# OER-9000/MB-iSTFT-VITS

Hardware: AMD Instinct MI355X
Metric: audio samples/sec (22.05 kHz), MB-iSTFT-VITS infer, batch 64 per GPU (higher is better)
Workload: dtype f32; 1 GPU; configs[1]: ljs_mb_istft_vits, batch 64 per GPU, infer(noise_scale=0, length_scale=1), all 8 outputs; global_batch=64, t_text=200, t_frames_max=566, parallelism=utterance-sharded dp1

## Files before the change

### include/mbistft_vits.h

```cpp
#ifndef MBISTFT_VITS_H
#define MBISTFT_VITS_H

#include <stddef.h>
#include <stdint.h>

#ifdef __cplusplus
extern "C" {
#endif

#define MBV_ABI_VERSION 3

#define MBV_DEC_MULTIBAND   0
#define MBV_DEC_MULTISTREAM 1
#define MBV_DEC_SINGLEBAND  2

typedef struct mbv_model mbv_model;

typedef struct mbv_config {
  int32_t struct_bytes;
  int32_t n_vocab;
  int32_t inter_channels;
  int32_t hidden_channels;
  int32_t filter_channels;
  int32_t n_heads;
  int32_t n_layers;
  int32_t kernel_size;
  int32_t upsample_initial_channel;
  int32_t spec_channels;
  int32_t resblock_kernel_sizes[3];
  int32_t resblock_dilations[3][3];
  int32_t resblock_type;
  int32_t n_speakers;
  int32_t gin_channels;
  int32_t decoder;
  int32_t device;
  int32_t use_sdp;
} mbv_config;

typedef struct mbv_outputs {
  float *o;
  float *o_mb;
  float *spec;
  float *phase;
  float *attn;
  float *y_mask;
  float *z;
  float *z_p;
  float *m_p;
  float *logs_p;
} mbv_outputs;

int  mbv_abi_version(void);
int  mbv_create(const mbv_config *cfg, mbv_model **out);
void mbv_destroy(mbv_model *m);
const char *mbv_last_error(const mbv_model *m);

int mbv_load_weight(mbv_model *m, const char *name, const float *data,
                    const int64_t *shape, int ndim);
int mbv_finalize_weights(mbv_model *m, void *stream);

int64_t mbv_arena_floats(mbv_model *m);
int mbv_export_arena(mbv_model *m, float *dst, int64_t capacity, void *stream);
int mbv_import_arena(mbv_model *m, const float *src, int64_t n_floats, void *stream);
int mbv_missing_weights(mbv_model *m, char *buf, size_t cap);

int mbv_encode(mbv_model *m, const int64_t *ids, const int64_t *lengths, const int64_t *sid,
               int B, int T, float length_scale, const float *noise_w, float noise_scale_w,
               int64_t *y_lengths_out, void *stream);

int mbv_synthesize(mbv_model *m, int t_frames, const float *noise, float noise_scale,
                   int max_len, const mbv_outputs *outs, void *stream);

int mbv_decode(mbv_model *m, const float *z, const float *g, int B, int t_frames,
               const mbv_outputs *outs, void *stream);

int mbv_decoder_context(const mbv_config *cfg, int32_t out[2]);
int mbv_decode_range(mbv_model *m, const float *z, const float *g, int B, int t_frames, int first, int count,
                     float *o, int64_t o_row_stride, void *stream);

int mbv_ragged_classes(const mbv_config *cfg, int splitk, int t_max, int32_t *first, int capacity);
int mbv_ragged_plan(const mbv_config *cfg, int splitk, int B, int t_frames, const int64_t *lengths, int32_t *run_of_row);
int mbv_decode_ragged(mbv_model *m, const float *z, const float *g, int B, int t_frames, const int64_t *lengths_host,
                      float *o, void *stream);
int mbv_synthesize_ragged(mbv_model *m, int t_frames, const float *noise, float noise_scale, int max_len,
                          const mbv_outputs *outs, const int64_t *y_lengths_host, void *stream);

typedef struct mbv_chunk {
  const float *z;
  int64_t z_stride;
  const float *g;
  int32_t t_frames;
  int32_t first, count;
  float *o;
} mbv_chunk;
int mbv_chunks_plan(const mbv_config *cfg, int splitk, int n, const int32_t *t_frames, int32_t *run_of_chunk);
int mbv_decode_chunks(mbv_model *m, const mbv_chunk *chunks_host, int n, void *stream);
int mbv_decode_chunks_routed(mbv_model *m, const mbv_chunk *chunks_host, const int32_t *route_frames, int n,
                             void *stream);
int64_t mbv_decoder_runs(mbv_model *m);

int mbv_tail_plan(const mbv_config *cfg, int32_t *out, int capacity);
int mbv_decode_masked(mbv_model *m, const float *z, const float *g, const int32_t *lengths, int B, int t_frames,
                      const mbv_outputs *outs, void *stream);
int64_t mbv_tail_dropped(mbv_model *m);

typedef struct mbv_enc_row {
  float length_scale, noise_scale_w;
  const float *noise_w;
  const void *durations;
  int32_t durations_dtype;
  int32_t t_text;
} mbv_enc_row;
typedef struct mbv_row {
  const float *noise;
  int64_t noise_stride;
  float noise_scale;
  int32_t keep;
  float *z;
} mbv_row;
int mbv_admit_plan(const mbv_config *cfg, int splitk, int n, const int32_t *t_text, int32_t *run_of_request);
int mbv_encode_rows(mbv_model *m, int slot, const int64_t *ids, const int64_t *lengths, const int64_t *sid, int B, int T,
                    const mbv_enc_row *rows_host, int64_t *y_lengths_out, void *stream);
int mbv_synthesize_rows(mbv_model *m, int slot, int t_frames, const mbv_row *rows_host, int n, void *stream);
int64_t mbv_encoder_runs(mbv_model *m);

int mbv_speaker_embedding(mbv_model *m, const int64_t *sid, int B, float *out, void *stream);

#define MBV_SPEAKER_SLOTS 256
#define MBV_BLEND_MAX 16
typedef struct mbv_speaker_def {
  int32_t slot;
  int32_t count;
  int32_t ids[MBV_BLEND_MAX];
  float weights[MBV_BLEND_MAX];
  const float *vector;
} mbv_speaker_def;
int mbv_speakers_define(mbv_model *m, const mbv_speaker_def *defs, int n, void *stream);
int mbv_speaker_release(mbv_model *m, int slot, void *stream);
int mbv_speaker_slots(void);
int mbv_speaker_defined(mbv_model *m, int64_t sid);
int64_t mbv_speaker_runs(mbv_model *m);

int mbv_set_option(mbv_model *m, const char *name, int value);
int mbv_get_option(mbv_model *m, const char *name);

int mbv_stage_times_ms(mbv_model *m, float out[5]);
int64_t mbv_ticket(mbv_model *m);
int mbv_stage_times_ms_at(mbv_model *m, int64_t ticket, float out[5]);

int mbv_kernel_times_ms(mbv_model *m, float out[2]);

int mbv_istft_pqmf(mbv_model *m, const float *x_post, int B, int t_frames, const float *filter,
                   int multistream, float *o, float *o_mb, float *spec, float *phase,
                   void *stream);

int mbv_voice_conversion(mbv_model *m, const float *y, const int64_t *y_lengths,
                         const int64_t *sid_src, const int64_t *sid_tgt, int B, int T,
                         const float *noise, const mbv_outputs *outs, int32_t *status, void *stream);

typedef struct mbv_align_outputs {
  int32_t *w;
  float *attn;
  float *x_mask;
  float *y_mask;
  float *z;
  float *z_p;
  float *m_p;
  float *logs_p;
  float *neg_cent;
} mbv_align_outputs;
int mbv_align(mbv_model *m, const int64_t *ids, const int64_t *lengths, const float *y, const int64_t *y_lengths,
              const int64_t *sid, int B, int T_text, int T_spec, const float *noise, float noise_scale,
              const mbv_align_outputs *outs, int32_t *status, void *stream);

int mbv_set_durations(mbv_model *m, const void *w, int dtype, int B, int T, int64_t *y_lengths_out, void *stream);

int mbv_istft_finalize(mbv_model *m, const float *spec, const float *phase, int B, int frames,
                       float *o, float *o_mb, void *stream);

int mbv_pcm16(mbv_model *m, const float *wave, const int64_t *y_lengths, int B, int64_t stride,
              int auto_normalize, int16_t *pcm, void *stream);

int mbv_pcm16_samples(mbv_model *m, const float *wave, const int64_t *valid_samples, int B, int64_t stride,
                      int auto_normalize, int16_t *pcm, void *stream);

#define MBV_RESAMPLE_KAISER_BEST 0
#define MBV_RESAMPLE_KAISER_FAST 1
// ... 210 lines not shown
  const void *wave;
  int64_t samples;
  int32_t wave_dtype;
  int32_t sid_src, sid_tgt;
  const float *noise;
  float noise_scale;
  float *z;
} mbv_convert_row;
int mbv_convert_plan(const mbv_config *cfg, int splitk, int n, const int32_t *t_frames, int32_t *run_of_request);
int mbv_convert_rows(mbv_model *m, const mbv_convert_row *rows_host, int n, int t_frames, int hop, int win,
                     float *g_out, void *stream);
int64_t mbv_converter_runs(mbv_model *m);

typedef struct mbv_convert_range {
  const void *wave;
  int64_t arrived;
  int32_t closed;
  int32_t wave_dtype;
  int32_t sid_src, sid_tgt;
  int32_t first, count;
  const float *noise;
  int64_t noise_stride;
  float noise_scale;
  float *z;
  int64_t z_stride;
} mbv_convert_range;
int mbv_converter_context(const mbv_config *cfg, int32_t out[2]);
int64_t mbv_spectrogram_ready(int64_t arrived, int closed, int n_fft, int hop);
int mbv_convert_window(const mbv_config *cfg, int first, int count, int64_t final_frames, int32_t out[2]);
int mbv_convert_ranges_plan(const mbv_config *cfg, int n, const int32_t *window_frames, int32_t *run_of_range);
int mbv_convert_ranges(mbv_model *m, const mbv_convert_range *rows_host, int n, int hop, int win, void *stream);

int64_t mbv_read_stage(mbv_model *m, const char *name, float *dst, int64_t capacity,
                       void *stream);

int mbv_op_rel_attention(mbv_model *m, const float *qkv, const float *emb_k, const float *emb_v,
                         const int64_t *lengths, float *o, int B, int H, int n_heads, int T, void *stream);

int mbv_op_conv1d(mbv_model *m, const float *x, const float *w_host, const float *bias_host,
                  float *y, int B, int Cin, int Cout, int T, int K, int dilation,
                  float in_slope, void *stream);

#define MBV_CONV_KIND_CONV 0
#define MBV_CONV_KIND_CONVT4 4
#define MBV_CONV_KIND_CONVT8 8
#define MBV_CONV_EPI_STORE 0
#define MBV_CONV_EPI_RESID 1
#define MBV_CONV_EPI_RESID_ACC 2
#define MBV_CONV_EPI_LN 7
typedef struct mbv_conv_desc {
  int32_t B, Cin, Cout, Tin, T, K, dil;
  int32_t x_rstride;
  int32_t kind;
  int32_t epi;
  float in_slope;
  int32_t relu, reflect1;
  const int32_t *in_lens;
  const int32_t *out_lens;
  const float *chan_add;
  const float *res;
  const float *res_chan_add;
  const float *accum_in;
  float out_scale;
  const int64_t *trim_lens;
  int32_t trim_num, trim_add;
  int32_t splitk;
  int32_t prec;
  int32_t legacy_convt;
  int64_t ws_floats;
  int32_t n_counters;
  const float *ln_gamma;
  const float *ln_beta;
  const int32_t *ln_out_lens;
  int32_t tail_once;
} mbv_conv_desc;
#define MBV_ROUTE_NARROW_M 1
#define MBV_ROUTE_NARROW_LAUNCH 2
#define MBV_ROUTE_M64 3
#define MBV_ROUTE_HALF 4
#define MBV_ROUTE_SMALL 5
#define MBV_ROUTE_BIG 6
#define MBV_ROUTE_SPLIT_BATCH 7
#define MBV_ROUTE_VS 8
int mbv_op_conv(mbv_model *m, const mbv_conv_desc *d, const float *x, const float *w_host, const float *bias_host,
                float *y, int32_t *plan_out, void *stream);
int mbv_conv_plan(const mbv_conv_desc *d, int32_t out[8]);

int mbv_op_embed(mbv_model *m, const int64_t *ids, const int64_t *lengths, const float *emb, float *x, int32_t *lens32,
                 int32_t *bad, int B, int T, int H, int n_vocab, void *stream);
int mbv_op_layernorm(mbv_model *m, const float *a, const float *r, const float *gamma, const float *beta, float *y,
                     int B, int C, int T, int pre_relu, const int32_t *out_lens, void *stream);
int mbv_op_durations(mbv_model *m, const float *h, const float *w, const float *bias, const int32_t *lens,
                     float length_scale, float *logw, float *w_ceil, int32_t *cum, int32_t *ylen32, int64_t *ylen64,
                     const int32_t *bad, int B, int C, int T, void *stream);
int mbv_op_expand(mbv_model *m, const float *stats, const int32_t *cum, const int32_t *ylen32, const float *noise,
                  float noise_scale, float *m_p, float *logs_p, float *z_p, float *z, float *attn, float *y_mask,
                  int B, int I, int T, int Tp, void *stream);
int mbv_op_cond_gemv(mbv_model *m, const float *g, const float *W, const float *bias, float *out, int B, int Cin,
                     int Cout, void *stream);
int mbv_op_gather_rows(mbv_model *m, const float *table, const int64_t *sid, float *out, int B, int C, int n_rows,
                       int32_t *bad, void *stream);
int mbv_op_posterior_sample(mbv_model *m, const float *stats, const float *noise, const int32_t *lens, float *z,
                            int B, int I, int T, void *stream);
int mbv_op_lens(mbv_model *m, const int64_t *lengths, int32_t *lens32, int32_t *bad, float *mask, int B, int T,
                void *stream);
int mbv_op_dds_sep(mbv_model *m, const float *x, const int32_t *lens, const float *w, const float *bias,
                   const float *gamma, const float *beta, float *y, int B, int C, int T, int K, int dil, void *stream);
int mbv_op_dds_res(mbv_model *m, const float *a, const float *xres, const float *gamma, const float *beta, float *y,
                   int B, int C, int T, const int32_t *out_lens, void *stream);
int mbv_op_sdp_pre(mbv_model *m, const float *z, int zc, const float *pre_w, const float *pre_b, const float *cond,
                   float *h, int B, int C, int T, void *stream);
int mbv_op_sdp_spline(mbv_model *m, const float *h, float *z, const int32_t *lens, int B, int C, int T,
                      float edge_const, void *stream);
int mbv_op_sdp_logw(mbv_model *m, const float *z, const float *mean, const float *logs, const int32_t *lens,
                    float *logw, int B, int T, void *stream);
int mbv_op_sdp_noise(mbv_model *m, const float *noise, float scale, float *z, int64_t n, void *stream);
int mbv_op_chan_add(mbv_model *m, float *x, const float *v, int B, int C, int T, void *stream);
int mbv_op_istft_single(mbv_model *m, const float *x_post, int B, int frames, int prescaled, float *o, float *spec,
                        float *phase, void *stream);
int mbv_op_neg_cent(mbv_model *m, const float *z_p, const float *m_p, const float *logs_p, const int32_t *t_y32,
                    const int32_t *t_x32, float *value, int B, int I, int T_t, int T_s, void *stream);
int mbv_op_max_path(mbv_model *m, const float *value, const int32_t *t_y32, const int32_t *t_x32, int32_t *w_out,
                    int32_t *path_out, int32_t *status, int B, int T_t, int T_s, void *stream);

#ifdef __cplusplus
}
#endif
#endif
```

### mb-istft-vits_amd/_capi.py

```python
import ctypes as C
import os
import subprocess

_HERE = os.path.dirname(os.path.abspath(__file__))
CSRC = os.path.join(_HERE, "csrc")
LIB_PATH = os.environ.get("MBV_LIB") or os.path.join(CSRC, "libmbistft_vits.so")

SYMBOLS = [
    "mbv_abi_version", "mbv_create", "mbv_destroy", "mbv_last_error", "mbv_load_weight",
    "mbv_finalize_weights", "mbv_missing_weights", "mbv_encode", "mbv_synthesize", "mbv_decode",
    "mbv_speaker_embedding", "mbv_stage_times_ms", "mbv_istft_pqmf", "mbv_read_stage",
    "mbv_op_conv1d", "mbv_kernel_times_ms", "mbv_istft_finalize", "mbv_pcm16", "mbv_voice_conversion",
    "mbv_set_option", "mbv_arena_floats", "mbv_export_arena", "mbv_import_arena", "mbv_ticket", "mbv_stage_times_ms_at", "mbv_op_rel_attention",
    "mbv_pcm16_samples", "mbv_resample", "mbv_resample_bank", "mbv_op_conv", "mbv_conv_plan",
    "mbv_spectrogram", "mbv_spectrogram_frames", "mbv_decoder_context", "mbv_decode_range",
    "mbv_resample_ready", "mbv_resample_pcm16_range",
    "mbv_ragged_classes", "mbv_decode_ragged", "mbv_synthesize_ragged", "mbv_ragged_plan",
    "mbv_chunks_plan", "mbv_decode_chunks", "mbv_decoder_runs",
    "mbv_pcm_chunks_plan", "mbv_resample_pcm16_chunks", "mbv_wire_runs",
    "mbv_op_embed", "mbv_op_layernorm", "mbv_op_durations", "mbv_op_expand", "mbv_op_cond_gemv", "mbv_op_gather_rows",
    "mbv_op_posterior_sample", "mbv_op_lens", "mbv_op_dds_sep", "mbv_op_dds_res", "mbv_op_sdp_pre", "mbv_op_sdp_spline",
    "mbv_op_sdp_logw", "mbv_op_sdp_noise", "mbv_op_chan_add", "mbv_op_istft_single",
    "mbv_align", "mbv_set_durations", "mbv_op_neg_cent", "mbv_op_max_path",
    "mbv_admit_plan", "mbv_encode_rows", "mbv_synthesize_rows", "mbv_encoder_runs", "mbv_get_option",
    "mbv_tail_plan", "mbv_tail_dropped", "mbv_decode_masked",
    "mbv_convert_plan", "mbv_convert_rows", "mbv_converter_runs",
    "mbv_decode_chunks_routed", "mbv_converter_context", "mbv_spectrogram_ready", "mbv_convert_window",
    "mbv_convert_ranges_plan", "mbv_convert_ranges",
    "mbv_resample_ready_open", "mbv_resample_ranges", "mbv_input_runs",
    "mbv_randn_blocks", "mbv_randn_host", "mbv_noise_runs",
    "mbv_limiter_ready", "mbv_resample_pcm16_range_limited", "mbv_resample_pcm16_chunks_limited",
    "mbv_g711_encode", "mbv_g711_decode", "mbv_resample_g711_range", "mbv_resample_g711_chunks",
    "mbv_pcm_fade_make", "mbv_resample_pcm16_range_faded", "mbv_resample_pcm16_chunks_faded",
    "mbv_resample_g711_range_faded", "mbv_resample_g711_chunks_faded",
    "mbv_token_marks", "mbv_token_marks_rows",
    "mbv_kweighting", "mbv_loudness_segments", "mbv_loudness", "mbv_loudness_range", "mbv_loudness_chunks",
    "mbv_loudness_runs",
    "mbv_turn_plan", "mbv_resample_turns",
    "mbv_shape_durations", "mbv_shape_durations_rows", "mbv_op_shape_durations", "mbv_shape_runs",
    "mbv_frame_gain", "mbv_frame_gain_rows", "mbv_op_frame_gain", "mbv_gain_runs",
    "mbv_resample_pcm16_range_shaped", "mbv_resample_pcm16_chunks_shaped", "mbv_resample_turns_shaped",
    "mbv_warp_plan", "mbv_warp_ready", "mbv_warp_ranges", "mbv_warp_runs",
    "mbv_speakers_define", "mbv_speaker_release", "mbv_speaker_slots", "mbv_speaker_defined", "mbv_speaker_runs",
]


ABI_VERSION = 3


class MbvConfig(C.Structure):
    _fields_ = [
        ("struct_bytes", C.c_int32), ("n_vocab", C.c_int32), ("inter_channels", C.c_int32),
        ("hidden_channels", C.c_int32), ("filter_channels", C.c_int32), ("n_heads", C.c_int32),
        ("n_layers", C.c_int32), ("kernel_size", C.c_int32),
        ("upsample_initial_channel", C.c_int32), ("spec_channels", C.c_int32),
        ("resblock_kernel_sizes", C.c_int32 * 3), ("resblock_dilations", (C.c_int32 * 3) * 3),
        ("resblock_type", C.c_int32),
        ("n_speakers", C.c_int32), ("gin_channels", C.c_int32), ("decoder", C.c_int32),
        ("device", C.c_int32), ("use_sdp", C.c_int32),
    ]


class MbvOutputs(C.Structure):
    _fields_ = [(n, C.c_void_p) for n in
                ("o", "o_mb", "spec", "phase", "attn", "y_mask", "z", "z_p", "m_p", "logs_p")]


class MbvChunk(C.Structure):
    _fields_ = [("z", C.c_void_p), ("z_stride", C.c_int64), ("g", C.c_void_p), ("t_frames", C.c_int32),
                ("first", C.c_int32), ("count", C.c_int32), ("o", C.c_void_p)]


class MbvPcmChunk(C.Structure):
    _fields_ = [("wave", C.c_void_p), ("in_total", C.c_int64), ("valid_samples", C.c_void_p),
                ("in_avail", C.c_int64), ("out_first", C.c_int64), ("out_count", C.c_int64), ("peak", C.c_void_p),
                ("pcm", C.c_void_p), ("pcm_capacity", C.c_int64), ("running_peak", C.c_void_p),
                ("out_samples", C.c_void_p)]


class MbvPcmLimit(C.Structure):
    _fields_ = [("ceiling", C.c_float), ("lookahead", C.c_int32), ("hold", C.c_int32)]


class MbvPcmFade(C.Structure):
    _fields_ = [("first", C.c_int64), ("count", C.c_int64), ("inv", C.c_float)]


def pcm_fade(first, count):
    f = MbvPcmFade()
    if lib().mbv_pcm_fade_make(int(first), int(count), C.byref(f)):
        raise ValueError("a fade is (first, count) with first >= 0 and count >= 0, got (%r, %r)" % (first, count))
    return f


NO_FADE = (0, -1, 0.0)


class MbvTurnSeg(C.Structure):
    _fields_ = [("wave", C.c_void_p), ("start", C.c_int64), ("length", C.c_int64), ("ramp", C.c_int32)]


class MbvTurnChunk(C.Structure):
    _fields_ = [("chunk", MbvPcmChunk), ("segs", C.POINTER(MbvTurnSeg)), ("n_segs", C.c_int32)]


TURN_MAX_SEGS = 4096


# ... 41 lines not shown


class MbvLoudnessChunk(C.Structure):
    _fields_ = [("wave", C.c_void_p), ("in_total", C.c_int64), ("valid_samples", C.c_void_p), ("in_avail", C.c_int64),
                ("seg_first", C.c_int64), ("seg_count", C.c_int64), ("state", C.c_void_p), ("energies", C.c_void_p),
                ("energy_capacity", C.c_int64), ("loudness", C.c_void_p)]


def kweighting(rate):
    c, m = (C.c_double * 10)(), (C.c_double * 16)()
    if lib().mbv_kweighting(int(rate), c, m):
        raise ValueError((lib().mbv_last_error(None) or b"mbv_kweighting failed").decode())
    return list(c), list(m)


def loudness_segments(rate, samples):
    hop = C.c_int32()
    n = lib().mbv_loudness_segments(int(rate), int(samples), C.byref(hop))
    if n < 0:
        raise ValueError((lib().mbv_last_error(None) or b"mbv_loudness_segments failed").decode())
    return int(hop.value), int(n)


class MbvEncRow(C.Structure):
    _fields_ = [("length_scale", C.c_float), ("noise_scale_w", C.c_float), ("noise_w", C.c_void_p),
                ("durations", C.c_void_p), ("durations_dtype", C.c_int32), ("t_text", C.c_int32)]


class MbvRow(C.Structure):
    _fields_ = [("noise", C.c_void_p), ("noise_stride", C.c_int64), ("noise_scale", C.c_float), ("keep", C.c_int32),
                ("z", C.c_void_p)]


class MbvConvertRow(C.Structure):
    _fields_ = [("wave", C.c_void_p), ("samples", C.c_int64), ("wave_dtype", C.c_int32), ("sid_src", C.c_int32),
                ("sid_tgt", C.c_int32), ("noise", C.c_void_p), ("noise_scale", C.c_float), ("z", C.c_void_p)]


class MbvConvertRange(C.Structure):
    _fields_ = [("wave", C.c_void_p), ("arrived", C.c_int64), ("closed", C.c_int32), ("wave_dtype", C.c_int32),
                ("sid_src", C.c_int32), ("sid_tgt", C.c_int32), ("first", C.c_int32), ("count", C.c_int32),
                ("noise", C.c_void_p), ("noise_stride", C.c_int64), ("noise_scale", C.c_float), ("z", C.c_void_p),
                ("z_stride", C.c_int64)]


class MbvResampleRange(C.Structure):
    _fields_ = [("wave", C.c_void_p), ("wave_dtype", C.c_int32), ("in_avail", C.c_int64), ("in_total", C.c_int64),
                ("out_first", C.c_int64), ("out_count", C.c_int64), ("out", C.c_void_p), ("out_capacity", C.c_int64)]


class MbvRandnBlock(C.Structure):
    _fields_ = [("dst", C.c_void_p), ("stride", C.c_int64), ("channels", C.c_int32), ("reserved", C.c_int32),
                ("first", C.c_int64), ("count", C.c_int64), ("seed", C.c_uint64), ("purpose", C.c_uint32),
                ("row", C.c_uint32)]


G711_LAWS = {"ulaw": 1, "alaw": 2}
WAVE_F32, WAVE_PCM16, WAVE_ULAW, WAVE_ALAW = 0, 1, 8, 9


NOISE_PRIOR, NOISE_SDP, NOISE_POSTERIOR = 0, 1, 2


class MbvAlignOutputs(C.Structure):
    _fields_ = [(n, C.c_void_p) for n in
                ("w", "attn", "x_mask", "y_mask", "z", "z_p", "m_p", "logs_p", "neg_cent")]


class MbvConvDesc(C.Structure):
    _fields_ = [(n, C.c_int32) for n in ("B", "Cin", "Cout", "Tin", "T", "K", "dil", "x_rstride", "kind", "epi")] + [
        ("in_slope", C.c_float), ("relu", C.c_int32), ("reflect1", C.c_int32),
        ("in_lens", C.c_void_p), ("out_lens", C.c_void_p), ("chan_add", C.c_void_p), ("res", C.c_void_p),
        ("res_chan_add", C.c_void_p), ("accum_in", C.c_void_p), ("out_scale", C.c_float),
        ("trim_lens", C.c_void_p), ("trim_num", C.c_int32), ("trim_add", C.c_int32),
        ("splitk", C.c_int32), ("prec", C.c_int32), ("legacy_convt", C.c_int32),
        ("ws_floats", C.c_int64), ("n_counters", C.c_int32),
        ("ln_gamma", C.c_void_p), ("ln_beta", C.c_void_p), ("ln_out_lens", C.c_void_p),
        ("tail_once", C.c_int32),
    ]


CONV_KIND_CONV, CONV_KIND_CONVT4, CONV_KIND_CONVT8 = 0, 4, 8
CONV_EPI_STORE, CONV_EPI_RESID, CONV_EPI_RESID_ACC, CONV_EPI_LN = 0, 1, 2, 7
ROUTES = {1: "NARROW_M", 2: "NARROW_LAUNCH", 3: "M64", 4: "HALF", 5: "SMALL", 6: "BIG", 7: "SPLIT_BATCH", 8: "VS"}
PLAN_FIELDS = ("route", "bm", "bn", "threads", "ck", "nb_big", "vs_tv", "S")


def build(force=False, verbose=False):
    if force:
        for f in os.listdir(CSRC):
            if f.endswith(".o") or f.endswith(".so"):
                os.remove(os.path.join(CSRC, f))
    r = subprocess.run(["bash", os.path.join(CSRC, "build.sh")], capture_output=True, text=True)
    if verbose or r.returncode:
        print(r.stdout, r.stderr)
    if r.returncode:
        raise RuntimeError("building libmbistft_vits.so failed:\n" + r.stderr[-4000:])
    return LIB_PATH


_lib = None


def lib():
    global _lib
    if _lib is not None:
        return _lib
    if not os.path.isfile(LIB_PATH):
        raise RuntimeError("%s not found: build it with `python -c 'import __graft_entry__ as g; "
                           "g.build()'` (hipcc, gfx950). There is no CPU fallback." % LIB_PATH)
    import torch
    L = C.CDLL(LIB_PATH)
    vp, i32, i64p, fp = C.c_void_p, C.c_int, C.POINTER(C.c_int64), C.c_void_p
    L.mbv_abi_version.restype = i32
    L.mbv_create.argtypes = [C.POINTER(MbvConfig), C.POINTER(vp)]
    L.mbv_destroy.argtypes = [vp]
    L.mbv_destroy.restype = None
    L.mbv_last_error.argtypes = [vp]
    L.mbv_last_error.restype = C.c_char_p
    L.mbv_load_weight.argtypes = [vp, C.c_char_p, vp, i64p, i32]
    L.mbv_finalize_weights.argtypes = [vp, vp]
    L.mbv_missing_weights.argtypes = [vp, C.c_char_p, C.c_size_t]
    L.mbv_encode.argtypes = [vp, vp, vp, vp, i32, i32, C.c_float, vp, C.c_float, vp, vp]
    L.mbv_synthesize.argtypes = [vp, i32, vp, C.c_float, i32, C.POINTER(MbvOutputs), vp]
    L.mbv_decode.argtypes = [vp, vp, vp, i32, i32, C.POINTER(MbvOutputs), vp]
    L.mbv_decoder_context.argtypes = [C.POINTER(MbvConfig), C.POINTER(C.c_int32 * 2)]
    L.mbv_decode_range.argtypes = [vp, vp, vp, i32, i32, i32, i32, vp, C.c_int64, vp]
    L.mbv_speaker_embedding.argtypes = [vp, vp, i32, vp, vp]
    L.mbv_stage_times_ms.argtypes = [vp, C.POINTER(C.c_float * 5)]
    L.mbv_kernel_times_ms.argtypes = [vp, C.POINTER(C.c_float * 2)]
    L.mbv_istft_pqmf.argtypes = [vp, vp, i32, i32, vp, i32, vp, vp, vp, vp, vp]
    L.mbv_istft_finalize.argtypes = [vp, vp, vp, i32, i32, vp, vp, vp]
    L.mbv_voice_conversion.argtypes = [vp, vp, vp, vp, vp, i32, i32, vp, C.POINTER(MbvOutputs), vp, vp]
    L.mbv_pcm16.argtypes = [vp, vp, vp, i32, C.c_int64, i32, vp, vp]
    L.mbv_pcm16_samples.argtypes = [vp, vp, vp, i32, C.c_int64, i32, vp, vp]
    L.mbv_resample.argtypes = [vp, vp, vp, i32, C.c_int64, i32, i32, i32, vp, C.c_int64, vp, vp]
    L.mbv_resample_bank.argtypes = [i32, i32, i32, vp, C.c_int64, C.POINTER(C.c_int32), C.POINTER(C.c_int32),
                                    C.POINTER(C.c_int32)]
    L.mbv_resample_ready.argtypes = [i32, i32, i32, C.c_int64, C.c_int64]
    L.mbv_resample_ready.restype = C.c_int64
    L.mbv_resample_pcm16_range.argtypes = [vp, vp, vp, i32, C.c_int64, i32, i32, i32, C.c_int64, C.c_int64, C.c_int64,
                                           vp, vp, C.c_int64, vp, vp, vp]
    L.mbv_spectrogram.argtypes = [vp, vp, i32, vp, i32, C.c_int64, i32, i32, i32, vp, C.c_int64, vp, vp]
    L.mbv_spectrogram_frames.argtypes = [C.c_int64, i32, i32]
    L.mbv_spectrogram_frames.restype = C.c_int64
    L.mbv_set_option.argtypes = [vp, C.c_char_p, i32]
    L.mbv_ticket.argtypes = [vp]
    L.mbv_ticket.restype = C.c_int64
    L.mbv_stage_times_ms_at.argtypes = [vp, C.c_int64, C.POINTER(C.c_float * 5)]
    L.mbv_arena_floats.argtypes = [vp]
    L.mbv_arena_floats.restype = C.c_int64
    L.mbv_export_arena.argtypes = [vp, vp, C.c_int64, vp]
    L.mbv_import_arena.argtypes = [vp, vp, C.c_int64, vp]
    L.mbv_read_stage.argtypes = [vp, C.c_char_p, vp, C.c_int64, vp]
    L.mbv_read_stage.restype = C.c_int64
    L.mbv_op_rel_attention.argtypes = [vp, vp, vp, vp, vp, vp, i32, i32, i32, i32, vp]
    L.mbv_op_conv1d.argtypes = [vp, vp, vp, vp, vp, i32, i32, i32, i32, i32, i32, C.c_float, vp]
    L.mbv_op_conv.argtypes = [vp, C.POINTER(MbvConvDesc), vp, vp, vp, vp, C.POINTER(C.c_int32 * 8), vp]
    L.mbv_conv_plan.argtypes = [C.POINTER(MbvConvDesc), C.POINTER(C.c_int32 * 8)]
    f32 = C.c_float
    L.mbv_op_embed.argtypes = [vp, vp, vp, vp, vp, vp, vp, i32, i32, i32, i32, vp]
    L.mbv_op_layernorm.argtypes = [vp, vp, vp, vp, vp, vp, i32, i32, i32, i32, vp, vp]
    L.mbv_op_durations.argtypes = [vp, vp, vp, vp, vp, f32, vp, vp, vp, vp, vp, vp, i32, i32, i32, vp]
    L.mbv_op_expand.argtypes = [vp, vp, vp, vp, vp, f32, vp, vp, vp, vp, vp, vp, i32, i32, i32, i32, vp]
    L.mbv_op_cond_gemv.argtypes = [vp, vp, vp, vp, vp, i32, i32, i32, vp]
    L.mbv_op_gather_rows.argtypes = [vp, vp, vp, vp, i32, i32, i32, vp, vp]
    L.mbv_op_posterior_sample.argtypes = [vp, vp, vp, vp, vp, i32, i32, i32, vp]
    L.mbv_op_lens.argtypes = [vp, vp, vp, vp, vp, i32, i32, vp]
    L.mbv_op_dds_sep.argtypes = [vp, vp, vp, vp, vp, vp, vp, vp, i32, i32, i32, i32, i32, vp]
    L.mbv_op_dds_res.argtypes = [vp, vp, vp, vp, vp, vp, i32, i32, i32, vp, vp]
    L.mbv_op_sdp_pre.argtypes = [vp, vp, i32, vp, vp, vp, vp, i32, i32, i32, vp]
    L.mbv_op_sdp_spline.argtypes = [vp, vp, vp, vp, i32, i32, i32, f32, vp]
    L.mbv_op_sdp_logw.argtypes = [vp, vp, vp, vp, vp, vp, i32, i32, vp]
    L.mbv_op_sdp_noise.argtypes = [vp, vp, f32, vp, C.c_int64, vp]
    L.mbv_op_chan_add.argtypes = [vp, vp, vp, i32, i32, i32, vp]
    L.mbv_op_istft_single.argtypes = [vp, vp, i32, i32, i32, vp, vp, vp, vp]
    L.mbv_align.argtypes = [vp, vp, vp, vp, vp, vp, i32, i32, i32, vp, f32, C.POINTER(MbvAlignOutputs), vp, vp]
    L.mbv_set_durations.argtypes = [vp, vp, i32, i32, i32, vp, vp]
    L.mbv_op_neg_cent.argtypes = [vp, vp, vp, vp, vp, vp, vp, i32, i32, i32, i32, vp]
    L.mbv_op_max_path.argtypes = [vp, vp, vp, vp, vp, vp, vp, i32, i32, i32, vp]
    optional = ("mbv_ragged_classes", "mbv_ragged_plan", "mbv_decode_ragged", "mbv_synthesize_ragged",
                "mbv_chunks_plan", "mbv_decode_chunks", "mbv_decoder_runs",
                "mbv_pcm_chunks_plan", "mbv_resample_pcm16_chunks", "mbv_wire_runs",
                "mbv_admit_plan", "mbv_encode_rows", "mbv_synthesize_rows", "mbv_encoder_runs",
                "mbv_get_option", "mbv_tail_plan", "mbv_tail_dropped", "mbv_decode_masked",
                "mbv_convert_plan", "mbv_convert_rows", "mbv_converter_runs",
                "mbv_decode_chunks_routed", "mbv_converter_context", "mbv_spectrogram_ready", "mbv_convert_window",
                "mbv_convert_ranges_plan", "mbv_convert_ranges",
                "mbv_resample_ready_open", "mbv_resample_ranges", "mbv_input_runs",
                "mbv_randn_blocks", "mbv_randn_host", "mbv_noise_runs",
                "mbv_limiter_ready", "mbv_resample_pcm16_range_limited", "mbv_resample_pcm16_chunks_limited",
                "mbv_g711_encode", "mbv_g711_decode", "mbv_resample_g711_range",
                "mbv_resample_g711_chunks",
                "mbv_pcm_fade_make", "mbv_resample_pcm16_range_faded", "mbv_resample_pcm16_chunks_faded",
                "mbv_resample_g711_range_faded", "mbv_resample_g711_chunks_faded",
                "mbv_token_marks", "mbv_token_marks_rows",
                "mbv_kweighting", "mbv_loudness_segments", "mbv_loudness", "mbv_loudness_range", "mbv_loudness_chunks",
                "mbv_loudness_runs", "mbv_turn_plan", "mbv_resample_turns",
                "mbv_shape_durations", "mbv_shape_durations_rows", "mbv_op_shape_durations", "mbv_shape_runs",
                "mbv_frame_gain", "mbv_frame_gain_rows", "mbv_op_frame_gain", "mbv_gain_runs",
                "mbv_resample_pcm16_range_shaped", "mbv_resample_pcm16_chunks_shaped",
                "mbv_resample_turns_shaped",
                "mbv_warp_plan", "mbv_warp_ready", "mbv_warp_ranges", "mbv_warp_runs",
                "mbv_speakers_define", "mbv_speaker_release", "mbv_speaker_slots", "mbv_speaker_defined",
                "mbv_speaker_runs") if os.environ.get("MBV_LIB") else ()
    if hasattr(L, "mbv_ragged_classes") or not optional:
        L.mbv_ragged_classes.argtypes = [C.POINTER(MbvConfig), i32, i32, C.POINTER(C.c_int32), i32]
        L.mbv_ragged_plan.argtypes = [C.POINTER(MbvConfig), i32, i32, i32, i64p, C.POINTER(C.c_int32)]
        L.mbv_decode_ragged.argtypes = [vp, vp, vp, i32, i32, i64p, vp, vp]
        L.mbv_synthesize_ragged.argtypes = [vp, i32, vp, C.c_float, i32, C.POINTER(MbvOutputs), i64p, vp]
    if hasattr(L, "mbv_decode_chunks") or not optional:
        L.mbv_chunks_plan.argtypes = [C.POINTER(MbvConfig), i32, i32, C.POINTER(C.c_int32), C.POINTER(C.c_int32)]
        L.mbv_decode_chunks.argtypes = [vp, C.POINTER(MbvChunk), i32, vp]
        L.mbv_decoder_runs.argtypes = [vp]
        L.mbv_decoder_runs.restype = C.c_int64
    if hasattr(L, "mbv_resample_pcm16_chunks") or not optional:
        L.mbv_pcm_chunks_plan.argtypes = [i32, i32, i32, C.POINTER(MbvPcmChunk), i32, i64p]
        L.mbv_pcm_chunks_plan.restype = C.c_int64
        L.mbv_resample_pcm16_chunks.argtypes = [vp, C.POINTER(MbvPcmChunk), i32, i32, i32, i32, vp, C.c_int64, vp]
        L.mbv_wire_runs.argtypes = [vp]
        L.mbv_wire_runs.restype = C.c_int64
    if hasattr(L, "mbv_encode_rows") or not optional:
        L.mbv_admit_plan.argtypes = [C.POINTER(MbvConfig), i32, i32, C.POINTER(C.c_int32), C.POINTER(C.c_int32)]
        L.mbv_encode_rows.argtypes = [vp, i32, vp, vp, vp, i32, i32, C.POINTER(MbvEncRow), vp, vp]
        L.mbv_synthesize_rows.argtypes = [vp, i32, i32, C.POINTER(MbvRow), i32, vp]
        L.mbv_encoder_runs.argtypes = [vp]
        L.mbv_encoder_runs.restype = C.c_int64
        L.mbv_get_option.argtypes = [vp, C.c_char_p]
    if hasattr(L, "mbv_tail_plan") or not optional:
        L.mbv_tail_plan.argtypes = [C.POINTER(MbvConfig), C.POINTER(C.c_int32), i32]
        L.mbv_tail_dropped.argtypes = [vp]
        L.mbv_tail_dropped.restype = C.c_int64
        L.mbv_decode_masked.argtypes = [vp, vp, vp, vp, i32, i32, C.POINTER(MbvOutputs), vp]
    if hasattr(L, "mbv_convert_rows") or not optional:
        L.mbv_convert_plan.argtypes = [C.POINTER(MbvConfig), i32, i32, C.POINTER(C.c_int32), C.POINTER(C.c_int32)]
        L.mbv_convert_rows.argtypes = [vp, C.POINTER(MbvConvertRow), i32, i32, i32, i32, vp, vp]
        L.mbv_converter_runs.argtypes = [vp]
        L.mbv_converter_runs.restype = C.c_int64
    if hasattr(L, "mbv_convert_ranges") or not optional:
        L.mbv_decode_chunks_routed.argtypes = [vp, C.POINTER(MbvChunk), C.POINTER(C.c_int32), i32, vp]
        L.mbv_converter_context.argtypes = [C.POINTER(MbvConfig), C.POINTER(C.c_int32 * 2)]
        L.mbv_spectrogram_ready.argtypes = [C.c_int64, i32, i32, i32]
        L.mbv_spectrogram_ready.restype = C.c_int64
        L.mbv_convert_window.argtypes = [C.POINTER(MbvConfig), i32, i32, C.c_int64, C.POINTER(C.c_int32 * 2)]
        L.mbv_convert_ranges_plan.argtypes = [C.POINTER(MbvConfig), i32, C.POINTER(C.c_int32), C.POINTER(C.c_int32)]
        L.mbv_convert_ranges.argtypes = [vp, C.POINTER(MbvConvertRange), i32, i32, i32, vp]
    if hasattr(L, "mbv_resample_ranges") or not optional:
        L.mbv_resample_ready_open.argtypes = [i32, i32, i32, C.c_int64]
        L.mbv_resample_ready_open.restype = C.c_int64
        L.mbv_resample_ranges.argtypes = [vp, C.POINTER(MbvResampleRange), i32, i32, i32, i32, vp]
        L.mbv_input_runs.argtypes = [vp]
        L.mbv_input_runs.restype = C.c_int64
    if hasattr(L, "mbv_randn_blocks") or not optional:
        L.mbv_randn_blocks.argtypes = [vp, C.POINTER(MbvRandnBlock), i32, vp]
        L.mbv_randn_host.argtypes = [C.c_uint64, C.c_uint32, C.c_uint32, C.c_uint32, C.c_int64, C.c_int64, vp]
        L.mbv_noise_runs.argtypes = [vp]
        L.mbv_noise_runs.restype = C.c_int64
    if hasattr(L, "mbv_limiter_ready") or not optional:
        L.mbv_limiter_ready.argtypes = [i32, i32, i32, C.c_int64, C.c_int64, i32]
        L.mbv_limiter_ready.restype = C.c_int64
        L.mbv_resample_pcm16_range_limited.argtypes = [vp, vp, vp, i32, C.c_int64, i32, i32, i32, C.c_int64, C.c_int64,
                                                       C.c_int64, vp, vp, C.c_int64, vp, vp, C.POINTER(MbvPcmLimit), vp]
        L.mbv_resample_pcm16_chunks_limited.argtypes = [vp, C.POINTER(MbvPcmChunk), C.POINTER(MbvPcmLimit), i32, i32,
                                                        i32, i32, vp, C.c_int64, vp]
    if hasattr(L, "mbv_resample_g711_range") or not optional:
        L.mbv_g711_encode.argtypes = [vp, vp, C.c_int64, i32, vp, vp]
        L.mbv_g711_decode.argtypes = [vp, vp, C.c_int64, i32, vp, vp]
        L.mbv_resample_g711_range.argtypes = [vp, vp, vp, i32, C.c_int64, i32, i32, i32, C.c_int64, C.c_int64, C.c_int64,
                                              vp, vp, C.c_int64, vp, vp, C.POINTER(MbvPcmLimit), i32, vp]
        L.mbv_resample_g711_chunks.argtypes = [vp, C.POINTER(MbvPcmChunk), C.POINTER(MbvPcmLimit), i32, i32, i32, i32,
                                               i32, vp, C.c_int64, vp]
    if hasattr(L, "mbv_pcm_fade_make") or not optional:
        fadep = C.POINTER(MbvPcmFade)
        L.mbv_pcm_fade_make.argtypes = [C.c_int64, C.c_int64, fadep]
        L.mbv_resample_pcm16_range_faded.argtypes = [vp, vp, vp, i32, C.c_int64, i32, i32, i32, C.c_int64, C.c_int64,
                                                     C.c_int64, vp, vp, C.c_int64, vp, vp, C.POINTER(MbvPcmLimit),
                                                     fadep, vp]
        L.mbv_resample_pcm16_chunks_faded.argtypes = [vp, C.POINTER(MbvPcmChunk), C.POINTER(MbvPcmLimit), fadep, i32,
                                                      i32, i32, i32, vp, C.c_int64, vp]
        L.mbv_resample_g711_range_faded.argtypes = [vp, vp, vp, i32, C.c_int64, i32, i32, i32, C.c_int64, C.c_int64,
                                                    C.c_int64, vp, vp, C.c_int64, vp, vp, C.POINTER(MbvPcmLimit), i32,
                                                    fadep, vp]
        L.mbv_resample_g711_chunks_faded.argtypes = [vp, C.POINTER(MbvPcmChunk), C.POINTER(MbvPcmLimit), fadep, i32,
                                                     i32, i32, i32, i32, vp, C.c_int64, vp]
    if hasattr(L, "mbv_token_marks") or not optional:
        L.mbv_token_marks.argtypes = [vp, vp, C.c_int64, vp]
        L.mbv_token_marks_rows.argtypes = [vp, i32, C.POINTER(MbvMarkRow), i32, vp]
    if hasattr(L, "mbv_loudness") or not optional:
        dp = C.POINTER(C.c_double)
        L.mbv_kweighting.argtypes = [i32, dp, dp]
        L.mbv_loudness_segments.argtypes = [i32, C.c_int64, C.POINTER(C.c_int32)]
        L.mbv_loudness_segments.restype = C.c_int64
        L.mbv_loudness.argtypes = [vp, vp, vp, i32, C.c_int64, i32, vp, vp, vp]
        L.mbv_loudness_range.argtypes = [vp, vp, vp, i32, C.c_int64, i32, C.c_int64, C.c_int64, C.c_int64, vp, vp,
                                         C.c_int64, vp, vp]
        L.mbv_loudness_chunks.argtypes = [vp, C.POINTER(MbvLoudnessChunk), i32, i32, vp]
        L.mbv_loudness_runs.argtypes = [vp]
        L.mbv_loudness_runs.restype = C.c_int64
    if hasattr(L, "mbv_resample_turns") or not optional:
        L.mbv_turn_plan.argtypes = [i32, i32, i32, C.POINTER(MbvTurnChunk), C.POINTER(MbvPcmLimit), i32, i64p]
        L.mbv_turn_plan.restype = C.c_int64
        L.mbv_resample_turns.argtypes = [vp, C.POINTER(MbvTurnChunk), C.POINTER(MbvPcmLimit), C.POINTER(MbvPcmFade), i32,
                                         i32, i32, i32, i32, vp, C.c_int64, vp]
    if hasattr(L, "mbv_shape_durations") or not optional:
        L.mbv_shape_durations.argtypes = [vp, vp, vp, C.POINTER(MbvFit), i32, i32, vp, vp, vp]
        L.mbv_shape_durations_rows.argtypes = [vp, i32, C.POINTER(MbvShapeRow), i32, vp, vp]
        L.mbv_op_shape_durations.argtypes = [vp, vp, vp, vp, vp, f32, C.POINTER(MbvFit), vp, vp, vp, vp, vp, vp, i32, i32,
                                             vp]
        L.mbv_shape_runs.argtypes = [vp]
        L.mbv_shape_runs.restype = C.c_int64
    if hasattr(L, "mbv_frame_gain") or not optional:
        envp = C.POINTER(MbvPcmEnvelope)
        L.mbv_frame_gain.argtypes = [vp, vp, vp, C.c_int64, i32, vp]
        L.mbv_frame_gain_rows.argtypes = [vp, i32, C.POINTER(MbvGainRow), i32, vp]
        L.mbv_op_frame_gain.argtypes = [vp, vp, vp, vp, vp, C.c_int64, i32, i32, i32, vp]
        L.mbv_gain_runs.argtypes = [vp]
# ... 41 lines not shown
```

### mb-istft-vits_amd/csrc/capi.hip

```cpp
#include "../../include/mbistft_vits.h"
#include "kernels.h"
#include "g711.h"

#include <algorithm>
#include <array>
#include <cmath>
#include <cstdarg>
#include <cstdio>
#include <cstdlib>
#include <cstring>
#include <map>
#include <set>
#include <string>
#include <vector>

using namespace mbv;

namespace {

constexpr int kWindow = 4;
constexpr int kDpFilter = 256;
constexpr int kFlowLayers = 4;
constexpr int kFlowK = 5;
constexpr int kNFlows = 4;
// ... 886 lines not shown
    HIPCHK(m, hipMalloc((void**)&m->darena, arena.size() * sizeof(float)));
    m->darena_floats = arena.size();
  }
  if (m->import_src) {
    if ((int64_t)arena.size() != m->import_n)
      return m->fail("mbv_import_arena: %lld floats offered, this configuration's arena has %zu (exported by another configuration or library build?)",
                     (long long)m->import_n, arena.size());
    HIPCHK(m, hipMemcpyAsync(m->darena, m->import_src, arena.size() * sizeof(float), hipMemcpyDeviceToDevice, stream));
    m->raw.clear();
  } else {
    HIPCHK(m, hipMemcpyAsync(m->darena, arena.data(), arena.size() * sizeof(float),
                             hipMemcpyHostToDevice, stream));
  }
  HIPCHK(m, hipStreamSynchronize(stream));
  m->arena_used = arena.size();
  m->harena.swap(arena);
  m->finalized = true;
  m->split_valid = false;
  if (m->conv_bf16 == 3 && ensure_split_arena(m, stream)) return 1;
  return reblend_voices(m, stream);
}

struct Bump {
  char* base; size_t cap, off = 0;
  template <typename Tp> Tp* take(size_t n) {
    off = align_up(off, 256);
    Tp* p = base ? reinterpret_cast<Tp*>(base + off) : nullptr;
    off += n * sizeof(Tp);
    return p;
  }
  bool fits() const { return off <= cap; }
};

int ensure(mbv_model* m, char** buf, size_t* cap, size_t need) {
  if (*cap >= need) return 0;
  if (*buf) { HIPCHK(m, hipDeviceSynchronize()); HIPCHK(m, hipFree(*buf)); *buf = nullptr; *cap = 0; }
  need = align_up(need + (need >> 3), 1 << 20);
  HIPCHK(m, hipMalloc((void**)buf, need));
  *cap = need;
  return 0;
}

template <typename Carve>
int lay_out(mbv_model* m, const char* who, char** buf, size_t* cap, Carve&& carve) {
  Bump sc{*buf, *cap};
  if (*buf) carve(sc);
  if (*buf && sc.fits()) return 0;
  Bump measure{nullptr, 0};
  carve(measure);
  if (ensure(m, buf, cap, measure.off)) return 1;
  sc = Bump{*buf, *cap};
  carve(sc);
  return sc.fits() ? 0 : m->fail("%s: scratch layout exceeds its buffer", who);
}

ConvArgs conv_shape(int Cin, int M, int K, int dil, int Tin, int T, int B, int splitk) {
  ConvArgs a{};
  a.Cin = Cin; a.M = M; a.Mpad = (int)align_up(M, 128); a.K = K; a.dil = dil; a.pad_left = (K - 1) * dil / 2;
  a.Tin = Tin; a.x_rstride = Tin; a.x_bstride = (int64_t)Cin * Tin;
  a.T = T; a.y_bstride = (int64_t)M * T; a.epi = EPI_STORE; a.in_slope = 1.f; a.out_scale = 1.f; a.B = B;
  a.splitk = splitk;
  return a;
}

ConvArgs conv_bind(const mbv_model* m, const PConv& p, ConvArgs a, const float* x, float* y) {
  a.x = x; a.y = y;
  a.w = m->W(p.w); a.bias = p.has_bias ? m->W(p.bias) : nullptr;
  a.w_split = m->Wsplit(p.w);
  a.ws = m->conv_ws; a.ws_floats = m->conv_ws_floats; a.counters = m->conv_cnt; a.n_counters = m->conv_ncnt;
  a.prec = a.w_split ? 3 : 0;
  return a;
}

ConvArgs conv_args(const mbv_model* m, const PConv& p, const float* x, int64_t x_bstride, int Tin,
                   float* y, int64_t y_bstride, int T, int B, int dil = 1) {
  ConvArgs a = conv_shape(p.Cin, p.M, p.K, dil, Tin, T, B, m->splitk);
  a.x_bstride = x_bstride; a.y_bstride = y_bstride;
  return conv_bind(m, p, a, x, y);
}


int tail_mode(const mbv_model* m) { return (!m->trim && !m->splitk && m->conv_bf16 != 3) ? m->tail_once : 0; }
bool tail_stage(int mode, int B, long conv_tiles) { return B > 1 && (mode == 2 || (mode == 1 && conv_tiles > 256)); }

bool decoder_stage_concurrent(const mbv_model* m, int B, int ch, int Lo, bool tail = false) {
  const long conv_tiles = (long)B * ((Lo + 383) / 384) * ((ch + 127) / 128);
  return m->dec_streams && m->aux_ok && m->cfg.resblock_type != 2 && (conv_tiles <= 192 || tail) && !m->trim;
}

struct DecodeRange {
  int t_full;
  int keep_first, keep_count;
  float* o;
  int64_t o_row_stride;
  const PoolRow* rows = nullptr;
  int max_keep = 0;
};

std::vector<DecLaunch> decoder_table(const mbv_config& c) {
  const bool sb = c.decoder == MBV_DEC_SINGLEBAND;
  const int us = dec_us(c), C0 = c.upsample_initial_channel;
  const int kPre = 7, kPost = 7;
  const int n_fft = 16, hop = 4;
  const int bands = sb ? 1 : 4, taps = 63;
  const int nq = c.resblock_type == 2 ? 2 : 3;
  std::vector<DecLaunch> t;
  auto conv = [&](int kind, int stage, int j, int q, int Cin, int M, int K, int dil, int num, int epi) -> DecLaunch& {
    DecLaunch e{};
    e.kind = kind; e.stage = stage; e.j = j; e.q = q;
    e.Cin = Cin; e.M = M; e.K = K; e.dil = dil; e.pad_left = (K - 1) * dil / 2;
    e.num = e.rate = num; e.lens = stage + 1; e.epi = epi; e.res = epi == EPI_RESID || epi == EPI_RESID_ACC;
    t.push_back(e);
    return t.back();
  };
  conv(DL_PRE, -1, 0, 0, c.inter_channels, C0, kPre, 1, 1, EPI_STORE);
  int num = 1;
  for (int i = 0; i < 2; ++i) {
    const int ch = C0 >> (i + 1);
    DecLaunch& u = conv(DL_UP, i, 0, 0, C0 >> i, us * ch, convt_taps(us), 1, num, EPI_CONVT);
    u.pad_left = convt_pad_left(us); u.convt_u = us; u.rate = us * num; u.lens = i;
    u.tk = kConvtK; u.tp = (kConvtK - us) / 2;
    num *= us;
    for (int j = 0; j < 3; ++j) {
      const int k = c.resblock_kernel_sizes[j];
      for (int q = 0; q < nq; ++q) {
        const int d = c.resblock_dilations[j][q];
        const int last = q == nq - 1 ? EPI_RESID_ACC : EPI_RESID;
        if (c.resblock_type == 2) {
          DecLaunch& e = conv(DL_C2, i, j, q, ch, ch, k, d, num, last);
          e.chan_add = e.res_chan_add = q == 0;
        } else {
          conv(DL_C1, i, j, q, ch, ch, k, d, num, EPI_STORE).chan_add = q == 0;
          conv(DL_C2, i, j, q, ch, ch, k, 1, num, last).res_chan_add = q == 0;
        }
      }
    }
  }
  DecLaunch& p = conv(DL_POST, 2, 0, 0, C0 >> 2, 2 * (n_fft / 2 + 1) * bands, kPost, 1, num, EPI_STORE);
  p.add = 1; p.reflect1 = 1; p.lens = 2;
  DecLaunch w{};
  w.kind = DL_TAIL; w.stage = 2; w.num = num; w.add = 1; w.rate = num * hop * bands;
  w.n_fft = n_fft; w.hop = hop; w.bands = bands; w.taps = taps;
  t.push_back(w);
  return t;
}

ConvArgs dec_shape(const DecLaunch& e, int len, int B, int splitk) {
  ConvArgs a = conv_shape(e.Cin, e.M, e.K, e.dil, e.num * len, e.num * len + e.add, B, splitk);
  a.pad_left = e.pad_left; a.epi = e.epi; a.convt_u = e.convt_u; a.reflect1 = e.reflect1;
  if (e.res) a.res_bstride = a.y_bstride;
  return a;
}
ConvArgs dec_planner_args(const DecLaunch& e, int len, int B, int splitk, int prec = 0, bool cond = false) {
  static const float kSome = 0.f;
  ConvArgs a = dec_shape(e, len, B, splitk);
  if (e.res) a.res = &kSome;
  if (cond && e.chan_add) a.chan_add = &kSome;
  if (cond && e.res_chan_add) a.res_chan_add = &kSome;
  a.prec = prec;
  return a;
}

struct Span { int64_t lo, hi; };
static Span span_conv(Span y, int K, int dil, int pad_left) { return {y.lo - pad_left, y.hi + (int64_t)(K - 1) * dil - pad_left}; }
static int64_t floor_div(int64_t a, int64_t b) { return a >= 0 ? a / b : -((-a + b - 1) / b); }
static int64_t ceil_div(int64_t a, int64_t b) { return -floor_div(-a, b); }
// ... 3 lines not shown
void decoder_context(const std::vector<DecLaunch>& table, int* Lc, int* Rc) {
  const int64_t t = 1 << 20;
  Span x{}, need{}, r{};
  for (size_t n = table.size(); n-- > 0;) {
    const DecLaunch& e = table[n];
    switch (e.kind) {
      case DL_TAIL:
        x = {e.rate * t, e.rate * t + e.rate - 1};
        if (e.bands > 1) x = {ceil_div(x.lo - e.taps / 2, e.bands), floor_div(x.hi + e.taps / 2, e.bands)};
        x = {ceil_div(x.lo + e.n_fft / 2 - (e.n_fft - 1), e.hop), floor_div(x.hi + e.n_fft / 2, e.hop)};
        break;
      case DL_POST:
        need = r = x = span_conv(x, e.K, e.dil, e.pad_left + e.reflect1);
        break;
      case DL_C1: case DL_C2:
        if (e.epi == EPI_RESID_ACC) { need = span_union(need, r); r = x; }
        r = span_conv(r, e.K, e.dil, e.pad_left);
        break;
      case DL_UP:
        need = r = x = span_convt(span_union(need, r), e.tk, e.convt_u, e.tp);
        break;
      case DL_PRE:
        x = span_conv(x, e.K, e.dil, e.pad_left);
        break;
    }
  }
  *Lc = (int)(t - x.lo);
  *Rc = (int)(x.hi - t);
}

static int64_t reach_conv(int64_t hi, int pad_left) { return hi + pad_left; }
static int64_t reach_convt(int64_t hi, int k, int u, int p) { return (int64_t)u * hi - p + k - 1; }
struct TailLaunch { int kind, stage, j, q, rate, reach; };
void decoder_tail_plan(const std::vector<DecLaunch>& table, std::vector<TailLaunch>* out) {
  out->clear();
  const int64_t len = 1 << 20;
  int64_t sum_hi = len - 1;
  int64_t hi = sum_hi, r = sum_hi;
  for (const DecLaunch& e : table) {
    int64_t h = 0;
    switch (e.kind) {
      case DL_PRE:
        h = sum_hi = reach_conv(sum_hi, e.pad_left);
        break;
      case DL_UP:
        h = hi = r = sum_hi = reach_convt(sum_hi, e.tk, e.convt_u, e.tp);
        break;
      case DL_C1: case DL_C2:
        h = r = reach_conv(r, e.pad_left);
        if (e.epi == EPI_RESID_ACC) { h = sum_hi = sum_hi > r ? sum_hi : r; r = hi; }
        break;
      case DL_POST:
        h = sum_hi = reach_conv(sum_hi, e.pad_left + e.reflect1);
        break;
      case DL_TAIL:
        h = e.hop * sum_hi + e.n_fft / 2 - 1;
        if (e.bands > 1) h = e.bands * h + e.taps / 2;
        break;
    }
    out->push_back({e.kind, e.stage, e.j, e.q, e.rate, (int)(h - ((int64_t)e.rate * len - 1))});
  }
}

struct RaggedRows {
  const int* len;
  const int* len_u;
  const int* len_uu;
  const int* row_map;
  float* o;
  int64_t o_row_stride;
  int t_min;
};

struct DecCall { int B, Td, zstride; bool lens, cond, own_o, ranged, ragged; };

constexpr int kTrimMargin = 32;
struct DecBufs {
  DecCall call;
  bool trim, tail;
  float* x0;
  struct TrimMap { int num, add, T, bn; int* map; bool built; };
  TrimMap trim_maps[12]; int n_trim;
  int trim_of[48];
  struct TailMap { int kind, j, q, bn; const int* map; };
  struct Stage { float *u, *t1s[3], *rs[3], *xs, *cb[3]; bool conc; int n_tail; TailMap tail_maps[kTailMapJobs]; TailMapJobs jobs; } st[2];
  int Bc;
  float *xpost, *otmp;
};

void carve_decoder(const mbv_model* m, const DecCall& k, Bump& sc, DecBufs* out) {
  const mbv_config& c = m->cfg;
  const std::vector<DecLaunch>& table = m->dec_table;
  const int B = k.B, Td = k.Td;
  DecBufs& d = *out;
  std::memset(&d, 0, sizeof d); d.call = k;
  d.trim = k.ragged ? !m->splitk : (m->trim && k.lens && !m->splitk && c.decoder != MBV_DEC_SINGLEBAND);
  d.tail = tail_mode(m) && !d.trim && !k.ragged && !k.ranged && k.lens && B > 1 && B <= 65535 && !k.cond;
  auto planned = [&](const DecLaunch& e) {
    ConvArgs a = dec_planner_args(e, Td, B, m->splitk, m->Wsplit(0) ? 3 : 0,
                                  k.cond && e.stage >= 0 && e.stage < 2 && m->rb[e.stage * 3 + e.j].cw.present);
    if (e.kind == DL_PRE) { a.x_rstride = k.zstride; a.x_bstride = (int64_t)e.Cin * k.zstride; }
    return a;
  };
  std::vector<TailLaunch> tail_plan;
  if (d.tail) decoder_tail_plan(table, &tail_plan);
  d.x0 = sc.take<float>((size_t)B * table[0].M * Td);
  for (const DecLaunch& up : table) {
    if (up.kind != DL_UP) continue;
    DecBufs::Stage& st = d.st[up.stage];
    const int ch = up.M / up.convt_u, Lo = up.rate * Td;
    const size_t n = (size_t)B * ch * Lo;
    const long stage_tiles = (long)B * ((Lo + 383) / 384) * ((ch + 127) / 128);
    if (d.tail && tail_stage(tail_mode(m), B, stage_tiles))
      for (size_t n_e = 0; n_e < table.size() && st.n_tail < kTailMapJobs; ++n_e) {
        const DecLaunch& e = table[n_e];
        if (e.stage != up.stage || (e.kind != DL_C1 && e.kind != DL_C2)) continue;
        const ConvArgs a = planned(e);
        const int bn = conv1d_trim_bn(a);
        if (!bn || conv1d_plan(a, false).route != conv1d_plan(a, true).route) continue;
        st.jobs.job[st.n_tail] = {e.rate, tail_plan[n_e].reach, Lo, bn, nullptr};
        st.tail_maps[st.n_tail++] = {e.kind, e.j, e.q, bn, nullptr};
      }
    st.conc = decoder_stage_concurrent(m, B, ch, Lo, st.n_tail > 0) && !d.trim;
    st.u = sc.take<float>(n);
    for (int j = 0; j < 3; ++j) {
      st.t1s[j] = j == 0 || st.conc ? sc.take<float>(n) : st.t1s[0];
      st.rs[j] = j == 0 || st.conc ? sc.take<float>(n) : st.rs[0];
    }
    st.xs = sc.take<float>(n);
  }
  for (const DecLaunch& up : table)
    for (int j = 0; j < 3 && up.kind == DL_UP; ++j)
      if (k.cond && m->rb[up.stage * 3 + j].cw.present) d.st[up.stage].cb[j] = sc.take<float>((size_t)B * (up.M / up.convt_u));
  const DecLaunch& post = table[table.size() - 2];
  const int64_t utt_bytes = (int64_t)post.M * (post.num * (int64_t)Td + post.add) * 4;
  int64_t cap_bytes = (1LL << 31) - 1;
  if (m->xpost_chunk_bytes > 0 && m->xpost_chunk_bytes < cap_bytes) cap_bytes = m->xpost_chunk_bytes;
  d.Bc = utt_bytes > (1LL << 31) - 1 ? 0 : (int)std::min<int64_t>(B, std::max<int64_t>(1, cap_bytes / utt_bytes));
  for (size_t n_e = 0; n_e < table.size(); ++n_e) {
    const DecLaunch& e = table[n_e];
    d.trim_of[n_e] = -1;
    if (!d.trim || e.kind == DL_TAIL || (e.kind == DL_POST && d.Bc != B)) continue;
    const ConvArgs a = planned(e);
    const int bn = conv1d_trim_bn(a);
    for (int t = 0; bn && t < d.n_trim && d.trim_of[n_e] < 0; ++t)
      if (d.trim_maps[t].num == e.num && d.trim_maps[t].add == e.add && d.trim_maps[t].T == a.T && d.trim_maps[t].bn == bn) d.trim_of[n_e] = t;
    if (bn && d.trim_of[n_e] < 0 && d.n_trim < 12) {
      d.trim_of[n_e] = d.n_trim;
      d.trim_maps[d.n_trim++] = {e.num, e.add, a.T, bn, sc.take<int>(launch_trim_map_ints(B, a.T, bn)), false};
    }
  }
  for (auto& st : d.st)
    for (int i = 0; i < st.n_tail; ++i)
      st.tail_maps[i].map = st.jobs.job[i].out = sc.take<int>(launch_tail_map_ints(B, st.jobs.job[i].T, st.jobs.job[i].BN));
  d.xpost = sc.take<float>((size_t)d.Bc * (utt_bytes / 4));
  if (k.own_o) d.otmp = sc.take<float>((size_t)B * table.back().rate * Td);
}

int run_decoder(mbv_model* m, const float* z, const int* zlens, const float* gvec, const mbv_outputs* outs,
                hipStream_t s, DecBufs& d, const DecodeRange* rg = nullptr, const RaggedRows* rr = nullptr) {
  const mbv_config& c = m->cfg;
  const std::vector<DecLaunch>& table = m->dec_table;
  const int B = d.call.B, Td = d.call.Td, zstride = d.call.zstride, gin = c.gin_channels;
  ++m->decoder_runs;
  if (rr) zlens = rr->len;
  float* o = rg ? rg->o : rr ? rr->o : outs ? outs->o : nullptr;
  const bool pooled = rg && rg->rows;
  if (d.call.lens != (zlens != nullptr) || d.call.cond != (gvec && gin) || d.call.ranged != (rg != nullptr) ||
      d.call.ragged != (rr != nullptr) || d.call.own_o != (!o && !pooled))
    return m->fail("internal error: the decoder's scratch was laid out for another call");
  if (!d.Bc)
    return m->fail("utterance too long for one launch: %d frames (x_post of ONE utterance must stay below 2 GiB)", Td);
  if (!o) o = d.otmp;
  const int rt_num = rg && !m->splitk ? rg->t_full : 0;
  hipStream_t const s_main = s;
  const int* const rr_lens[3] = {rr ? rr->len : nullptr, rr ? rr->len_u : nullptr, rr ? rr->len_uu : nullptr};
  auto conv = [&](const DecLaunch& e, const PConv& p, const float* x, float* y, float in_slope, int nb) {
    ConvArgs a = conv_bind(m, p, dec_shape(e, Td, nb, m->splitk), x, y);
    a.in_slope = in_slope;
    if (rr) a.in_lens = rr_lens[e.lens];
    return a;
  };
  HIPCHK(m, hipEventRecord(m->evk[0], s));
  bool route_drift = false, tail_drift = false;
  auto narrow_alone = [&](const ConvArgs& a, int num, int add, int len) {
    ConvArgs s1 = a;
    s1.B = 1; s1.trim_map = nullptr;
    s1.T = num * len + add;
    s1.Tin = a.Tin - a.T + s1.T;
    s1.x_rstride = s1.Tin; s1.x_bstride = (int64_t)a.Cin * s1.Tin;
    s1.y_bstride = a.y_bstride / a.T * s1.T;
    s1.res_bstride = a.res ? (int64_t)a.M * s1.T : 0;
    const int r = conv1d_plan(s1, false).route;
    return r == CONV_NARROW_M || r == CONV_NARROW_LAUNCH;
  };
  auto with_trim = [&](ConvArgs& a, const DecLaunch& e) {
    if (rr && !m->splitk) {
      const bool narrow_long = narrow_alone(a, e.num, e.add, rg ? rg->t_full : Td);
      if (narrow_alone(a, e.num, e.add, rr->t_min) != narrow_long) route_drift = true;
      if (rg) {
        const int r = conv1d_plan(a, false, rt_num * e.num + e.add).route;
        if ((r == CONV_NARROW_M || r == CONV_NARROW_LAUNCH) != narrow_long) route_drift = true;
      }
    }
    if (!d.trim) return;
    const int at = d.trim_of[&e - table.data()], bn = conv1d_trim_bn(a);
    if (bn != (at < 0 ? 0 : d.trim_maps[at].bn)) { tail_drift = true; return; }
    if (at < 0) return;
    DecBufs::TrimMap& k = d.trim_maps[at];
    if (!k.built) launch_trim_map(zlens, B, e.num, e.num * (rr ? 0 : kTrimMargin) + e.add, a.T, bn, k.map, s_main);
    k.built = true;
    a.trim_map = k.map; a.trim_bn = bn;
  };
  const DecBufs::Stage* tail_stage_bufs = nullptr;
  auto with_tail = [&](ConvArgs& a, const DecLaunch& e) -> const DecBufs::TailMap* {
    for (int n_t = 0; n_t < tail_stage_bufs->n_tail; ++n_t) {
      const DecBufs::TailMap& t = tail_stage_bufs->tail_maps[n_t];
      if (t.kind != e.kind || t.j != e.j || t.q != e.q) continue;
      if (conv1d_trim_bn(a) != t.bn) { tail_drift = true; return nullptr; }
      a.trim_map = t.map; a.trim_bn = t.bn;
      return &t;
    }
    return nullptr;
  };
  {
    const DecLaunch& e = table[0];
    ConvArgs a = conv(e, m->conv_pre, z, d.x0, 1.f, B);
    a.x_bstride = (int64_t)e.Cin * zstride;
    a.x_rstride = zstride;
    a.in_lens = zlens;
    with_trim(a, e);
    launch_conv1d(a, s, rt_num);
  }
  m->stages["dec_conv_pre"] = {d.x0, (int64_t)B * table[0].M * Td};
  const float* cur = d.x0;
  size_t next = 1;
  for (int i = 0; i < 2; ++i) {
    DecBufs::Stage& bufs = d.st[i];
    const DecLaunch& up = table[next++];
    const int ch = up.M / up.convt_u;
    const size_t n = (size_t)B * ch * up.rate * Td;
    float *const u = bufs.u, *const xs = bufs.xs;
    const bool conc = bufs.conc;
    tail_stage_bufs = &bufs;
    launch_tail_maps(zlens, B, bufs.jobs, bufs.n_tail, m->tail_cnt, s_main);
    {
      ConvArgs a = conv(up, m->upc[i], cur, u, kLrelu, B);
      with_trim(a, up);
      launch_conv1d(a, s);
    }
    m->stages[i == 0 ? "dec_up_0" : "dec_up_1"] = {u, (int64_t)n};
    if (conc) {
      HIPCHK(m, hipEventRecord(m->ev_fork, s_main));
      for (auto& st : m->aux) HIPCHK(m, hipStreamWaitEvent(st, m->ev_fork, 0));
    }
    auto resblocks = [&]() -> int {
    for (int j = 0; j < 3; ++j) {
      const auto& R = m->rb[i * 3 + j];
      hipStream_t s = (conc && j > 0) ? m->aux[j - 1] : s_main;
      float* const t1 = bufs.t1s[j];
      float* const r = bufs.rs[j];
      auto own_ws = [&](ConvArgs& a) {
        if (!conc) return;
        const size_t third = a.ws_floats / 3;
        const int cthird = a.n_counters / 3;
        a.ws += (size_t)j * third; a.ws_floats = third;
        a.counters += (size_t)j * cthird; a.n_counters = cthird;
      };
      const float* cadd = nullptr;
      if (gvec && gin && R.cw.present) {
        launch_cond_gemv(gvec, nullptr, nullptr, m->W(R.cw.off), m->W(R.cb.off), bufs.cb[j], B, gin, ch, s);
        cadd = bufs.cb[j];
      }
      const float* state = u;
      for (; table[next].stage == i && table[next].j == j; ++next) {
        const DecLaunch& e = table[next];
        const bool first = e.kind == DL_C1, second = !first && c.resblock_type != 2;
        ConvArgs a = conv(e, second ? R.c2[e.q] : R.c1[e.q], second ? t1 : state, first ? t1 : r, kLrelu, B);
        if (e.res) a.res = state;
        if (e.chan_add) a.chan_add = cadd;
        if (e.res_chan_add) a.res_chan_add = cadd;
        if (e.epi == EPI_RESID_ACC) {
          a.y = xs;
          a.accum_in = j == 0 ? nullptr : xs;
          a.out_scale = j == 2 ? (1.f / 3.f) : 1.f;
          if (conc && j > 0) HIPCHK(m, hipStreamWaitEvent(s, m->ev_rb[j - 1], 0));
        }
        own_ws(a);
        with_trim(a, e);
        const DecBufs::TailMap* tm = with_tail(a, e);
        launch_conv1d(a, s, rt_num * e.num);
        if (tm) launch_tail_fill(a.y, a.y_bstride, B, a.M, a.T, tm->bn, tm->map, s);
        if (conc && e.epi == EPI_RESID_ACC) HIPCHK(m, hipEventRecord(m->ev_rb[j], s));
        if (!first) state = r;
      }
    }
    return 0;
    };
    if (resblocks()) {
      if (conc) for (auto& st : m->aux) (void)hipStreamSynchronize(st);
      return 1;
    }
    if (conc) HIPCHK(m, hipStreamWaitEvent(s_main, m->ev_rb[2], 0));
    m->stages[i == 0 ? "dec_res_0" : "dec_res_1"] = {xs, (int64_t)n};
    cur = xs;
  }
  const DecLaunch &post = table[next], &wave = table[next + 1];
  const bool sb = wave.bands == 1;
  const int L = post.num * Td, Fr = L + post.add, prow = post.M, Bc = d.Bc;
  const int bins = wave.n_fft / 2 + 1;
  float* const xpost = d.xpost;
  const int upf = wave.rate / 4;
  IstftRange keep{rg ? upf * rg->keep_first : 0, rg ? upf * (rg->keep_first + rg->keep_count) : 0,
                  rg ? rg->o_row_stride : 0, nullptr, nullptr};
  if (rr) keep = IstftRange{0, upf * Td, rr->o_row_stride, rr->len, rr->row_map};
  const int64_t M4 = (int64_t)wave.rate * Td;
  for (int b0 = 0; b0 < B; b0 += Bc) {
    const int nb = B - b0 < Bc ? B - b0 : Bc;
    {
      ConvArgs a = conv(post, m->conv_post, cur + (size_t)b0 * post.Cin * L, xpost, 0.01f, nb);
      if (rr) a.in_lens += b0;
      if (nb == B) with_trim(a, post);
      launch_conv1d(a, s);
    }
    if (b0 == 0) HIPCHK(m, hipEventRecord(m->evk[1], s));
    const bool plain = !rg && !rr;
    float* const ob = pooled ? nullptr : rr ? o : o + (size_t)b0 * (rg ? rg->o_row_stride : M4);
    auto extra = [&](float* p, int64_t per_row) { return plain && p ? p + (size_t)b0 * per_row : nullptr; };
    IstftRange kb = keep;
    if (rr) { kb.row_lens += b0; kb.row_map += b0; }
    if (sb) {
      IstftSbArgs ia{};
      ia.x_post = xpost; ia.o = ob;
      ia.spec = extra(outs ? outs->spec : nullptr, bins * Fr);
      ia.phase = extra(outs ? outs->phase : nullptr, bins * Fr);
      ia.B = nb; ia.F = Fr; ia.exact_math = m->exact_math; ia.prescaled = 1;
      if (pooled) launch_istft_single_pool(ia, rg->rows + b0, rg->max_keep, s);
      else if (!plain) launch_istft_single_range(ia, kb, s);
      else launch_istft_single(ia, s);
    } else {
      IstftArgs ia{};
      const bool ms = c.decoder == MBV_DEC_MULTISTREAM;
      ia.x_post = xpost; ia.filt = m->W(m->filt.off); ia.o = ob;
      ia.o_mb = extra(outs ? outs->o_mb : nullptr, (ms ? wave.bands : 1) * M4);
      ia.spec = extra(outs ? outs->spec : nullptr, wave.bands * bins * Fr);
      ia.phase = extra(outs ? outs->phase : nullptr, wave.bands * bins * Fr);
      ia.B = nb; ia.Tp = Td; ia.multistream = ms;
      ia.fixed_bank = !ia.multistream; ia.exact_math = m->exact_math; ia.prescaled = 1;
      if (plain && d.trim && nb == B && !ia.o_mb && !ia.spec && !ia.phase) ia.trim_lens = zlens;
      if (pooled) launch_istft_pqmf_pool(ia, rg->rows + b0, rg->max_keep, s);
      else if (!plain) launch_istft_pqmf_range(ia, kb, s);
      else launch_istft_pqmf(ia, s);
    }
  }
  if (Bc == B) m->stages["x_post"] = {xpost, (int64_t)B * prow * Fr};
  m->xpost_F = Fr;
  m->xpost_rows = prow;
  HIPCHK(m, hipEventRecord(m->evk[2], s));
  m->evk_set = true;
  m->evk_split = Bc < B;
  if (tail_drift) return m->fail("internal error: a tile map was planned for another tile width than its launch uses");
  if (route_drift) return m->fail("internal error: a %s run holds rows whose convs plan differently (ragged_classes out of step with run_decoder)", pooled ? "pooled" : "ragged");
  return 0;
}

void ragged_classes(const mbv_config& c, int splitk, int t_max, std::vector<int>* first) {
  first->assign(1, 1);
  if (splitk) return;
  const std::vector<DecLaunch> table = decoder_table(c);
  std::vector<char> prev, cur;
  for (int len = 1; len <= t_max; ++len) {
    cur.clear();
    for (const DecLaunch& e : table) {
      if (e.kind == DL_TAIL) continue;
      const int r = conv1d_plan(dec_planner_args(e, len, 1, 0), false).route;
// ... 3402 lines not shown
  OP_REFUSE((int64_t)B * 18 * frames * 4 >= (1LL << 31), "x_post must stay below 2 GiB");
  OP_BEGIN();
  IstftSbArgs a{};
  a.x_post = x_post; a.o = o; a.spec = spec; a.phase = phase;
  a.B = B; a.F = frames; a.exact_math = m->exact_math; a.prescaled = prescaled != 0;
  launch_istft_single(a, s);
  OP_END();
}

int mbv_op_neg_cent(mbv_model* m, const float* z_p, const float* m_p, const float* logs_p, const int32_t* t_y32,
                    const int32_t* t_x32, float* value, int B, int I, int T_t, int T_s, void* stream) {
  if (!m) return 1;
  OP_REFUSE(!z_p || !m_p || !logs_p || !t_y32 || !t_x32 || !value, "NULL argument");
  OP_REFUSE(B <= 0 || I <= 0 || T_t <= 0 || T_s <= 0, "B, I, T_t and T_s must be > 0");
  OP_REFUSE(B > kGridYZ || (T_t + 63) / 64 > kGridYZ, "B <= 65535 and T_t <= 64 * 65535 required");
  OP_BEGIN();
  launch_neg_cent(z_p, m_p, logs_p, (int64_t)I * T_s, t_y32, t_x32, value, B, I, T_t, T_s, s);
  OP_END();
}

int mbv_op_max_path(mbv_model* m, const float* value, const int32_t* t_y32, const int32_t* t_x32, int32_t* w_out,
                    int32_t* path_out, int32_t* status, int B, int T_t, int T_s, void* stream) {
  if (!m) return 1;
  OP_REFUSE(!value || !t_y32 || !t_x32 || !w_out, "NULL argument");
  OP_REFUSE(B <= 0 || T_t <= 0 || T_s <= 0, "B, T_t and T_s must be > 0");
  OP_REFUSE(!max_path_supported(T_s), "T_s must be <= 1024");
  OP_BEGIN();
  const size_t bits_bytes = max_path_scratch_bytes(B, T_t, T_s);
  if (bits_bytes && ensure(m, &m->scrB, &m->scrB_bytes, bits_bytes)) return 1;
  launch_max_path(value, t_y32, t_x32, w_out, path_out, status, bits_bytes ? m->scrB : nullptr, B, T_t, T_s, s);
  OP_END();
}
#undef OP_REFUSE
#undef OP_BEGIN
#undef OP_END

int mbv_op_conv1d(mbv_model* m, const float* x, const float* w_host, const float* bias_host, float* y,
                  int B, int Cin, int Cout, int T, int K, int dilation, float in_slope, void* stream) {
  if (!m) return 1;
  if (Cin % 32) return m->fail("mbv_op_conv1d: Cin must be a multiple of 32");
  if (!conv1d_supported(K, dilation)) return m->fail("mbv_op_conv1d: K <= 11 and (K-1)*dilation <= 72 required");
  DEVICE_GUARD(m);
  hipStream_t s = (hipStream_t)stream;
  const int Mpad = (int)align_up(Cout, 128);
  std::vector<float> packed((size_t)K * Cin * Mpad, 0.f);
  for (int k = 0; k < K; ++k)
    for (int ci = 0; ci < Cin; ++ci)
      for (int co = 0; co < Cout; ++co)
        packed[conv_pack_index(k, ci, co, Cin, Mpad)] = w_host[((size_t)co * Cin + ci) * K + k];
  float *dw = nullptr, *db = nullptr;
  HIPCHK(m, hipMalloc((void**)&dw, packed.size() * 4));
  HIPCHK(m, hipMemcpy(dw, packed.data(), packed.size() * 4, hipMemcpyHostToDevice));
  if (bias_host) {
    HIPCHK(m, hipMalloc((void**)&db, (size_t)Cout * 4));
    HIPCHK(m, hipMemcpy(db, bias_host, (size_t)Cout * 4, hipMemcpyHostToDevice));
  }
  ConvArgs a{};
  a.x = x; a.x_bstride = (int64_t)Cin * T; a.Tin = T; a.x_rstride = T; a.Cin = Cin;
  a.w = dw; a.bias = db; a.M = Cout; a.Mpad = Mpad; a.K = K; a.dil = dilation;
  a.pad_left = (K - 1) * dilation / 2; a.in_slope = in_slope;
  a.y = y; a.y_bstride = (int64_t)Cout * T; a.T = T; a.epi = EPI_STORE; a.out_scale = 1.f; a.B = B;
  a.ws = m->conv_ws; a.ws_floats = m->conv_ws_floats; a.counters = m->conv_cnt; a.n_counters = m->conv_ncnt;
  a.splitk = m->splitk;
  float* dws = nullptr;
  if (m->conv_bf16 == 3) {
    HIPCHK(m, hipMalloc((void**)&dws, packed.size() * 4));
    launch_split_planes(dw, dws, packed.size(), s);
    a.w_split = dws;
  }
  a.prec = a.w_split ? 3 : 0;
  launch_conv1d(a, s);
  HIPCHK(m, hipStreamSynchronize(s));
  HIPCHK(m, hipFree(dw));
  if (dws) HIPCHK(m, hipFree(dws));
  if (db) HIPCHK(m, hipFree(db));
  return 0;
}

}

namespace {
static_assert(MBV_ROUTE_NARROW_M == CONV_NARROW_M && MBV_ROUTE_NARROW_LAUNCH == CONV_NARROW_LAUNCH &&
              MBV_ROUTE_M64 == CONV_M64 && MBV_ROUTE_HALF == CONV_HALF && MBV_ROUTE_SMALL == CONV_SMALL &&
              MBV_ROUTE_BIG == CONV_BIG && MBV_ROUTE_SPLIT_BATCH == CONV_SPLIT_BATCH && MBV_ROUTE_VS == CONV_VS,
              "route numbers of the C-ABI and the launcher");
static_assert(MBV_CONV_EPI_LN == EPI_LN, "epilogue numbers of the C-ABI and the launcher");

const char* conv_desc_args(const mbv_conv_desc& d, ConvArgs* out) {
  const bool convt = d.kind == MBV_CONV_KIND_CONVT4 || d.kind == MBV_CONV_KIND_CONVT8;
  if (d.kind != MBV_CONV_KIND_CONV && !convt) return "kind must be MBV_CONV_KIND_CONV, _CONVT4 or _CONVT8";
  if (d.B <= 0 || d.Cin <= 0 || d.Cout <= 0 || d.Tin <= 0 || d.T <= 0) return "B, Cin, Cout, Tin and T must be > 0";
  if (d.x_rstride != 0 && d.x_rstride < d.Tin) return "x_rstride must be 0 or >= Tin";
  const bool ln = d.epi == MBV_CONV_EPI_LN;
  if ((d.epi < MBV_CONV_EPI_STORE || d.epi > MBV_CONV_EPI_RESID_ACC) && !ln) return "epi must be STORE, RESID, RESID_ACC or LN";
  if (d.prec != 0 && d.prec != 3) return "prec must be 0 or 3";
  if (d.epi == MBV_CONV_EPI_STORE && (d.res || d.res_chan_add)) return "res / res_chan_add need a RESID epilogue";
  if (d.epi != MBV_CONV_EPI_STORE && !ln && !d.res) return "RESID and RESID_ACC need res";
  if (d.epi != MBV_CONV_EPI_STORE && !ln && (d.out_lens || d.relu)) return "out_lens / relu belong to STORE and LN";
  if (!ln && (d.ln_gamma || d.ln_beta || d.ln_out_lens)) return "ln_gamma / ln_beta / ln_out_lens belong to LN";
  if (ln) {
    if (convt) return "LN: a conv only";
    if (!d.ln_gamma || !d.ln_beta) return "LN needs ln_gamma and ln_beta";
    if (d.res_chan_add || d.trim_lens || d.prec) return "LN takes no res_chan_add, no trimmed launch and no prec 3";
    if (d.T > 256) return "LN: T <= 256 (the narrow kernel's rule in mbv_encode)";
  }
  if (d.epi != MBV_CONV_EPI_RESID_ACC && d.accum_in) return "accum_in belongs to RESID_ACC";
  if (d.legacy_convt) return "legacy_convt must be 0 (the stand-alone ConvTranspose kernel was removed)";
  if (d.trim_lens && d.splitk) return "a trimmed launch takes no split-K";
  if (d.tail_once && (!d.trim_lens || convt || ln)) return "tail_once needs trim_lens and a conv with a STORE / RESID / RESID_ACC epilogue";
  const int U = d.kind;
  if (convt) {
    if (d.T != d.Tin) return "ConvTranspose: T must equal Tin (input frames)";
    if (d.epi != MBV_CONV_EPI_STORE || d.out_lens || d.relu || d.reflect1) return "ConvTranspose: plain STORE only";
    if (d.Cin % 16 || d.Cout % 32) return "ConvTranspose: Cin % 16 == 0 and Cout % 32 == 0";
  } else {
    if (d.Cin % 32) return "conv: Cin must be a multiple of 32";
    if (!conv1d_supported(d.K, d.dil)) return "conv: K <= 11 and (K - 1) * dil <= 72 required";
  }
  ConvArgs a{};
  a.Tin = d.Tin; a.x_rstride = d.x_rstride ? d.x_rstride : d.Tin; a.Cin = d.Cin;
  a.x_bstride = (int64_t)d.Cin * a.x_rstride;
  a.M = convt ? U * d.Cout : d.Cout;
  a.Mpad = (int)align_up(a.M, 128);
  a.K = convt ? convt_taps(U) : d.K;
  a.dil = convt ? 1 : d.dil;
  a.pad_left = convt ? convt_pad_left(U) : (a.K - 1) * a.dil / 2;
  a.in_slope = d.in_slope;
  a.in_lens = d.in_lens; a.chan_add = d.chan_add; a.reflect1 = d.reflect1;
  a.T = d.T;
  a.y_bstride = (int64_t)d.Cout * d.T * (convt ? U : 1);
  a.epi = convt ? EPI_CONVT : d.epi;
  a.convt_u = convt ? U : 0;
  a.relu = d.relu; a.out_lens = d.out_lens;
  a.res = d.res; a.res_bstride = (int64_t)d.Cout * d.T; a.res_chan_add = d.res_chan_add;
  a.accum_in = d.accum_in; a.out_scale = d.epi == MBV_CONV_EPI_RESID_ACC ? d.out_scale : 1.f;
  a.B = d.B;
  a.splitk = d.splitk != 0;
  a.prec = d.prec;
  if ((a.epi == EPI_RESID || a.epi == EPI_RESID_ACC) && (unsigned long long)a.M * a.T * 4ull >= (1ull << 32))
    return "one utterance's output exceeds 4 GiB";
  if (ln) {
    a.ln_gamma = d.ln_gamma; a.ln_beta = d.ln_beta; a.ln_out_lens = d.ln_out_lens;
    if (!conv1d_narrow_supported(a)) return "LN outside the narrow kernel's range (conv1d_narrow_supported)";
  }
  *out = a;
  return nullptr;
}

void plan_ints(const ConvPlan& p, int32_t* out) {
  const int32_t v[8] = {p.route, p.bm, p.bn, p.threads, p.ck, p.nb_big, p.vs_tv, p.S};
  std::memcpy(out, v, sizeof v);
}

const char* conv_desc_plan(const mbv_conv_desc& d, const ConvArgs& a, ConvPlan* p) {
  if (d.trim_lens) {
    const int bn = conv1d_trim_bn(a);
    if (!bn) return "this conv runs on a kernel without trimmed launches (conv1d_trim_bn 0)";
    *p = conv1d_plan(a, true);
    if (p->bn != bn) return "internal error: conv1d_trim_bn and the trimmed plan disagree";
    return nullptr;
  }
  *p = conv1d_plan(a, false);
  return nullptr;
}

struct DevAllocs {
  std::vector<void*> p;
  ~DevAllocs() { for (void* q : p) (void)hipFree(q); }
};
}

extern "C" {

int mbv_conv_plan(const mbv_conv_desc* d, int32_t out[8]) {
  if (!d || !out) { g_create_error = "mbv_conv_plan: NULL argument"; return 1; }
  ConvArgs a{};
  const char* why = conv_desc_args(*d, &a);
  ConvPlan p{};
  if (!why) {
    a.ws_floats = d->ws_floats > 0 ? (size_t)d->ws_floats : 0;
    a.n_counters = d->n_counters > 0 ? d->n_counters : 0;
    why = conv_desc_plan(*d, a, &p);
  }
  if (why) { g_create_error = std::string("mbv_conv_plan: ") + why; return 1; }
  plan_ints(p, out);
  return 0;
}

int mbv_op_conv(mbv_model* m, const mbv_conv_desc* d, const float* x, const float* w_host, const float* bias_host,
                float* y, int32_t* plan_out, void* stream) {
  if (!m) return 1;
  if (!d || !x || !w_host || !y) return m->fail("mbv_op_conv: NULL argument");
  ConvArgs a{};
  const char* why = conv_desc_args(*d, &a);
  if (why) return m->fail("mbv_op_conv: %s", why);
  a.ws = m->conv_ws; a.ws_floats = m->conv_ws_floats; a.counters = m->conv_cnt; a.n_counters = m->conv_ncnt;
  if (m->splitk && !d->trim_lens) a.splitk = 1;
  ConvPlan p{};
  if ((why = conv_desc_plan(*d, a, &p))) return m->fail("mbv_op_conv: %s", why);
  DEVICE_GUARD(m);
  hipStream_t s = (hipStream_t)stream;
  DevAllocs mem;
  auto upload = [&](const void* src, size_t bytes, void** dst) -> int {
    HIPCHK(m, hipMalloc(dst, bytes));
    mem.p.push_back(*dst);
    HIPCHK(m, hipMemcpy(*dst, src, bytes, hipMemcpyHostToDevice));
    return 0;
  };
  const bool convt = a.epi == EPI_CONVT;
  const int U = a.convt_u;
  std::vector<float> zero_bias;
  if (!bias_host) { zero_bias.assign(d->Cout, 0.f); bias_host = zero_bias.data(); }
  std::vector<float> wp((size_t)a.K * a.Cin * a.Mpad, 0.f), bp(a.M);
  if (convt) {
    pack_convt_rows(w_host, bias_host, a.Cin, d->Cout, U, a.Mpad, wp.data(), bp.data());
  } else {
    std::vector<int> rows(a.M);
    for (int i = 0; i < a.M; ++i) rows[i] = i;
    pack_conv_rows(w_host, a.Cin, a.K, rows.data(), a.M, nullptr, a.Mpad, wp.data());
    std::memcpy(bp.data(), bias_host, (size_t)a.M * 4);
  }
  void *dw = nullptr, *db = nullptr;
  if (upload(wp.data(), wp.size() * 4, &dw) || upload(bp.data(), bp.size() * 4, &db)) return 1;
  a.w = (const float*)dw; a.bias = (const float*)db;
  if (a.prec == 3) {
    void* dws = nullptr;
    HIPCHK(m, hipMalloc(&dws, wp.size() * 4));
    mem.p.push_back(dws);
    launch_split_planes(a.w, (float*)dws, wp.size(), s);
    a.w_split = (const float*)dws;
  }
  a.x = x; a.y = y;
  if (d->trim_lens) {
    std::vector<int> l32(d->B);
    for (int b = 0; b < d->B; ++b) {
      const int64_t v = d->trim_lens[b];
      l32[b] = v < 0 ? 0 : (v > a.T ? a.T : (int)v);
    }
    void* dl = nullptr;
    if (upload(l32.data(), l32.size() * 4, &dl)) return 1;
    void* map = nullptr;
    HIPCHK(m, hipMalloc(&map, launch_trim_map_ints(d->B, a.T, p.bn) * sizeof(int)));
    mem.p.push_back(map);
    if (d->tail_once) {
      if (d->B > 65535) return m->fail("mbv_op_conv: tail_once takes at most 65535 rows");
      void* tmap = nullptr;
      HIPCHK(m, hipMalloc(&tmap, launch_tail_map_ints(d->B, a.T, p.bn) * sizeof(int)));
      mem.p.push_back(tmap);
      TailMapJobs jobs{};
      jobs.job[0] = {d->trim_num, d->trim_add, a.T, p.bn, (int*)tmap};
      launch_tail_maps((const int*)dl, d->B, jobs, 1, m->tail_cnt, s);
      map = tmap;
    } else {
      launch_trim_map((const int*)dl, d->B, d->trim_num, d->trim_add, a.T, p.bn, (int*)map, s);
    }
    a.trim_map = (const int*)map; a.trim_bn = p.bn;
  }
  launch_conv1d(a, s);
  if (d->tail_once) launch_tail_fill(a.y, a.y_bstride, a.B, a.M, a.T, a.trim_bn, a.trim_map, s);
  HIPCHK(m, hipGetLastError());
  HIPCHK(m, hipStreamSynchronize(s));
  if (plan_out) plan_ints(p, plan_out);
  return 0;
}

}
```

### mb-istft-vits_amd/csrc/conv1d.hip

```cpp
#include "kernels.h"
#include <cstdio>
#include <cstdlib>

#ifndef MBV_CONV_GLDS
#define MBV_CONV_GLDS 8
#endif
namespace mbv {

typedef float f32x16 __attribute__((ext_vector_type(16)));
typedef float f32x4 __attribute__((ext_vector_type(4)));

__device__ __forceinline__ float lrelu(float v, float slope) { return v > 0.f ? v : v * slope; }
__device__ __forceinline__ float sigmoidf_(float v) { return 1.f / (1.f + expf(-v)); }

#ifdef MBV_CONV_STAMPS
#define MBV_CSTAMP(ID)                                                                        \
  if ((tid & 255) == 0 && stamp_n < 511) stamp_lds[tid >> 8][++stamp_n] = (__builtin_amdgcn_s_memrealtime() << 4) | (unsigned)(ID);
#define MBV_CSTAMP_FLUSH()                                                                    \
  {                                                                                           \
    if ((tid & 255) == 0) stamp_lds[tid >> 8][0] = stamp_n;                                   \
    __syncthreads();                                                                          \
    unsigned long long* sb_ = reinterpret_cast<unsigned long long*>(a.ws) + (size_t)blockIdx.x * 1024; \
    for (int e = tid; e < 1024; e += NT) sb_[e] = stamp_lds[e >> 9][e & 511];                 \
  }
// ... 49 lines not shown
        }
      if (EPI == EPI_RESID_ACC && a.accum_in) {
        const __amdgpu_buffer_rsrc_t ra =
            __builtin_amdgcn_make_buffer_rsrc(const_cast<float*>(a.accum_in + (int64_t)b * a.y_bstride), 0, nrec, 0x00020000);
#pragma unroll
        for (int i = 0; i < WM; ++i) {
          float tmp[16][WN];
#pragma unroll
          for (int r = 0; r < 16; ++r) {
            const unsigned so = (unsigned)(i * 32 + (r & 3) + 8 * (r >> 2)) * rowT;
#pragma unroll
            for (int j = 0; j < WN; ++j)
              tmp[r][j] = __builtin_bit_cast(float, __builtin_amdgcn_raw_buffer_load_b32(ra, (int)vo[j], (int)so, 0));
          }
#pragma unroll
          for (int r = 0; r < 16; ++r)
#pragma unroll
            for (int j = 0; j < WN; ++j) acc[i][j][r] += tmp[r][j];
        }
      }
    } else if (EPI == EPI_RES_SKIP && full && a.split % 32 == 0) {
      const int64_t col_off = (int64_t)(4 * hl) * a.T + t0 + wn * 32 * WN + l31;
#pragma unroll
      for (int i = 0; i < WM; ++i) {
        const int trow = wrow0 + i * 32;
        const bool is_x = trow < a.split;
        const float* base = is_x ? a.y + (int64_t)b * a.y_bstride + (int64_t)trow * a.T
                                 : a.skip + ((int64_t)b * (a.M - a.split) + (trow - a.split)) * a.T;
        if (is_x || a.skip_accum) {
#pragma unroll
          for (int r = 0; r < 16; ++r) {
            const float* q = base + col_off + (int64_t)((r & 3) + 8 * (r >> 2)) * a.T;
#pragma unroll
            for (int j = 0; j < WN; ++j) acc[i][j][r] = q[j * 32];
          }
        } else {
#pragma unroll
          for (int r = 0; r < 16; ++r)
#pragma unroll
            for (int j = 0; j < WN; ++j) acc[i][j][r] = 0.f;
        }
      }
    } else if (EPI == EPI_COUPLE && full) {
      const float* py = a.y + (int64_t)b * a.y_bstride + lane_off;
#pragma unroll
      for (int i = 0; i < WM; ++i)
#pragma unroll
        for (int r = 0; r < 16; ++r) {
          const float* q = py + (int64_t)(i * 32 + (r & 3) + 8 * (r >> 2)) * a.T;
#pragma unroll
          for (int j = 0; j < WN; ++j) acc[i][j][r] = a.couple_sign * q[j * 32];
        }
    } else {
#pragma unroll
    for (int i = 0; i < WM; ++i)
#pragma unroll
      for (int r = 0; r < 16; ++r) {
        const int row = wrow0 + i * 32 + (r & 3) + 8 * (r >> 2) + 4 * hl;
#pragma unroll
        for (int j = 0; j < WN; ++j) {
          float v0 = 0.f;
          if constexpr (kInit) {
            const int t = t0 + wn * 32 * WN + j * 32 + l31;
            if (row < a.M && t < a.T) {
              if constexpr (EPI == EPI_RESID) {
                v0 = a.res[(int64_t)b * a.res_bstride + (int64_t)row * a.T + t];
              } else if constexpr (EPI == EPI_RESID_ACC) {
                v0 = a.res[(int64_t)b * a.res_bstride + (int64_t)row * a.T + t];
                if (a.accum_in) v0 += a.accum_in[(int64_t)b * a.y_bstride + (int64_t)row * a.T + t];
              } else if constexpr (EPI == EPI_RES_SKIP) {
                if (row < a.split) v0 = a.y[(int64_t)b * a.y_bstride + (int64_t)row * a.T + t];
                else if (a.skip_accum) v0 = a.skip[((int64_t)b * (a.M - a.split) + (row - a.split)) * a.T + t];
              } else {
                v0 = a.couple_sign * a.y[(int64_t)b * a.y_bstride + (int64_t)row * a.T + t];
              }
            }
          }
          acc[i][j][r] = v0;
        }
      }
    }
}

template <int WM, int WN, int CK, int NWN, int EPI, int PREC = 0, int NWM = 2, int VS = 0>
__global__ __launch_bounds__(64 * NWM * NWN, 2) void conv1d_mfma_kernel(const ConvArgs a, int tiles_x,
                                                                        int tiles_y, int total_tiles,
                                                                        int ksplit) {
  constexpr int NT = 64 * NWM * NWN;
  constexpr bool DB = NWN == 4;
  constexpr int BM = 32 * WM * NWM;
  constexpr int BN = 32 * WN * NWN;
  constexpr int G = CK / 8;
  extern __shared__ __attribute__((aligned(16))) float lds[];

  const int tid = threadIdx.x;
  const int lane = tid & 63;
#ifdef MBV_CONV_STAMPS
  int stamp_n = 0;
  __shared__ unsigned long long stamp_lds[2][512];
#endif
  const int wave = NWN == 2 ? __builtin_amdgcn_readfirstlane(tid >> 6) : tid >> 6;
  const int wm = wave / NWN, wn = wave % NWN;
  const int hl = lane >> 5, l31 = lane & 31;

  const int halo = (a.K - 1) * a.dil;
  const int XL = BN + halo;
  const int buf_f4 = G * 2 * XL + a.K * G * 2 * BM + 2 * BM;
  f32x4* const lds4 = reinterpret_cast<f32x4*>(lds);
  const int tin_eff = a.reflect1 ? a.Tin + 1 : a.Tin;

  constexpr int HALO_MAX = CK == 8 ? 72 : (CK == 16 ? 24 : 0);
  constexpr int KMAX = CK == 8 ? 11 : (CK == 16 ? 5 : 1);
  constexpr int NXP = (G * 2 * (BN + HALO_MAX) + NT - 1) / NT;
  constexpr int NW = (KMAX * G * 2 * BM + NT - 1) / NT;
  constexpr int RPI = NT / BM;
  constexpr int ROWS_PER_TAP = 2 * G;
  static_assert(RPI % ROWS_PER_TAP == 0 || ROWS_PER_TAP % RPI == 0, "weight-row decomposition");
  constexpr bool GLDS = DB && (CK <= MBV_CONV_GLDS || NWM == 1);
  f32x4 wreg[GLDS ? 1 : NW];
  f32x4 xreg[NXP];
  int xoff[NXP];
  const int totalW = a.K * ROWS_PER_TAP * BM;
  const int wq = tid % BM, wR0 = tid / BM;
  const int wtap0 = RPI >= ROWS_PER_TAP ? wR0 / ROWS_PER_TAP : 0;
  const int wrem0 = RPI >= ROWS_PER_TAP ? wR0 % ROWS_PER_TAP : wR0;
  const int64_t tap_stride = (int64_t)(a.Cin / 8) * 2 * a.Mpad * 4;

  int lb = 0, lm0 = 0, lt0 = 0;
  const float* wlane = nullptr;
  const float* xb = nullptr;

#define MBV_SETUP_TILE(TILE)                                                                 \
  {                                                                                          \
    const int tile_ = (TILE);                                                                \
    if (a.trim_map) {                     \
      const int ux_ = tile_ / tiles_y;                                                       \
      lb = a.trim_map[a.B + 1 + ux_]; lm0 = (tile_ % tiles_y) * BM; lt0 = (ux_ - a.trim_map[lb]) * BN; \
    } else {                                                                                 \
      const int tx_ = tile_ % tiles_x, rest_ = tile_ / tiles_x;                              \
      lb = rest_ / tiles_y; lm0 = (rest_ % tiles_y) * BM; lt0 = tx_ * BN;                    \
    }                                                                                        \
    wlane = (PREC == 3 ? a.w_split : a.w) + (int64_t)wtap0 * tap_stride + ((int64_t)wrem0 * a.Mpad + lm0 + wq) * 4; \
    xb = a.x + (int64_t)lb * a.x_bstride;                                                    \
    const int len_in_ = a.in_lens ? a.in_lens[lb] : 0x7fffffff;                              \
    int P = tid / XL, col = tid - P * XL;                                                    \
    _Pragma("unroll") for (int u = 0; u < NXP; ++u) {                                        \
      int off = -1;                                                                          \
      if (P < 2 * G) {                                                                       \
        int gi = lt0 - a.pad_left + col;                                                     \
        if constexpr (VS) {      \
          if (gi >= 0) {                                                                     \
            const int bq_ = gi / a.vs_tv, tq_ = gi - bq_ * a.vs_tv;                          \
            if (bq_ < a.B && tq_ < a.Tin && (!a.in_lens || tq_ < a.in_lens[bq_]))            \
              off = bq_ * (int)a.x_bstride + ((P >> 1) * 8 + (P & 1)) * a.x_rstride + tq_;   \
          }                                                                                  \
        } else                                                                               \
        if (gi >= 0 && gi < tin_eff) {                                                       \
          if (a.reflect1) gi = gi == 0 ? 1 : gi - 1;                                         \
          if (gi < len_in_) off = ((P >> 1) * 8 + (P & 1)) * a.x_rstride + gi;               \
        }                                                                                    \
      }                                                                                      \
      xoff[u] = off;                                                                         \
      col += NT;                                                                             \
      _Pragma("unroll") for (int w = 0; w < NT / 128; ++w)                                   \
        if (col >= XL) { col -= XL; ++P; }                                                   \
    }                                                                                        \
  }
#define MBV_ISSUE(CN)                                                                        \
  {                                                                                          \
    const int cn_ = (CN);                                                                    \
    const float* wchunk = wlane + (int64_t)(cn_ / 8) * 2 * a.Mpad * 4;                       \
    if constexpr (!GLDS) {                                                                   \
    _Pragma("unroll") for (int u = 0; u < NW; ++u) {                                         \
      int64_t off;                                                                           \
      if constexpr (RPI >= ROWS_PER_TAP) {                                                   \
        int tap = wtap0 + u * (RPI / ROWS_PER_TAP);     \
        tap = tap < a.K ? tap : a.K - 1;                                                     \
        off = (int64_t)(tap - wtap0) * tap_stride;                                           \
      } else {                                                                               \
        constexpr int PPT = ROWS_PER_TAP / RPI;                          \
        int tap = u / PPT;                                                 \
        tap = tap < a.K ? tap : a.K - 1;                                                     \
        off = tap * tap_stride + (int64_t)((u % PPT) * RPI) * a.Mpad * 4;                    \
      }                                                                                      \
      wreg[u] = *reinterpret_cast<const f32x4*>(wchunk + off);                               \
    }                                                                                        \
    }                                                                                        \
    const float* xchunk = xb + (int64_t)cn_ * a.x_rstride;                                   \
    const unsigned rs2 = 2u * (unsigned)a.x_rstride;                                         \
    _Pragma("unroll") for (int u = 0; u < NXP; ++u) {                                        \
      f32x4 v = {0.f, 0.f, 0.f, 0.f};                                                        \
      if (xoff[u] >= 0) {                                                                    \
        const unsigned o = (unsigned)xoff[u];                                                \
        v[0] = xchunk[o]; v[1] = xchunk[o + rs2]; v[2] = xchunk[o + 2 * rs2]; v[3] = xchunk[o + 3 * rs2]; \
      }                                                                                      \
      xreg[u] = v;                                                                           \
    }                                                                                        \
  }
#define MBV_COMMIT(CN, XS, WS)                                                               \
  {                                                                                          \
    const int cn_ = (CN);                                                                    \
    if constexpr (!GLDS) {                                                                   \
    _Pragma("unroll") for (int u = 0; u < NW; ++u) {                                         \
      const int e = tid + NT * u;                                                            \
      if (e < totalW) (WS)[e] = wreg[u];                        \
    }                                                                                        \
    }                                                                                        \
    int P = tid / XL, col = tid - P * XL;                                                    \
    _Pragma("unroll") for (int u = 0; u < NXP; ++u) {                                        \
      if (P < 2 * G) {                                                                       \
        f32x4 v = {0.f, 0.f, 0.f, 0.f};                                                      \
        if (xoff[u] >= 0) {                                                                  \
          v = xreg[u];                                                                       \
          if (a.chan_add) {                                                                  \
            const float* ca = a.chan_add + lb * a.Cin + cn_ + (P >> 1) * 8 + (P & 1);        \
            v[0] += ca[0]; v[1] += ca[2]; v[2] += ca[4]; v[3] += ca[6];                      \
          }                                                                                  \
          _Pragma("unroll") for (int s4 = 0; s4 < 4; ++s4) v[s4] = lrelu(v[s4], a.in_slope); \
        }                                                                                    \
        (XS)[P * XL + col] = PREC == 3 ? split_slot(v) : v;                                  \
      }                                                                                      \
      col += NT;                                                                             \
      _Pragma("unroll") for (int w = 0; w < NT / 128; ++w)                                   \
        if (col >= XL) { col -= XL; ++P; }                                                   \
    }                                                                                        \
  }

#define MBV_GLDS_W(CN, WS)                                                                   \
  {                                                                                          \
    const float* wchunk = wlane + (int64_t)((CN) / 8) * 2 * a.Mpad * 4;                      \
    const int wave_e0 = __builtin_amdgcn_readfirstlane(tid & ~63);                           \
    const unsigned lds0 = __builtin_amdgcn_readfirstlane(                                    \
        (unsigned)(size_t)(__attribute__((address_space(3))) void*)((WS) + wave_e0));        \
    _Pragma("unroll") for (int u = 0; u < NW; ++u) {                                         \
      int64_t off;                                                                           \
      if constexpr (RPI >= ROWS_PER_TAP) {                                                   \
        off = (int64_t)(u * (RPI / ROWS_PER_TAP)) * tap_stride;                              \
      } else {                                                                               \
        constexpr int PPT = ROWS_PER_TAP / RPI;                                              \
        off = (u / PPT) * tap_stride + (int64_t)((u % PPT) * RPI) * a.Mpad * 4;              \
      }                                                                                      \
      if (wave_e0 + NT * u < totalW) {                 \
        unsigned keep_m0;                                                                    \
        asm volatile("s_mov_b32 %0, m0\n\ts_mov_b32 m0, %2\n\ts_nop 0\n\t"                  \
                     "global_load_lds_dwordx4 %1, off\n\ts_mov_b32 m0, %0"                   \
                     : "=&s"(keep_m0) : "v"(wchunk + off), "s"(lds0 + (unsigned)(NT * u * 16)) : "memory"); \
      }                                                                                      \
    }                                                                                        \
  }
#define MBV_GLDS_DRAIN() asm volatile("s_waitcnt vmcnt(0)" ::: "memory")

  const int nck = a.Cin / CK;
  const int S = NWN == 2 ? ksplit : 1;
  if (a.trim_map) total_tiles = a.trim_map[a.B] * tiles_y;
  const int total_units = total_tiles * S;
  __shared__ int s_ticket;
  int s_unit = blockIdx.x;
  int s_c = (s_unit % S) * nck / S, s_end = (s_unit % S + 1) * nck / S;
  int pend_cn = -1;
#define MBV_ISSUE_NEXT()                                                                     \
  if (s_unit < total_units) {                                                                \
    const bool first_ = s_c == (s_unit % S) * nck / S;                                       \
    if (first_) MBV_SETUP_TILE(s_unit / S);                                                  \
    MBV_ISSUE(s_c * CK);                                                                     \
    pend_cn = s_c * CK;                                                                      \
    if (++s_c == s_end) {                                                                    \
      s_unit += gridDim.x;                                                                   \
      s_c = (s_unit % S) * nck / S;                                                          \
      s_end = (s_unit % S + 1) * nck / S;                                                    \
    }                                                                                        \
  }

  MBV_ISSUE_NEXT();
  {
    f32x4* const X0 = lds4;
    f32x4* const W0 = X0 + G * 2 * XL;
    if (pend_cn >= 0) {
      if constexpr (GLDS) { MBV_GLDS_W(pend_cn, W0); }
      MBV_COMMIT(pend_cn, X0, W0);
    }
    pend_cn = -1;
  }
  if constexpr (GLDS) { MBV_GLDS_DRAIN(); }
  __syncthreads();

  int q = 0;
  for (int unit = blockIdx.x; unit < total_units; unit += gridDim.x) {
    const int tile = unit / S, sp = unit % S;
    const int c_lo = sp * nck / S, c_hi = (sp + 1) * nck / S;
    int b, m0, t0;
    if (a.trim_map) {
      const int ux = tile / tiles_y;
      b = a.trim_map[a.B + 1 + ux]; m0 = (tile % tiles_y) * BM; t0 = (ux - a.trim_map[b]) * BN;
    } else {
      const int tx = tile % tiles_x, rest = tile / tiles_x;
      b = rest / tiles_y; m0 = (rest % tiles_y) * BM; t0 = tx * BN;
    }
    const int wrow0 = m0 + wm * 32 * WM;
    int nact = (a.M - wrow0 + 31) / 32;
    nact = nact < 0 ? 0 : (nact > WM ? WM : nact);
    int nj = ((VS ? a.B * a.vs_tv : a.T) - (t0 + wn * 32 * WN) + 31) / 32;
    nj = nj < 0 ? 0 : (nj > WN ? WN : nj);

    f32x16 acc[WM][WN];
    MBV_CSTAMP(1)
    float rowc = 0.f;
    {
      const int row = wrow0 + lane;
      if constexpr (EPI == EPI_GATE) {
        const int ch = (wrow0 >> 6) * 32 + l31;
        if (lane < 32 * WM && ch < a.gate_half) {
          const int idx = hl ? a.gate_half + ch : ch;
          rowc = a.bias ? a.bias[idx] : 0.f;
          if (a.gate_cond) rowc += a.gate_cond[(int64_t)b * a.gate_cond_bstride + idx];
        }
      } else if (lane < 32 * WM && row < a.M) {
        rowc = a.bias ? a.bias[row] : 0.f;
        if constexpr (EPI == EPI_RESID || EPI == EPI_RESID_ACC)
          if (a.res_chan_add) rowc += a.res_chan_add[b * a.M + row];
      }
    }
    const bool full = !VS && wrow0 + 32 * WM <= a.M && t0 + wn * 32 * WN + 32 * WN <= a.T;
    const int64_t lane_off = (int64_t)(wrow0 + 4 * hl) * a.T + t0 + wn * 32 * WN + l31;
    if (S == 1) {
      conv_acc_init<WM, WN, EPI>(acc, a, b, wrow0, t0, wn, hl, l31, full, lane_off);
    } else {
#pragma unroll
      for (int i = 0; i < WM; ++i)
#pragma unroll
        for (int j = 0; j < WN; ++j)
#pragma unroll
          for (int r = 0; r < 16; ++r) acc[i][j][r] = 0.f;
    }
    if constexpr (DB) { MBV_ISSUE_NEXT(); }
    if constexpr (EPI == EPI_RESID || EPI == EPI_RESID_ACC || EPI == EPI_RES_SKIP || EPI == EPI_COUPLE) {
#ifndef MBV_CONV_NO_ACC_PIN
#pragma unroll
      for (int i = 0; i < WM; ++i)
#pragma unroll
        for (int j = 0; j < WN; ++j) asm volatile("" : "+v"(acc[i][j]));
#endif
    }
    MBV_CSTAMP(2)

    for (int c = c_lo; c < c_hi; ++c, ++q) {
      f32x4* const Xs = lds4 + (DB ? ((q & 1) ? buf_f4 : 0) : 0);
      f32x4* const Ws = Xs + G * 2 * XL;
      f32x4* const Xn = lds4 + (DB ? ((q & 1) ? 0 : buf_f4) : 0);
      f32x4* const Wn = Xn + G * 2 * XL;
      if constexpr (!DB) { MBV_ISSUE_NEXT(); }
      if constexpr (GLDS) {
        if (pend_cn >= 0) { MBV_GLDS_W(pend_cn, Wn); }
      }

      MBV_CSTAMP(3)
      const int nsteps = a.K * G;
      const f32x4* wbase = Ws + hl * BM + wm * 32 * WM + l31;
      const f32x4* xbase = Xs + hl * XL + wn * 32 * WN + l31;
      if (nact == WM || (PREC == 3 && nact > 0)) {
        f32x4 a0[WM], b0[WN], a1[WM], b1[WN];
#define MBV_LOAD_AB(ST, AV, BV)                                                   \
        {                                                                          \
          const int st_ = (ST);                                                    \
          const int tap_ = st_ / G, g_ = st_ % G;                                  \
          const f32x4* wp_ = wbase + st_ * (2 * BM);                               \
          const f32x4* xp_ = xbase + g_ * (2 * XL) + tap_ * a.dil;                 \
          _Pragma("unroll") for (int i = 0; i < WM; ++i) AV[i] = wp_[i * 32];      \
          _Pragma("unroll") for (int j = 0; j < WN; ++j) BV[j] = xp_[j * 32];      \
        }
           \
#define MBV_SKIP(ST) (EPI == EPI_CONVT ? ((ST) / G == 0 ? 1 : ((ST) / G == a.K - 1 ? 0 : -1)) : -1)
#define MBV_MMA(AV, BV, SK, ALLJ)                                                  \
        {                                                                          \
          const int sk_ = (SK);                                                    \
          _Pragma("unroll") for (int s4 = 0; s4 < 4; ++s4)                         \
            _Pragma("unroll") for (int i = 0; i < WM; ++i)                         \
              _Pragma("unroll") for (int j = 0; j < WN; ++j)                       \
                if (((ALLJ) || j < nj) && (EPI != EPI_CONVT || i != sk_))          \
                  acc[i][j] = __builtin_amdgcn_mfma_f32_32x32x2f32(AV[i][s4], BV[j][s4], acc[i][j], 0, 0, 0);   \
        }
#define MBV_STEP_LOOP(ALLJ)                                                        \
        {                                                                          \
          MBV_LOAD_AB(0, a0, b0);                                                  \
          int st = 0;                                                              \
          for (; st + 1 < nsteps; st += 2) {                                       \
            MBV_LOAD_AB(st + 1, a1, b1);                                           \
            __builtin_amdgcn_sched_barrier(0);                                     \
            MBV_MMA(a0, b0, MBV_SKIP(st), ALLJ);                                   \
            __builtin_amdgcn_sched_barrier(0);                                     \
            MBV_LOAD_AB(st + 2, a0, b0);    \
            __builtin_amdgcn_sched_barrier(0);                                     \
            MBV_MMA(a1, b1, MBV_SKIP(st + 1), ALLJ);                               \
            __builtin_amdgcn_sched_barrier(0);                                     \
          }                                                                        \
          if (st < nsteps) { MBV_MMA(a0, b0, MBV_SKIP(st), ALLJ); }    \
        }
#define MBV_BF16_LOOP()                                                                                   \
        for (int st = 0; st < nsteps; st += 2) {                                                           \
          f32x4 ra0[WM], rb0[WN], ra1[WM], rb1[WN];                                                        \
          MBV_LOAD_AB(st, ra0, rb0);                                                                       \
          if (st + 1 < nsteps) {                                                                           \
            MBV_LOAD_AB(st + 1, ra1, rb1);                                                                 \
          } else {                                      \
            _Pragma("unroll") for (int i = 0; i < WM; ++i) ra1[i] = f32x4{0.f, 0.f, 0.f, 0.f};             \
            _Pragma("unroll") for (int j = 0; j < WN; ++j) rb1[j] = f32x4{0.f, 0.f, 0.f, 0.f};             \
          }                                                                                                \
// ... 131 lines not shown
      if constexpr (WM == 2) {
        if (nact == 2) {
          const int cbase = (wrow0 >> 6) * 32;
          float* yb = a.y + (int64_t)b * a.y_bstride;
#pragma unroll
          for (int r = 0; r < 16; ++r) {
            const int k = (r & 3) + 8 * (r >> 2) + 4 * hl;
            const float bt = __shfl(rowc, k), bs = __shfl(rowc, 32 + k);
            const int c = cbase + k;
            if (c >= a.gate_half) continue;
#pragma unroll
            for (int j = 0; j < WN; ++j) {
              const int t = t0 + wn * 32 * WN + j * 32 + l31;
              if (t < T) {
                const float vt = tanhf(acc[0][j][r] + bt);
                const float vs = sigmoidf_(acc[1][j][r] + bs);
                yb[(int64_t)c * T + t] = vt * vs;
              }
            }
          }
        }
      }
    } else if constexpr (EPI == EPI_CONVT) {
      if constexpr (WM == 2) {
        float* yb = a.y + (int64_t)b * a.y_bstride;
        if (a.convt_u == 4) {
          const int Tout = 4 * T;
          int64_t vs_o[VS ? WN : 1];
          bool vs_ok[VS ? WN : 1];
          if constexpr (VS) {
#pragma unroll
            for (int j = 0; j < WN; ++j) {
              const int tv = t0 + wn * 32 * WN + j * 32 + l31;
              const int bq = tv / a.vs_tv, tq = tv - bq * a.vs_tv;
              vs_ok[j] = bq < a.B && tq < T;
              vs_o[j] = (int64_t)bq * a.y_bstride + 4 * (int64_t)tq;
            }
          }
#pragma unroll
          for (int r = 0; r < 16; r += 2) {
            const int k = (r & 3) + 8 * (r >> 2) + 4 * hl;
            const float bias = __shfl(rowc, k);
            const int co = (wrow0 >> 6) * 16 + (k >> 1);
#pragma unroll
            for (int j = 0; j < WN; ++j) {
              const int t = t0 + wn * 32 * WN + j * 32 + l31;
              if constexpr (VS) {
                if (vs_ok[j]) {
                  f32x4 o = {acc[0][j][r] + bias, acc[0][j][r + 1] + bias, acc[1][j][r] + bias,
                             acc[1][j][r + 1] + bias};
                  *reinterpret_cast<f32x4*>(a.y + vs_o[j] + (int64_t)co * Tout) = o;
                }
              } else
              if (t < T) {
                f32x4 o = {acc[0][j][r] + bias, acc[0][j][r + 1] + bias, acc[1][j][r] + bias,
                           acc[1][j][r + 1] + bias};
                *reinterpret_cast<f32x4*>(yb + (int64_t)co * Tout + 4 * (int64_t)t) = o;
              }
            }
          }
        } else {
          const int Tout = 8 * T;
#pragma unroll
          for (int rg = 0; rg < 4; ++rg) {
            const int k = 8 * rg + 4 * hl;
            const float bias = __shfl(rowc, k);
            const int co = (wrow0 >> 6) * 8 + (k >> 2);
#pragma unroll
            for (int j = 0; j < WN; ++j) {
              const int t = t0 + wn * 32 * WN + j * 32 + l31;
              if (t < T) {
                float* dst = yb + (int64_t)co * Tout + 8 * (int64_t)t;
#pragma unroll
                for (int i = 0; i < 2; ++i) {
                  f32x4 o = {acc[i][j][4 * rg] + bias, acc[i][j][4 * rg + 1] + bias,
                             acc[i][j][4 * rg + 2] + bias, acc[i][j][4 * rg + 3] + bias};
                  *reinterpret_cast<f32x4*>(dst + 4 * i) = o;
                }
              }
            }
          }
        }
      }
    } else if ((EPI == EPI_STORE || EPI == EPI_RESID || EPI == EPI_RESID_ACC) && full && !a.out_lens) {
      float* py = a.y + (int64_t)b * a.y_bstride + lane_off;
#pragma unroll
      for (int i = 0; i < WM; ++i)
#pragma unroll
        for (int r = 0; r < 16; ++r) {
          const int k0 = i * 32 + (r & 3) + 8 * (r >> 2);
          const float bias = __shfl(rowc, k0 + 4 * hl);
          float* q = py + (int64_t)k0 * T;
#pragma unroll
          for (int j = 0; j < WN; ++j) {
            float v = acc[i][j][r] + bias;
            if constexpr (EPI == EPI_STORE) { if (a.relu) v = fmaxf(v, 0.f); }
            if constexpr (EPI == EPI_RESID_ACC) v *= a.out_scale;
            q[j * 32] = v;
          }
        }
    } else if (EPI == EPI_RES_SKIP && full && a.split % 32 == 0) {
      const int64_t col_off = (int64_t)(4 * hl) * T + t0 + wn * 32 * WN + l31;
#pragma unroll
      for (int i = 0; i < WM; ++i) {
        const int trow = wrow0 + i * 32;
        const bool is_x = trow < a.split;
        float* base = is_x ? a.y + (int64_t)b * a.y_bstride + (int64_t)trow * T
                           : a.skip + ((int64_t)b * (a.M - a.split) + (trow - a.split)) * T;
#pragma unroll
        for (int r = 0; r < 16; ++r) {
          const int k0 = (r & 3) + 8 * (r >> 2);
          const float bias = __shfl(rowc, i * 32 + k0 + 4 * hl);
          float* q = base + col_off + (int64_t)k0 * T;
#pragma unroll
          for (int j = 0; j < WN; ++j) {
            const int t = t0 + wn * 32 * WN + j * 32 + l31;
            float v = acc[i][j][r] + bias;
            if (is_x) v = t < len_out ? v : 0.f;
            q[j * 32] = v;
          }
        }
      }
    } else if (EPI == EPI_COUPLE && full) {
      float* py = a.y + (int64_t)b * a.y_bstride + lane_off;
#pragma unroll
      for (int i = 0; i < WM; ++i)
#pragma unroll
        for (int r = 0; r < 16; ++r) {
          const int k0 = i * 32 + (r & 3) + 8 * (r >> 2);
          const float bias = __shfl(rowc, k0 + 4 * hl);
          float* q = py + (int64_t)k0 * T;
#pragma unroll
          for (int j = 0; j < WN; ++j) {
            const int t = t0 + wn * 32 * WN + j * 32 + l31;
            const float v = a.couple_sign * (acc[i][j][r] + bias);
            q[j * 32] = t < len_out ? v : 0.f;
          }
        }
    } else {
#pragma unroll
      for (int i = 0; i < WM; ++i) {
#pragma unroll
        for (int r = 0; r < 16; ++r) {
          const int k = i * 32 + (r & 3) + 8 * (r >> 2) + 4 * hl;
          const float bias = __shfl(rowc, k);
          const int row = wrow0 + k;
          if (i >= nact || row >= a.M) continue;
#pragma unroll
          for (int j = 0; j < WN; ++j) {
            const int t = t0 + wn * 32 * WN + j * 32 + l31;
            if (t >= T) continue;
            float v = acc[i][j][r] + bias;
            const float mask = t < len_out ? 1.f : 0.f;
            const int64_t o = (int64_t)b * a.y_bstride + (int64_t)row * T + t;
            if constexpr (EPI == EPI_STORE) {
              if (a.relu) v = fmaxf(v, 0.f);
              if (a.out_lens) v *= mask;
              a.y[o] = v;
            } else if constexpr (EPI == EPI_RESID) {
              a.y[o] = v;
            } else if constexpr (EPI == EPI_RESID_ACC) {
              a.y[o] = v * a.out_scale;
            } else if constexpr (EPI == EPI_RES_SKIP) {
              if (row < a.split) a.y[o] = v * mask;
              else a.skip[((int64_t)b * (a.M - a.split) + (row - a.split)) * T + t] = v;
            } else if constexpr (EPI == EPI_COUPLE) {
              a.y[o] = a.couple_sign * v * mask;
            }
          }
        }
      }
    }
    MBV_CSTAMP(8)
  }
  MBV_CSTAMP_FLUSH()
#undef MBV_ISSUE_NEXT
#undef MBV_SETUP_TILE
#undef MBV_ISSUE
#undef MBV_COMMIT
#undef MBV_GLDS_W
#undef MBV_GLDS_DRAIN
}

constexpr int kSplitkTinyDiv = 16;
static int conv_splitk_factor(const ConvArgs& a, int BM, int BN, int CK, int NWN, int NT, long total, bool trimmed) {
  const long slots = 256L * (NT == 512 ? 1 : 2);
  int S = 1;
  const int nck = a.Cin / CK;
  const bool tiny = total * (long)kSplitkTinyDiv <= slots;
  const int min_chunks = tiny ? 2 : 4;
  if (NWN == 2 && a.splitk && a.ws_floats && a.n_counters && total * 4 <= slots && nck >= (tiny ? 4 : 16) &&
      total <= a.n_counters && !trimmed) {
    S = (int)(slots / total);
    if (S > nck / min_chunks) S = nck / min_chunks;
    if (S > 16) S = 16;
    while (S > 1 && (size_t)total * S * BM * BN > a.ws_floats) --S;
    if (S < 1) S = 1;
  }
  return S;
}

template <int WM, int WN, int CK, int NWN, int EPI, int PREC = 0, int NWM = 2, int VS = 0>
static void launch_epi(const ConvArgs& a, hipStream_t s) {
  constexpr int BM = 32 * WM * NWM, BN = 32 * WN * NWN, G = CK / 8, NT = 64 * NWM * NWN;
  const int XL = BN + (a.K - 1) * a.dil;
  const size_t buf_f4 = (size_t)G * 2 * XL + (size_t)a.K * G * 2 * BM + 2 * BM;
  const size_t lds_bytes = buf_f4 * 16 * (NWN == 4 ? 2 : 1);
  const int tiles_x = VS ? (int)(((long)a.B * a.vs_tv + BN - 1) / BN) : (a.T + BN - 1) / BN, tiles_y = (a.M + BM - 1) / BM;
  const long total = VS ? (long)tiles_x * tiles_y : (long)tiles_x * tiles_y * a.B;
  const long slots = 256L * (NT == 512 ? 1 : 2);
  const int S = conv_splitk_factor(a, BM, BN, CK, NWN, NT, total, a.trim_map != nullptr);
  if (a.trim_map && a.trim_bn != BN) {
    fprintf(stderr, "mbv: trimmed decode: tile map built for %d-column tiles, the launch uses %d\n", a.trim_bn, BN);
    abort();
  }
  const long units = total * S;
  const int grid = (int)(units > slots ? slots : units);
  static bool attr = false;
  if (!attr) {
    (void)hipFuncSetAttribute(reinterpret_cast<const void*>(&conv1d_mfma_kernel<WM, WN, CK, NWN, EPI, PREC, NWM, VS>),
                              hipFuncAttributeMaxDynamicSharedMemorySize,
#ifdef MBV_CONV_STAMPS
                              150 * 1024);
#else
                              160 * 1024 - 256);
#endif
    attr = true;
  }
  hipLaunchKernelGGL((conv1d_mfma_kernel<WM, WN, CK, NWN, EPI, PREC, NWM, VS>), dim3(grid), dim3(NT), lds_bytes, s, a,
                     tiles_x, tiles_y, (int)total, S);
}

template <int WM, int WN, int CK, int NWN>
static void launch_one(const ConvArgs& a, hipStream_t s) {
  if constexpr (WM == 2) {
    if (a.prec == 3) {
      if constexpr (CK <= 16) {
        switch (a.epi) {
          case EPI_STORE: launch_epi<WM, WN, CK, NWN, EPI_STORE, 3>(a, s); return;
          case EPI_RESID: launch_epi<WM, WN, CK, NWN, EPI_RESID, 3>(a, s); return;
          case EPI_RESID_ACC: launch_epi<WM, WN, CK, NWN, EPI_RESID_ACC, 3>(a, s); return;
          case EPI_CONVT:
            if constexpr (CK == 16) { launch_epi<WM, WN, CK, NWN, EPI_CONVT, 3>(a, s); return; }
            break;
          case EPI_GATE:
            if constexpr (CK == 16) { launch_epi<WM, WN, CK, NWN, EPI_GATE, 3>(a, s); return; }
            break;
          default: break;
        }
      } else {
        if (a.epi == EPI_RES_SKIP) { launch_epi<WM, WN, CK, NWN, EPI_RES_SKIP, 3>(a, s); return; }
      }
    }
  }
  switch (a.epi) {
    case EPI_STORE: launch_epi<WM, WN, CK, NWN, EPI_STORE>(a, s); break;
    case EPI_RESID: launch_epi<WM, WN, CK, NWN, EPI_RESID>(a, s); break;
    case EPI_RESID_ACC: launch_epi<WM, WN, CK, NWN, EPI_RESID_ACC>(a, s); break;
    case EPI_RES_SKIP: launch_epi<WM, WN, CK, NWN, EPI_RES_SKIP>(a, s); break;
    case EPI_COUPLE: launch_epi<WM, WN, CK, NWN, EPI_COUPLE>(a, s); break;
    case EPI_GATE:
      if constexpr (WM == 2) { launch_epi<WM, WN, CK, NWN, EPI_GATE>(a, s); break; }
    case EPI_CONVT:
      if constexpr (WM == 2 && CK == 16) {
        if (a.epi == EPI_CONVT) { launch_epi<WM, WN, CK, NWN, EPI_CONVT>(a, s); break; }
      }
    default:
      fprintf(stderr, "mbv: conv1d epilogue %d not built for this tile shape\n", a.epi);
      abort();
  }
}

bool conv1d_supported(int K, int dil) {
  return K >= 1 && K <= 11 && (K - 1) * dil <= 72;
}

template <int WM, int WN, int NWN>
static void launch_ck(const ConvArgs& a, hipStream_t s) {
  const int halo = (a.K - 1) * a.dil;
  if (!conv1d_supported(a.K, a.dil)) {
    fprintf(stderr, "mbv: conv1d kernel size %d / dilation %d outside the built range\n", a.K, a.dil);
    abort();
  }
  if (a.K == 1) launch_one<WM, WN, 32, NWN>(a, s);
  else if (a.K <= 5 && halo <= 24) launch_one<WM, WN, 16, NWN>(a, s);
  else launch_one<WM, WN, 8, NWN>(a, s);
}

constexpr int kNarrowMinUnits = 16;

ConvPlan conv1d_plan(const ConvArgs& a, bool trimmed, int route_T) {
  ConvPlan p{};
  p.S = 1;
  if (a.epi == EPI_LN) { p.route = CONV_NARROW_M; return p; }
  if (!trimmed && conv1d_narrow_supported(a)) {
    const long tiles128 = (long)((a.T + 127) / 128) * ((a.M + 127) / 128) * a.B;
    const long units32 = (((long)a.B * ((a.T + 15) / 16) + 1) / 2) * ((a.M + 127) / 128);
    if (a.splitk && tiles128 <= 128) {
      if (units32 >= kNarrowMinUnits) { p.route = CONV_NARROW_LAUNCH; return p; }
    } else if ((route_T > 0 ? route_T : a.T) <= 256) {
      p.route = CONV_NARROW_M;
      return p;
    }
  }
  const int halo = (a.K - 1) * a.dil;
  const int ck = a.K == 1 ? 32 : (a.K <= 5 && halo <= 24) ? 16 : 8;
  const bool wide_m = a.M > 64 || a.epi == EPI_GATE || a.epi == EPI_CONVT;
  bool big = false;
  int nb_big = 0;
  if (wide_m && a.T >= 384) {
    const double eff2 = 0.90 * a.T / (double)(((a.T + 127) / 128) * 128);
    const double eff3 = a.T / (double)(((a.T + 383) / 384) * 384);
    const long tpb3 = (long)((a.T + 383) / 384) * ((a.M + 127) / 128);
    const long tpb2 = (long)((a.T + 127) / 128) * ((a.M + 127) / 128);
    const long blocks3 = tpb3 * a.B;
    big = eff3 >= eff2 && blocks3 >= 512;
    if (!a.splitk && !trimmed && eff3 >= eff2 && blocks3 > 256 && a.B > 1) {
      const double c2 = 0.65;
      auto rounds = [](long n, long slots) { return (double)((n + slots - 1) / slots); };
      double best = big ? rounds(blocks3, 256) : rounds(tpb2 * a.B, 512) * c2;
      for (long k = blocks3 / 256; k >= 1; --k) {
        const long nb = 256 * k / tpb3;
        if (nb < 1 || nb >= a.B) continue;
        const double cost = rounds(nb * tpb3, 256) + rounds((a.B - nb) * tpb2, 512) * c2;
        if (cost < 0.9 * best) { best = cost / 0.9; nb_big = (int)nb; }
      }
    }
  }
  auto shape = [&](int route, int bm, int bn, int threads, int ck_) {
    p.route = route; p.bm = bm; p.bn = bn; p.threads = threads; p.ck = ck_;
  };
  if (a.epi == EPI_CONVT && a.convt_u == 4 && a.prec != 3 && !a.splitk && !trimmed && !a.chan_add &&
      !a.reflect1 && a.B > 1 && a.K > 1 && a.K <= 5 && halo <= 24 && a.T >= 128 &&
      (int64_t)a.B * a.x_bstride < (1ll << 31)) {
    auto rounds = [](long n, long slots) { return (double)((n + slots - 1) / slots); };
    const long tiles_y = (a.M + 127) / 128;
    const long tv = a.T + halo;
    const double cost_vs = rounds(((long)a.B * tv + 383) / 384 * tiles_y, 256);
    double cur;
    if (nb_big > 0) {
      const long tpb3 = (long)((a.T + 383) / 384) * tiles_y, tpb2 = (long)((a.T + 127) / 128) * tiles_y;
      cur = rounds(nb_big * tpb3, 256) + rounds((a.B - nb_big) * tpb2, 512) * 0.65;
    } else if (big) {
      cur = rounds((long)((a.T + 383) / 384) * tiles_y * a.B, 256);
    } else {
      cur = rounds((long)((a.T + 127) / 128) * tiles_y * a.B, 512) * 0.65;
    }
    if (cost_vs >= 2.0 && cost_vs < 0.95 * cur) {
      shape(CONV_VS, 128, 384, 512, 16);
      p.vs_tv = (int)tv;
      return p;
    }
  }
  if (nb_big > 0) {
    shape(CONV_SPLIT_BATCH, 128, 384, 512, ck);
    p.nb_big = nb_big;
    return p;
  }
  if (wide_m) {
    if (big) shape(CONV_BIG, 128, 384, 512, ck);
    else shape(CONV_SMALL, 128, 128, 256, ck);
  } else {
    if (a.T >= 384 && a.K > 1 && a.prec != 3 && !a.splitk && !trimmed &&
        (a.epi == EPI_STORE || a.epi == EPI_RESID || a.epi == EPI_RESID_ACC) &&
        (long)((a.T + 383) / 384) * a.B >= 512 && a.T / (double)(((a.T + 383) / 384) * 384) >= 0.90 * a.T / (double)(((a.T + 127) / 128) * 128)) {
      shape(CONV_HALF, 64, 384, 256, a.K <= 5 && halo <= 24 ? 16 : 8);
      return p;
    }
    shape(CONV_M64, 64, 128, 256, ck);
  }
  const long total = (long)((a.T + p.bn - 1) / p.bn) * ((a.M + p.bm - 1) / p.bm) * a.B;
  p.S = conv_splitk_factor(a, p.bm, p.bn, p.ck, p.bn == 384 ? 4 : 2, p.threads, total, trimmed);
  return p;
}

int conv1d_trim_bn(const ConvArgs& a) {
  if (a.epi == EPI_LN || a.splitk) return 0;
  const int r = conv1d_plan(a, false).route;
  if (r == CONV_NARROW_M || r == CONV_NARROW_LAUNCH) return 0;
  return conv1d_plan(a, true).bn;
}

void launch_conv1d(const ConvArgs& a, hipStream_t s, int route_T) {
  if ((a.epi == EPI_RESID || a.epi == EPI_RESID_ACC) && (unsigned long long)a.M * a.T * 4ull >= (1ull << 32)) {
    fprintf(stderr, "mbv: conv1d: one utterance's [%d x %d] output exceeds 4 GiB\n", a.M, a.T);
    abort();
  }
  if (a.epi == EPI_LN && !conv1d_narrow_supported(a)) { fprintf(stderr, "mbv: EPI_LN outside the narrow kernel's range\n"); abort(); }
  const ConvPlan p = conv1d_plan(a, a.trim_map != nullptr, route_T);
  switch (p.route) {
    case CONV_NARROW_M: launch_conv1d_narrow(a, false, s); return;
    case CONV_NARROW_LAUNCH: launch_conv1d_narrow(a, true, s); return;
    case CONV_VS: {
      ConvArgs av = a;
      av.vs_tv = p.vs_tv;
      launch_epi<2, 3, 16, 4, EPI_CONVT, 0, 2, 1>(av, s);
      return;
    }
    case CONV_SPLIT_BATCH: {
      ConvArgs a1 = a, a2 = a;
      const int nb = p.nb_big;
      a1.B = nb;
      a2.B = a.B - nb;
      a2.x += (int64_t)nb * a.x_bstride;
      a2.y += (int64_t)nb * a.y_bstride;
      if (a.in_lens) a2.in_lens += nb;
      if (a.out_lens) a2.out_lens += nb;
      if (a.chan_add) a2.chan_add += (int64_t)nb * a.Cin;
      if (a.res) a2.res += (int64_t)nb * a.res_bstride;
      if (a.res_chan_add) a2.res_chan_add += (int64_t)nb * a.M;
      if (a.accum_in) a2.accum_in += (int64_t)nb * a.y_bstride;
      if (a.gate_cond) a2.gate_cond += (int64_t)nb * a.gate_cond_bstride;
      if (a.skip) a2.skip += (int64_t)nb * (a.M - a.split) * a.T;
      launch_ck<2, 3, 4>(a1, s);
      launch_ck<2, 2, 2>(a2, s);
      return;
    }
    case CONV_BIG: launch_ck<2, 3, 4>(a, s); return;
    case CONV_SMALL: launch_ck<2, 2, 2>(a, s); return;
    case CONV_HALF:
      if (p.ck == 16) {
        switch (a.epi) {
          case EPI_STORE: launch_epi<2, 3, 16, 4, EPI_STORE, 0, 1>(a, s); return;
          case EPI_RESID: launch_epi<2, 3, 16, 4, EPI_RESID, 0, 1>(a, s); return;
          default: launch_epi<2, 3, 16, 4, EPI_RESID_ACC, 0, 1>(a, s); return;
        }
      }
      switch (a.epi) {
        case EPI_STORE: launch_epi<2, 3, 8, 4, EPI_STORE, 0, 1>(a, s); return;
        case EPI_RESID: launch_epi<2, 3, 8, 4, EPI_RESID, 0, 1>(a, s); return;
        default: launch_epi<2, 3, 8, 4, EPI_RESID_ACC, 0, 1>(a, s); return;
      }
    default: launch_ck<1, 2, 2>(a, s); return;
  }
}

}
```

### mb-istft-vits_amd/csrc/kernels.h

```cpp
#pragma once
#include <hip/hip_runtime.h>
#include <stdint.h>

#include <vector>

namespace mbv {

template <typename Row, int N>
struct RowsArg { Row row[N]; };
struct NoExtra {
  template <typename Row>
  __device__ void operator()(int, const Row&) const {}
};
template <typename Row, int N, typename Extra>
__global__ void rows_kernel(const RowsArg<Row, N> r, int n, int first, Row* __restrict__ dst, const Extra extra) {
  const int i = threadIdx.x;
  if (i >= n) return;
  dst[first + i] = r.row[i];
  extra(first + i, r.row[i]);
}
template <int N, typename Row, typename Fill, typename Extra = NoExtra>
void upload_rows(size_t n, Row* dst, hipStream_t s, Fill fill, Extra extra = Extra{}) {
  static_assert(sizeof(RowsArg<Row, N>) + 64 <= 4096, "kernel arguments stay under 4 KiB per launch");
  for (size_t f = 0; f < n; f += N) {
    RowsArg<Row, N> r{};
    const int nn = (int)(n - f < (size_t)N ? n - f : (size_t)N);
    for (int i = 0; i < nn; ++i) r.row[i] = fill(f + i);
    hipLaunchKernelGGL((rows_kernel<Row, N, Extra>), dim3(1), dim3(N), 0, s, r, nn, (int)f, dst, extra);
  }
}

enum ConvEpilogue : int {
  EPI_STORE = 0,
  EPI_RESID = 1,
  EPI_RESID_ACC = 2,
  EPI_GATE = 3,
  EPI_RES_SKIP = 4,
  EPI_COUPLE = 5,
  EPI_CONVT = 6,
  EPI_LN = 7,
};

struct ConvArgs {
  const float* x;
  int64_t x_bstride;
  int Tin;
  int x_rstride;
  int Cin;
  const float* w;
  const float* bias;
  int M;
  int Mpad;
  int K;
  int dil;
  int pad_left;
  float in_slope;
  const int* in_lens;
  const float* chan_add;
  int reflect1;
  float* y;
  int64_t y_bstride;
  int T;
  int epi;
  int relu;
  const int* out_lens;
  const float* res;
  int64_t res_bstride;
  const float* res_chan_add;
  const float* accum_in;
  float out_scale;
  const float* gate_cond;
  int gate_cond_bstride;
  int gate_half;
  float* skip;
  int split;
  int skip_accum;
  float couple_sign;
  int B;
  const int* trim_map;
  int trim_bn;
  int vs_tv;
  float* ws;
  size_t ws_floats;
  unsigned* counters;
  int n_counters;
  int convt_u;
  int splitk;
  int prec;
  const float* w_split;
  const float* ln_gamma;
  const float* ln_beta;
  const int* ln_out_lens;
};
enum ConvRoute : int {
  CONV_NARROW_M = 1,
  CONV_NARROW_LAUNCH = 2,
  CONV_M64 = 3,
  CONV_HALF = 4,
  CONV_SMALL = 5,
  CONV_BIG = 6,
  CONV_SPLIT_BATCH = 7,
  CONV_VS = 8,
};
struct ConvPlan {
  int route;
  int bm, bn, threads, ck;
  int nb_big;
  int vs_tv;
  int S;
};
ConvPlan conv1d_plan(const ConvArgs& a, bool trimmed, int route_T = 0);
inline ConvPlan conv1d_plan(const ConvArgs& a) { return conv1d_plan(a, a.trim_map != nullptr); }
void launch_conv1d(const ConvArgs& a, hipStream_t s, int route_T = 0);
bool conv1d_supported(int K, int dil);
bool conv1d_narrow_supported(const ConvArgs& a);
void launch_conv1d_narrow(const ConvArgs& a, bool by_launch_size, hipStream_t s);

struct WnLayerArgs {
  const float* h_in;
  float* h_out;
  float* skip;
  const int* lens;
  const int* ustart;
  const int* hmap;
  const float* wg; const float* bg;
  const float* gcond;
  int gcond_bstride;
  const float* wr; const float* br;
  int B, H, T;
  int Mg_pad;
  int Mr, Mr_pad;
  int last;
  int skip_accum;
  int Gi;
  int in_cb;
  const float* wpre;
  int wpre_Mpad;
  int Cs;
  float* x1;
  int64_t x1_bstride;
  float couple_sign;
};
bool wn_fused_supported(int H, int K);
bool wn_fused_fits(int B, int H, int T);
bool wn_prefold_fits(int H, int I);
bool wn_postfold_fits(int H, int I);
size_t wn_units_ints(int B, int T);
void launch_wn_units(const int* lens, int B, int T, int* ustart, int* hmap, hipStream_t s);
void launch_wn_layer(const WnLayerArgs& a, hipStream_t s);

void launch_embed(const int64_t* ids, const int64_t* lens, const float* emb, float* x, int* lens32,
                  int* bad, int B, int T, int H, int n_vocab, hipStream_t s);
void launch_split_planes(const float* src, float* dst, size_t n_floats, hipStream_t s);
void launch_layernorm(const float* a, const float* r, const float* gamma, const float* beta,
                      float* y, int B, int C, int T, int pre_relu, const int* out_lens,
                      hipStream_t s);
void launch_rel_attention(const float* qkv, const float* emb_k, const float* emb_v,
                          const int* lens, float* o, int B, int H, int n_heads, int T,
                          hipStream_t s);

void launch_durations(const float* h, const float* w, const float* b, const int* lens,
                      float length_scale, float* logw, float* w_ceil, int* cum, int* ylen32,
                      int64_t* ylen64, const int* bad, int B, int C, int T, hipStream_t s);
struct FitOut { float scale; int32_t status; };
struct ShapeRow {
  const float* scale;
  const int* extra;
  FitOut* fit_out;
  int64_t frames;
  float lo, hi, scalar;
  int32_t row, t_text, pad_;
};
constexpr int kShapeChunk = 64;
void launch_shape_durations(const float* logw, const int* lens, const float* scale, const int* extra, float scalar,
                            const ShapeRow* fit, float* w_ceil, int* cum, int* ylen32, int64_t* ylen64, const int* bad,
                            float* fit_stage, FitOut* fit_out, int B, int T, hipStream_t s);
void launch_shape_durations_rows(const float* logw, const int* lens, const ShapeRow* rows, int n, float* w_ceil,
                                 int* cum, int* ylen32, int64_t* ylen64, const int* bad, int T, hipStream_t s);
struct MarkRow {
  int64_t* dst;
  int32_t count, pad_;
};
void launch_token_marks(const int* cum, int B, int T, int64_t* dst, int64_t stride, int count, const MarkRow* rows,
                        hipStream_t s);
struct GainRow {
// ... 219 lines not shown
constexpr int kWaveAlaw = 9;
struct ResampleRangeRow {
  const void* x;
  int32_t dtype;
  int32_t closed;
  int64_t n;
  int64_t out_first, out_end;
  float* out;
};
int64_t resample_ready_open(const ResampleGeom& g, int64_t in_avail);
void launch_resample_ranges(const ResampleRangeRow* rows, int n, int64_t max_count, const float* bank,
                            const ResampleGeom& g, hipStream_t s);

void resample_window(int filter, std::vector<double>* win, int* num_zeros, int* nb);

constexpr float kPitchMin = 0.5f, kPitchMax = 2.0f;
constexpr int kWarpTile = 256;
constexpr int kWarpWindow = 776;
int64_t warp_plan(int hop, int64_t F, const float* R, double* U, int64_t* n_out);
int warp_half_width(int num_zeros, int64_t F, const float* R);
int64_t warp_ready(int hop, int64_t F, const float* R, const double* U, int num_zeros, int64_t in_avail);
struct WarpRow {
  const float* x;
  int64_t n, in_avail;
  const double* U;
  const float* R;
  int32_t F, hop;
  PcmEnv env;
  int64_t out_first, out_end;
  float* out;
  const float* win;
  int32_t num_zeros, hw;
};
void launch_warp_ranges(const WarpRow* rows, int n, int64_t max_count, hipStream_t s);

constexpr size_t kSpectrogramMaxLds = 80 * 1024;
int64_t spectrogram_frames(int64_t n, int n_fft, int hop);
size_t spectrogram_lds_bytes(int n_fft, int hop, int FB);
int spectrogram_block_frames(int n_fft, int hop);
void spectrogram_tables(int n_fft, int win, std::vector<float>* tw, std::vector<float>* window);
void launch_spectrogram(const void* x, int dtype, const int64_t* valid, int B, int64_t in_stride, int n_fft, int hop,
                        const float* tw, const float* win, float* spec, int64_t F, int64_t* spec_lengths,
                        hipStream_t s);

void launch_neg_cent(const float* z_p, const float* m_p, const float* logs_p, int64_t p_bstride, const int* t_ys,
                     const int* t_xs, float* value, int B, int I, int Tt, int Ts, hipStream_t s);
constexpr int kMaxPathMaxTs = 1024;
constexpr size_t kMaxPathLdsBytes = 64 * 1024;
bool max_path_supported(int Ts);
size_t max_path_lds_bytes(int Tt, int Ts);
size_t max_path_scratch_bytes(int B, int Tt, int Ts);
void launch_max_path(const float* value, const int* t_ys, const int* t_xs, int* w, int* path, int* status,
                     void* bits_scratch, int B, int Tt, int Ts, hipStream_t s);
void launch_set_durations(const void* w, int dtype, const int* lens, float* w_ceil, int* cum, int* ylen32,
                          int64_t* ylen64, const int* bad, int B, int T, hipStream_t s);
void launch_align_status(const int* bad_x, const int* bad_y, const int* mas, int* status, float* w_f, const int* w_i,
                         int B, int T, hipStream_t s);

void launch_posterior_sample(const float* stats, const float* noise, const int* lens, float* z, int B,
                             int I, int T, hipStream_t s, float noise_scale = 1.f);

struct ConvertRow {
  const void* wave;
  int64_t samples;
  int dtype, frames;
  int sid_src, sid_tgt;
  int first, reserved;
};
struct ConvertRowCols {
  int* lens; int64_t* sid_src; int64_t* sid_tgt;
  __device__ void operator()(int i, const ConvertRow& k) const { lens[i] = k.frames; sid_src[i] = k.sid_src; sid_tgt[i] = k.sid_tgt; }
};
void launch_spectrogram_rows(const ConvertRow* rows, int B, int n_fft, int hop, const float* tw, const float* win,
                             float* dst, int cpad, int64_t F, hipStream_t s);
void launch_posterior_sample_rows(const float* stats, const AdmitSynRow* rows, const int* lens, float* z, int B,
                                  int I, int T, hipStream_t s);
void launch_sequence_mask(const int* lens, float* mask, int B, int T, hipStream_t s);
void launch_lens_to_i32(const int64_t* lens, int* out, int B, int T, int* bad, hipStream_t s);

void launch_fill(float* p, float v, int64_t n, hipStream_t s);
size_t launch_trim_map_ints(int B, int T, int BN);
void launch_trim_map(const int* lens, int B, int num, int add, int T, int BN, int* out, hipStream_t s);
constexpr int kTailMapJobs = 24;
struct TailMapJob { int num, reach, T, BN; int* out; };
struct TailMapJobs { TailMapJob job[kTailMapJobs]; };
size_t launch_tail_map_ints(int B, int T, int BN);
void launch_tail_maps(const int* lens, int B, const TailMapJobs& jobs, int n, unsigned long long* dropped, hipStream_t s);
void launch_tail_fill(float* y, int64_t y_bstride, int B, int M, int T, int BN, const int* map, hipStream_t s);
constexpr int kRaggedChunk = 256;
struct RaggedRowsArg { int row[kRaggedChunk]; int len[kRaggedChunk]; };
void launch_ragged_rows(const RaggedRowsArg& r, int n, int first, int us, int* out, int stride, hipStream_t s);
void launch_gather_frames(const float* src, int64_t src_bstride, int src_rstride, const int* rows, const int* lens,
                          int n, int C, int T, float* dst, hipStream_t s);
constexpr int kPoolChunk = 64;
struct PoolRowLens {
  int* lens; int stride, us;
  __device__ void operator()(int i, const PoolRow& k) const {
    lens[i] = k.len; lens[stride + i] = us * k.len; lens[2 * stride + i] = us * us * k.len;
  }
};
void launch_gather_windows(const PoolRow* rows, int n, int C, int T, float* dst, int gin, float* gdst, hipStream_t s);
int conv1d_trim_bn(const ConvArgs& a);

struct RandnRow {
  float* dst;
  int64_t stride, begin;
  uint32_t seed_lo, seed_hi, purpose, row;
  int32_t first, count, quads, reserved;
};
constexpr int kRandnChunk = 64;
void launch_randn_blocks(const RandnRow* rows, int n, int64_t total, hipStream_t s);
void randn_host(uint64_t seed, uint32_t purpose, uint32_t row, uint32_t c, int64_t first, int64_t count, float* dst);

struct LoudnessParams {
  double coef[10];
  double M[16];
  double z_abs;
  int32_t H, pad_;
};
void kweighting_host(int rate, LoudnessParams* p);
struct LoudnessRow {
  const float* x;
  const int64_t* valid;
  int64_t avail;
  int64_t k0, k1;
  double* state;
  double* energy;
  float* L;
};
constexpr int kLoudnessChunk = 32;
void launch_loudness(const LoudnessRow* rows, int n, const LoudnessParams& p, hipStream_t s);

}
```

### mb-istft-vits_amd/csrc/ops.hip

```cpp
#include "kernels.h"

namespace mbv {

__global__ void embed_kernel(const int64_t* ids, const int64_t* lens, const float* emb, float* x,
                             int* lens32, int* bad, int B, int T, int H, int n_vocab, float scale) {
  const int b = blockIdx.z;
  const int c = blockIdx.y;
  const int t = blockIdx.x * blockDim.x + threadIdx.x;
  if (t == 0 && c == 0) {
    const long long l = lens[b];
    lens32[b] = l < 0 ? 0 : (l > T ? T : (int)l);
    if (l < 0 || l > T) bad[b] = 1;
  }
  if (t >= T) return;
  const int len = (int)lens[b];
  long long id = ids[(int64_t)b * T + t];
  if (id < 0 || id >= n_vocab) {
    if (c == 0) bad[b] = 1;
    id = 0;
  }
  float v = emb[id * H + c] * scale;
  x[((int64_t)b * H + c) * T + t] = t < len ? v : 0.f;
}

// ... 631 lines not shown
  hipLaunchKernelGGL(posterior_sample_kernel<true>, grid, dim3(128), 0, s, stats, nullptr, lens, z, I, T, 0.f, rows);
}

__global__ void sequence_mask_kernel(const int* lens, float* mask, int T) {
  const int b = blockIdx.y;
  const int t = blockIdx.x * blockDim.x + threadIdx.x;
  if (t < T) mask[(int64_t)b * T + t] = t < lens[b] ? 1.f : 0.f;
}

void launch_sequence_mask(const int* lens, float* mask, int B, int T, hipStream_t s) {
  hipLaunchKernelGGL(sequence_mask_kernel, dim3((T + 255) / 256, B), dim3(256), 0, s, lens, mask, T);
}

__global__ void lens_to_i32_kernel(const int64_t* lens, int* out, int B, int T, int* bad) {
  const int b = blockIdx.x * blockDim.x + threadIdx.x;
  if (b >= B) return;
  const long long l = lens[b];
  out[b] = l < 0 ? 0 : (l > T ? T : (int)l);
  bad[b] = (l < 0 || l > T) ? 1 : 0;
}

void launch_lens_to_i32(const int64_t* lens, int* out, int B, int T, int* bad, hipStream_t s) {
  hipLaunchKernelGGL(lens_to_i32_kernel, dim3((B + 63) / 64), dim3(64), 0, s, lens, out, B, T, bad);
}

__global__ void fill_kernel(float* p, float v, int64_t n) {
  int64_t i = (int64_t)blockIdx.x * blockDim.x + threadIdx.x;
  const int64_t stride = (int64_t)gridDim.x * blockDim.x;
  for (; i < n; i += stride) p[i] = v;
}

__global__ void trim_map_kernel(const int* __restrict__ lens, int B, int num, int add, int T, int BN, int* __restrict__ out) {
  __shared__ int part[256];
  const int tid = threadIdx.x;
  const int per = (B + 255) / 256;
  auto tiles_of = [&](int b) {
    long lim = (long)lens[b] * num + add;
    lim = lim < 0 ? 0 : (lim > T ? T : lim);
    return (int)((lim + BN - 1) / BN);
  };
  int s = 0;
  for (int i = 0; i < per; ++i) { const int b = tid * per + i; if (b < B) s += tiles_of(b); }
  part[tid] = s;
  __syncthreads();
  if (tid == 0) { int run = 0; for (int i = 0; i < 256; ++i) { const int v = part[i]; part[i] = run; run += v; } }
  __syncthreads();
  int run = part[tid];
  for (int i = 0; i < per; ++i) {
    const int b = tid * per + i;
    if (b < B) {
      out[b] = run;
      const int n = tiles_of(b);
      for (int k = 0; k < n; ++k) out[B + 1 + run + k] = b;
      run += n;
      if (b == B - 1) out[B] = run;
    }
  }
}
size_t launch_trim_map_ints(int B, int T, int BN) { return (size_t)B + 1 + (size_t)B * ((T + BN - 1) / BN); }
void launch_trim_map(const int* lens, int B, int num, int add, int T, int BN, int* out, hipStream_t s) {
  hipLaunchKernelGGL(trim_map_kernel, dim3(1), dim3(256), 0, s, lens, B, num, add, T, BN, out);
}

__global__ void tail_map_kernel(const int* __restrict__ lens, int B, const TailMapJobs jobs, unsigned long long* __restrict__ dropped) {
  __shared__ int part[256];
  __shared__ int part_b[256];
  const TailMapJob jb = jobs.job[blockIdx.x];
  const int num = jb.num, reach = jb.reach, T = jb.T, BN = jb.BN;
  int* const out = jb.out;
  const int tid = threadIdx.x;
  const int per = (B + 255) / 256;
  int best = 0x7fffffff, best_b = 0x7fffffff;
  for (int i = 0; i < per; ++i) { const int b = tid * per + i; if (b < B && lens[b] < best) { best = lens[b]; best_b = b; } }
  part[tid] = best; part_b[tid] = best_b;
  __syncthreads();
  if (tid == 0) {
    for (int i = 1; i < 256; ++i) if (part[i] < best) { best = part[i]; best_b = part_b[i]; }
    part_b[0] = best_b;
  }
  __syncthreads();
  const int donor = part_b[0];
  __syncthreads();
  const int full = (T + BN - 1) / BN;
  auto tiles_of = [&](int b) {
    if (b == donor) return full;
    long lim = (long)lens[b] * num + reach;
    lim = lim < 0 ? 0 : (lim > T ? T : lim);
    return (int)((lim + BN - 1) / BN);
  };
  int s = 0;
  for (int i = 0; i < per; ++i) { const int b = tid * per + i; if (b < B) s += tiles_of(b); }
  part[tid] = s;
  __syncthreads();
  if (tid == 0) { int run = 0; for (int i = 0; i < 256; ++i) { const int v = part[i]; part[i] = run; run += v; } }
  __syncthreads();
  int run = part[tid];
  for (int i = 0; i < per; ++i) {
    const int b = tid * per + i;
    if (b < B) {
      out[b] = run;
      const int n = tiles_of(b);
      for (int k = 0; k < n; ++k) out[B + 1 + run + k] = b;
      run += n;
      if (b == B - 1) {
        out[B] = run;
        out[B + 1 + (long)B * full] = donor;
        if (dropped) atomicAdd(dropped, (unsigned long long)((long)B * full - run));
      }
    }
  }
}
size_t launch_tail_map_ints(int B, int T, int BN) { return launch_trim_map_ints(B, T, BN) + 1; }
void launch_tail_maps(const int* lens, int B, const TailMapJobs& jobs, int n, unsigned long long* dropped, hipStream_t s) {
  if (n <= 0) return;
  hipLaunchKernelGGL(tail_map_kernel, dim3(n), dim3(256), 0, s, lens, B, jobs, dropped);
}

template <bool VEC>
__global__ void tail_fill_kernel(float* __restrict__ y, int64_t y_bstride, int B, int T, int BN, const int* __restrict__ map) {
  const int m = blockIdx.x, b = blockIdx.y;
  const int full = (T + BN - 1) / BN;
  const int donor = map[B + 1 + (long)B * full];
  if (b == donor) return;
  const long c0 = (long)(map[b + 1] - map[b]) * BN;
  if (c0 >= T) return;
  const float* src = y + (int64_t)donor * y_bstride + (int64_t)m * T;
  float* dst = y + (int64_t)b * y_bstride + (int64_t)m * T;
  if constexpr (VEC) {
    for (long c = c0 + 4 * threadIdx.x; c < T; c += 4 * blockDim.x)
      *reinterpret_cast<float4*>(dst + c) = *reinterpret_cast<const float4*>(src + c);
  } else {
    for (long c = c0 + threadIdx.x; c < T; c += blockDim.x) dst[c] = src[c];
  }
}
void launch_tail_fill(float* y, int64_t y_bstride, int B, int M, int T, int BN, const int* map, hipStream_t s) {
  const bool vec = T % 4 == 0 && y_bstride % 4 == 0 && BN % 4 == 0 && (reinterpret_cast<uintptr_t>(y) & 15) == 0;
  if (vec) hipLaunchKernelGGL(tail_fill_kernel<true>, dim3(M, B), dim3(256), 0, s, y, y_bstride, B, T, BN, map);
  else hipLaunchKernelGGL(tail_fill_kernel<false>, dim3(M, B), dim3(256), 0, s, y, y_bstride, B, T, BN, map);
}

__global__ void ragged_rows_kernel(const RaggedRowsArg r, int n, int first, int us, int* __restrict__ out, int stride) {
  const int i = threadIdx.x;
  if (i >= n) return;
  const int len = r.len[i];
  out[first + i] = r.row[i];
  out[stride + first + i] = len;
  out[2 * stride + first + i] = us * len;
  out[3 * stride + first + i] = us * us * len;
}

void launch_ragged_rows(const RaggedRowsArg& r, int n, int first, int us, int* out, int stride, hipStream_t s) {
  hipLaunchKernelGGL(ragged_rows_kernel, dim3(1), dim3(kRaggedChunk), 0, s, r, n, first, us, out, stride);
}

__global__ void gather_frames_kernel(const float* __restrict__ src, int64_t src_bstride, int src_rstride,
                                     const int* __restrict__ rows, const int* __restrict__ lens, int C, int T,
                                     float* __restrict__ dst) {
  const int i = blockIdx.z, c = blockIdx.y;
  const int t = blockIdx.x * blockDim.x + threadIdx.x;
  const int len = lens ? lens[i] : T;
  if (t < T && t < len)
    dst[((int64_t)i * C + c) * T + t] = src[rows[i] * src_bstride + (int64_t)c * src_rstride + t];
}

void launch_gather_frames(const float* src, int64_t src_bstride, int src_rstride, const int* rows, const int* lens,
                          int n, int C, int T, float* dst, hipStream_t s) {
  const int nt = T >= 256 ? 256 : 64;
  hipLaunchKernelGGL(gather_frames_kernel, dim3((T + nt - 1) / nt, C, n), dim3(nt), 0, s, src, src_bstride,
                     src_rstride, rows, lens, C, T, dst);
}

__global__ void gather_windows_kernel(const PoolRow* __restrict__ rows, int C, int T, float* __restrict__ dst, int gin,
                                      float* __restrict__ gdst) {
  const int i = blockIdx.z, c = blockIdx.y;
  const int t = blockIdx.x * blockDim.x + threadIdx.x;
  const PoolRow r = rows[i];
  if (c == C) {
    for (int k = t; k < gin; k += gridDim.x * blockDim.x) gdst[(int64_t)i * gin + k] = r.g[k];
    return;
  }
  if (t < T && t < r.len) dst[((int64_t)i * C + c) * T + t] = r.z[(int64_t)c * r.z_stride + r.wa + t];
}

void launch_gather_windows(const PoolRow* rows, int n, int C, int T, float* dst, int gin, float* gdst, hipStream_t s) {
  const int nt = T >= 256 ? 256 : 64;
  hipLaunchKernelGGL(gather_windows_kernel, dim3((T + nt - 1) / nt, C + (gin > 0 ? 1 : 0), n), dim3(nt), 0, s, rows, C, T,
                     dst, gin, gdst);
}

void launch_fill(float* p, float v, int64_t n, hipStream_t s) {
  int blocks = (int)((n + 255) / 256);
  if (blocks > 4096) blocks = 4096;
  if (blocks < 1) blocks = 1;
  hipLaunchKernelGGL(fill_kernel, dim3(blocks), dim3(256), 0, s, p, v, n);
}

}
```

Baseline: 178.5 million samples/s.

## Add packed-tail conv route that concatenates trimmed utterance columns across the batch

```diff
diff --git a/include/mbistft_vits.h b/include/mbistft_vits.h
--- a/include/mbistft_vits.h
+++ b/include/mbistft_vits.h
@@ -103,6 +103,8 @@
 int mbv_decode_masked(mbv_model *m, const float *z, const float *g, const int32_t *lengths, int B, int t_frames,
                       const mbv_outputs *outs, void *stream);
 int64_t mbv_tail_dropped(mbv_model *m);
+int mbv_tail_pack_table(const int64_t *lens, int B, int num, int reach, int T, int halo, int pad_right, int bn,
+                        int32_t *out, int64_t capacity);
 
 typedef struct mbv_enc_row {
   float length_scale, noise_scale_w;
@@ -479,6 +481,7 @@
 #define MBV_ROUTE_BIG 6
 #define MBV_ROUTE_SPLIT_BATCH 7
 #define MBV_ROUTE_VS 8
+#define MBV_ROUTE_TAIL_PACK 9
 int mbv_op_conv(mbv_model *m, const mbv_conv_desc *d, const float *x, const float *w_host, const float *bias_host,
                 float *y, int32_t *plan_out, void *stream);
 int mbv_conv_plan(const mbv_conv_desc *d, int32_t out[8]);
diff --git a/mb-istft-vits_amd/_capi.py b/mb-istft-vits_amd/_capi.py
--- a/mb-istft-vits_amd/_capi.py
+++ b/mb-istft-vits_amd/_capi.py
@@ -23,7 +23,7 @@
     "mbv_op_sdp_logw", "mbv_op_sdp_noise", "mbv_op_chan_add", "mbv_op_istft_single",
     "mbv_align", "mbv_set_durations", "mbv_op_neg_cent", "mbv_op_max_path",
     "mbv_admit_plan", "mbv_encode_rows", "mbv_synthesize_rows", "mbv_encoder_runs", "mbv_get_option",
-    "mbv_tail_plan", "mbv_tail_dropped", "mbv_decode_masked",
+    "mbv_tail_plan", "mbv_tail_dropped", "mbv_decode_masked", "mbv_tail_pack_table",
     "mbv_convert_plan", "mbv_convert_rows", "mbv_converter_runs",
     "mbv_decode_chunks_routed", "mbv_converter_context", "mbv_spectrogram_ready", "mbv_convert_window",
     "mbv_convert_ranges_plan", "mbv_convert_ranges",
@@ -231,7 +231,8 @@
 
 CONV_KIND_CONV, CONV_KIND_CONVT4, CONV_KIND_CONVT8 = 0, 4, 8
 CONV_EPI_STORE, CONV_EPI_RESID, CONV_EPI_RESID_ACC, CONV_EPI_LN = 0, 1, 2, 7
-ROUTES = {1: "NARROW_M", 2: "NARROW_LAUNCH", 3: "M64", 4: "HALF", 5: "SMALL", 6: "BIG", 7: "SPLIT_BATCH", 8: "VS"}
+ROUTES = {1: "NARROW_M", 2: "NARROW_LAUNCH", 3: "M64", 4: "HALF", 5: "SMALL", 6: "BIG", 7: "SPLIT_BATCH", 8: "VS",
+          9: "TAIL_PACK"}
 PLAN_FIELDS = ("route", "bm", "bn", "threads", "ck", "nb_big", "vs_tv", "S")
 
 
@@ -352,7 +353,7 @@
                 "mbv_resample_turns_shaped",
                 "mbv_warp_plan", "mbv_warp_ready", "mbv_warp_ranges", "mbv_warp_runs",
                 "mbv_speakers_define", "mbv_speaker_release", "mbv_speaker_slots", "mbv_speaker_defined",
-                "mbv_speaker_runs") if os.environ.get("MBV_LIB") else ()
+                "mbv_speaker_runs", "mbv_tail_pack_table") if os.environ.get("MBV_LIB") else ()
     if hasattr(L, "mbv_ragged_classes") or not optional:
         L.mbv_ragged_classes.argtypes = [C.POINTER(MbvConfig), i32, i32, C.POINTER(C.c_int32), i32]
         L.mbv_ragged_plan.argtypes = [C.POINTER(MbvConfig), i32, i32, i32, i64p, C.POINTER(C.c_int32)]
@@ -381,6 +382,8 @@
         L.mbv_tail_dropped.argtypes = [vp]
         L.mbv_tail_dropped.restype = C.c_int64
         L.mbv_decode_masked.argtypes = [vp, vp, vp, vp, i32, i32, C.POINTER(MbvOutputs), vp]
+    if hasattr(L, "mbv_tail_pack_table") or not optional:
+        L.mbv_tail_pack_table.argtypes = [i64p, i32, i32, i32, i32, i32, i32, i32, C.POINTER(C.c_int32), C.c_int64]
     if hasattr(L, "mbv_convert_rows") or not optional:
         L.mbv_convert_plan.argtypes = [C.POINTER(MbvConfig), i32, i32, C.POINTER(C.c_int32), C.POINTER(C.c_int32)]
         L.mbv_convert_rows.argtypes = [vp, C.POINTER(MbvConvertRow), i32, i32, i32, i32, vp, vp]
diff --git a/mb-istft-vits_amd/csrc/capi.hip b/mb-istft-vits_amd/csrc/capi.hip
--- a/mb-istft-vits_amd/csrc/capi.hip
+++ b/mb-istft-vits_amd/csrc/capi.hip
@@ -992,6 +992,8 @@
 
 int tail_mode(const mbv_model* m) { return (!m->trim && !m->splitk && m->conv_bf16 != 3) ? m->tail_once : 0; }
 bool tail_stage(int mode, int B, long conv_tiles) { return B > 1 && (mode == 2 || (mode == 1 && conv_tiles > 256)); }
+constexpr int kTailPackMaxTiles = 8;
+bool tail_pack_stage(int Lo, int bn) { return (Lo + bn - 1) / bn <= kTailPackMaxTiles; }
 
 bool decoder_stage_concurrent(const mbv_model* m, int B, int ch, int Lo, bool tail = false) {
   const long conv_tiles = (long)B * ((Lo + 383) / 384) * ((ch + 127) / 128);
@@ -1161,7 +1163,7 @@
   struct TrimMap { int num, add, T, bn; int* map; bool built; };
   TrimMap trim_maps[12]; int n_trim;
   int trim_of[48];
-  struct TailMap { int kind, j, q, bn; const int* map; };
+  struct TailMap { int kind, j, q, bn; const int* map; int pack_blocks; };
   struct Stage { float *u, *t1s[3], *rs[3], *xs, *cb[3]; bool conc; int n_tail; TailMap tail_maps[kTailMapJobs]; TailMapJobs jobs; } st[2];
   int Bc;
   float *xpost, *otmp;
@@ -1197,8 +1199,16 @@
         const ConvArgs a = planned(e);
         const int bn = conv1d_trim_bn(a);
         if (!bn || conv1d_plan(a, false).route != conv1d_plan(a, true).route) continue;
+        ConvArgs ap = a;
+        ap.tail_pack = 1;
+        if (tail_pack_stage(Lo, bn) && conv1d_plan(ap, true).route == CONV_TAIL_PACK) {
+          const int halo = (a.K - 1) * a.dil, gap = tail_pack_gap(halo);
+          st.jobs.job[st.n_tail] = {e.rate, tail_plan[n_e].reach, Lo, bn, nullptr, gap, halo - a.pad_left};
+          st.tail_maps[st.n_tail++] = {e.kind, e.j, e.q, bn, nullptr, tail_pack_blocks(B, Lo, gap, bn)};
+          continue;
+        }
         st.jobs.job[st.n_tail] = {e.rate, tail_plan[n_e].reach, Lo, bn, nullptr};
-        st.tail_maps[st.n_tail++] = {e.kind, e.j, e.q, bn, nullptr};
+        st.tail_maps[st.n_tail++] = {e.kind, e.j, e.q, bn, nullptr, 0};
       }
     st.conc = decoder_stage_concurrent(m, B, ch, Lo, st.n_tail > 0) && !d.trim;
     st.u = sc.take<float>(n);
@@ -1231,7 +1241,9 @@
   }
   for (auto& st : d.st)
     for (int i = 0; i < st.n_tail; ++i)
-      st.tail_maps[i].map = st.jobs.job[i].out = sc.take<int>(launch_tail_map_ints(B, st.jobs.job[i].T, st.jobs.job[i].BN));
+      st.tail_maps[i].map = st.jobs.job[i].out = sc.take<int>(
+          st.jobs.job[i].pack_gap ? tail_pack_ints(B, st.jobs.job[i].T, st.jobs.job[i].pack_gap, st.jobs.job[i].BN)
+                                  : launch_tail_map_ints(B, st.jobs.job[i].T, st.jobs.job[i].BN));
   d.xpost = sc.take<float>((size_t)d.Bc * (utt_bytes / 4));
   if (k.own_o) d.otmp = sc.take<float>((size_t)B * table.back().rate * Td);
 }
@@ -1297,6 +1309,11 @@
       const DecBufs::TailMap& t = tail_stage_bufs->tail_maps[n_t];
       if (t.kind != e.kind || t.j != e.j || t.q != e.q) continue;
       if (conv1d_trim_bn(a) != t.bn) { tail_drift = true; return nullptr; }
+      if (t.pack_blocks) {
+        a.tail_pack = 1; a.pack_tbl = t.map; a.pack_blocks = t.pack_blocks;
+        if (conv1d_plan(a, true, rt_num * e.num).route != CONV_TAIL_PACK) { tail_drift = true; return nullptr; }
+        return &t;
+      }
       a.trim_map = t.map; a.trim_bn = t.bn;
       return &t;
     }
@@ -1369,7 +1386,7 @@
         with_trim(a, e);
         const DecBufs::TailMap* tm = with_tail(a, e);
         launch_conv1d(a, s, rt_num * e.num);
-        if (tm) launch_tail_fill(a.y, a.y_bstride, B, a.M, a.T, tm->bn, tm->map, s);
+        if (tm) launch_tail_fill(a.y, a.y_bstride, B, a.M, a.T, tm->bn, tm->map, s, tm->pack_blocks > 0);
         if (conc && e.epi == EPI_RESID_ACC) HIPCHK(m, hipEventRecord(m->ev_rb[j], s));
         if (!first) state = r;
       }
@@ -4938,7 +4955,8 @@
 namespace {
 static_assert(MBV_ROUTE_NARROW_M == CONV_NARROW_M && MBV_ROUTE_NARROW_LAUNCH == CONV_NARROW_LAUNCH &&
               MBV_ROUTE_M64 == CONV_M64 && MBV_ROUTE_HALF == CONV_HALF && MBV_ROUTE_SMALL == CONV_SMALL &&
-              MBV_ROUTE_BIG == CONV_BIG && MBV_ROUTE_SPLIT_BATCH == CONV_SPLIT_BATCH && MBV_ROUTE_VS == CONV_VS,
+              MBV_ROUTE_BIG == CONV_BIG && MBV_ROUTE_SPLIT_BATCH == CONV_SPLIT_BATCH && MBV_ROUTE_VS == CONV_VS &&
+              MBV_ROUTE_TAIL_PACK == CONV_TAIL_PACK,
               "route numbers of the C-ABI and the launcher");
 static_assert(MBV_CONV_EPI_LN == EPI_LN, "epilogue numbers of the C-ABI and the launcher");
 
@@ -4963,6 +4981,7 @@
   if (d.epi != MBV_CONV_EPI_RESID_ACC && d.accum_in) return "accum_in belongs to RESID_ACC";
   if (d.legacy_convt) return "legacy_convt must be 0 (the stand-alone ConvTranspose kernel was removed)";
   if (d.trim_lens && d.splitk) return "a trimmed launch takes no split-K";
+  if (d.tail_once < 0 || d.tail_once > 2) return "tail_once must be 0, 1 or 2";
   if (d.tail_once && (!d.trim_lens || convt || ln)) return "tail_once needs trim_lens and a conv with a STORE / RESID / RESID_ACC epilogue";
   const int U = d.kind;
   if (convt) {
@@ -4993,6 +5012,7 @@
   a.B = d.B;
   a.splitk = d.splitk != 0;
   a.prec = d.prec;
+  a.tail_pack = d.tail_once == 2;
   if ((a.epi == EPI_RESID || a.epi == EPI_RESID_ACC) && (unsigned long long)a.M * a.T * 4ull >= (1ull << 32))
     return "one utterance's output exceeds 4 GiB";
   if (ln) {
@@ -5100,12 +5120,23 @@
     mem.p.push_back(map);
     if (d->tail_once) {
       if (d->B > 65535) return m->fail("mbv_op_conv: tail_once takes at most 65535 rows");
+      const bool packed = p.route == CONV_TAIL_PACK;
+      const int halo = (a.K - 1) * a.dil, gap = tail_pack_gap(halo);
       void* tmap = nullptr;
-      HIPCHK(m, hipMalloc(&tmap, launch_tail_map_ints(d->B, a.T, p.bn) * sizeof(int)));
+      HIPCHK(m, hipMalloc(&tmap, (packed ? tail_pack_ints(d->B, a.T, gap, p.bn) : launch_tail_map_ints(d->B, a.T, p.bn)) * sizeof(int)));
       mem.p.push_back(tmap);
       TailMapJobs jobs{};
-      jobs.job[0] = {d->trim_num, d->trim_add, a.T, p.bn, (int*)tmap};
+      jobs.job[0] = {d->trim_num, d->trim_add, a.T, p.bn, (int*)tmap, packed ? gap : 0, packed ? halo - a.pad_left : 0};
       launch_tail_maps((const int*)dl, d->B, jobs, 1, m->tail_cnt, s);
+      if (packed) {
+        a.pack_tbl = (const int*)tmap; a.pack_blocks = tail_pack_blocks(d->B, a.T, gap, p.bn);
+        launch_conv1d(a, s);
+        launch_tail_fill(a.y, a.y_bstride, a.B, a.M, a.T, p.bn, a.pack_tbl, s, true);
+        HIPCHK(m, hipGetLastError());
+        HIPCHK(m, hipStreamSynchronize(s));
+        if (plan_out) plan_ints(p, plan_out);
+        return 0;
+      }
       map = tmap;
     } else {
       launch_trim_map((const int*)dl, d->B, d->trim_num, d->trim_add, a.T, p.bn, (int*)map, s);
@@ -5120,4 +5151,26 @@
   return 0;
 }
 
-}
+int mbv_tail_pack_table(const int64_t* lens, int B, int num, int reach, int T, int halo, int pad_right, int bn,
+                        int32_t* out, int64_t capacity) {
+  if (!lens || B <= 0 || T <= 0 || halo < 0 || pad_right < 0 || pad_right > halo || bn < 32 || bn % 32) return -1;
+  const int gap = tail_pack_gap(halo);
+  const int64_t n = (int64_t)tail_pack_ints(B, T, gap, bn);
+  if (!out) return n > 0x7fffffff ? -1 : (int)n;
+  if (capacity < n || n > 0x7fffffff) return -1;
+  auto len_of = [&](int b) { return lens[b] < 0 ? 0 : (lens[b] > T ? (int64_t)T : lens[b]); };
+  int donor = 0;
+  for (int b = 1; b < B; ++b) if (len_of(b) < len_of(donor)) donor = b;
+  int run = 0;
+  for (int b = 0; b < B; ++b) {
+    const int sp = tail_pack_sp(len_of(b), num, reach, T, b == donor);
+    out[kTailPackHdr + b] = sp;
+    tail_pack_row(out, B, b, run, sp, gap, pad_right);
+    run += tail_pack_row_blocks(sp, gap);
+  }
+  for (int i = kTailPackHdr + B; i < tail_pack_entries_at(B); ++i) out[i] = 0;
+  tail_pack_finish(out, B, T, gap, bn, donor, run);
+  return (int)n;
+}
+
+}
diff --git a/mb-istft-vits_amd/csrc/conv1d.hip b/mb-istft-vits_amd/csrc/conv1d.hip
--- a/mb-istft-vits_amd/csrc/conv1d.hip
+++ b/mb-istft-vits_amd/csrc/conv1d.hip
@@ -155,6 +155,61 @@
     }
 }
 
+template <int WM, int WN, int EPI>
+__device__ __forceinline__ void conv_acc_init_packed(f32x16 (&acc)[WM][WN], const ConvArgs& a, const int4* pack_ent,
+                                                     int wrow0, int t0, int wn, int hl, int l31) {
+  if constexpr (EPI == EPI_RESID || EPI == EPI_RESID_ACC) {
+    const __amdgpu_buffer_rsrc_t rr = __builtin_amdgcn_make_buffer_rsrc(
+        const_cast<float*>(a.res), 0, (unsigned)((unsigned long long)a.B * a.res_bstride * 4ull), 0x00020000);
+    unsigned vo[WN], va[WN];
+#pragma unroll
+    for (int j = 0; j < WN; ++j) {
+      const int4 e = pack_ent[(t0 >> 5) + wn * WN + j];
+      const int t = e.y + l31;
+      const bool ok = e.w && t < a.T;
+      const unsigned in_row = (unsigned)((wrow0 + 4 * hl) * a.T + t);
+      vo[j] = ok ? ((unsigned)e.x * (unsigned)a.res_bstride + in_row) * 4u : 0x7fffffffu;
+      va[j] = ok ? ((unsigned)e.x * (unsigned)a.y_bstride + in_row) * 4u : 0x7fffffffu;
+    }
+    const unsigned rowT = (unsigned)a.T * 4u;
+#pragma unroll
+    for (int i = 0; i < WM; ++i)
+#pragma unroll
+      for (int r = 0; r < 16; ++r) {
+        const unsigned so = (unsigned)(i * 32 + (r & 3) + 8 * (r >> 2)) * rowT;
+#pragma unroll
+        for (int j = 0; j < WN; ++j)
+          acc[i][j][r] = __builtin_bit_cast(float, __builtin_amdgcn_raw_buffer_load_b32(rr, (int)vo[j], (int)so, 0));
+      }
+    if (EPI == EPI_RESID_ACC && a.accum_in) {
+      const __amdgpu_buffer_rsrc_t ra = __builtin_amdgcn_make_buffer_rsrc(
+          const_cast<float*>(a.accum_in), 0, (unsigned)((unsigned long long)a.B * a.y_bstride * 4ull), 0x00020000);
+#pragma unroll
+      for (int i = 0; i < WM; ++i) {
+        float tmp[16][WN];
+#pragma unroll
+        for (int r = 0; r < 16; ++r) {
+          const unsigned so = (unsigned)(i * 32 + (r & 3) + 8 * (r >> 2)) * rowT;
+#pragma unroll
+          for (int j = 0; j < WN; ++j)
+            tmp[r][j] = __builtin_bit_cast(float, __builtin_amdgcn_raw_buffer_load_b32(ra, (int)va[j], (int)so, 0));
+        }
+#pragma unroll
+        for (int r = 0; r < 16; ++r)
+#pragma unroll
+          for (int j = 0; j < WN; ++j) acc[i][j][r] += tmp[r][j];
+      }
+    }
+  } else {
+#pragma unroll
+    for (int i = 0; i < WM; ++i)
+#pragma unroll
+      for (int j = 0; j < WN; ++j)
+#pragma unroll
+        for (int r = 0; r < 16; ++r) acc[i][j][r] = 0.f;
+  }
+}
+
 template <int WM, int WN, int CK, int NWN, int EPI, int PREC = 0, int NWM = 2, int VS = 0>
 __global__ __launch_bounds__(64 * NWM * NWN, 2) void conv1d_mfma_kernel(const ConvArgs a, int tiles_x,
                                                                         int tiles_y, int total_tiles,
@@ -181,6 +236,7 @@
   const int buf_f4 = G * 2 * XL + a.K * G * 2 * BM + 2 * BM;
   f32x4* const lds4 = reinterpret_cast<f32x4*>(lds);
   const int tin_eff = a.reflect1 ? a.Tin + 1 : a.Tin;
+  const int4* const pack_ent = VS == 2 ? reinterpret_cast<const int4*>(a.pack_tbl + tail_pack_entries_at(a.B)) : nullptr;
 
   constexpr int HALO_MAX = CK == 8 ? 72 : (CK == 16 ? 24 : 0);
   constexpr int KMAX = CK == 8 ? 11 : (CK == 16 ? 5 : 1);
@@ -206,6 +262,9 @@
 #define MBV_SETUP_TILE(TILE)                                                                 \
   {                                                                                          \
     const int tile_ = (TILE);                                                                \
+    if constexpr (VS == 2) {           \
+      lb = 0; lm0 = (tile_ % tiles_y) * BM; lt0 = (tile_ / tiles_y) * BN;                    \
+    } else                                                                                   \
     if (a.trim_map) {                     \
       const int ux_ = tile_ / tiles_y;                                                       \
       lb = a.trim_map[a.B + 1 + ux_]; lm0 = (tile_ % tiles_y) * BM; lt0 = (ux_ - a.trim_map[lb]) * BN; \
@@ -221,8 +280,16 @@
       int off = -1;                                                                          \
       if (P < 2 * G) {                                                                       \
         int gi = lt0 - a.pad_left + col;                                                     \
-        if constexpr (VS) {      \
-          if (gi >= 0) {                                                                     \
+        if constexpr (VS == 2) {  \
+          if (gi >= 0 && (gi >> 5) < a.pack_blocks) {                                        \
+            const int4 e_ = pack_ent[gi >> 5];                                               \
+            const int cq_ = e_.y + (gi & 31);                                                \
+            if (cq_ < e_.z && cq_ < a.Tin)                                                   \
+              off = e_.x * (int)a.x_bstride + ((P >> 1) * 8 + (P & 1)) * a.x_rstride + cq_;  \
+          }                                                                                  \
+        } else                                                                               \
+        if constexpr (VS == 1) {  \
+          if (gi >= 0) {                                                                  \
             const int bq_ = gi / a.vs_tv, tq_ = gi - bq_ * a.vs_tv;                          \
             if (bq_ < a.B && tq_ < a.Tin && (!a.in_lens || tq_ < a.in_lens[bq_]))            \
               off = bq_ * (int)a.x_bstride + ((P >> 1) * 8 + (P & 1)) * a.x_rstride + tq_;   \
@@ -326,6 +393,7 @@
   const int nck = a.Cin / CK;
   const int S = NWN == 2 ? ksplit : 1;
   if (a.trim_map) total_tiles = a.trim_map[a.B] * tiles_y;
+  if constexpr (VS == 2) total_tiles = a.pack_tbl[0] * tiles_y;
   const int total_units = total_tiles * S;
   __shared__ int s_ticket;
   int s_unit = blockIdx.x;
@@ -362,6 +430,9 @@
     const int tile = unit / S, sp = unit % S;
     const int c_lo = sp * nck / S, c_hi = (sp + 1) * nck / S;
     int b, m0, t0;
+    if constexpr (VS == 2) {
+      b = 0; m0 = (tile % tiles_y) * BM; t0 = (tile / tiles_y) * BN;
+    } else
     if (a.trim_map) {
       const int ux = tile / tiles_y;
       b = a.trim_map[a.B + 1 + ux]; m0 = (tile % tiles_y) * BM; t0 = (ux - a.trim_map[b]) * BN;
@@ -374,6 +445,7 @@
     nact = nact < 0 ? 0 : (nact > WM ? WM : nact);
     int nj = ((VS ? a.B * a.vs_tv : a.T) - (t0 + wn * 32 * WN) + 31) / 32;
     nj = nj < 0 ? 0 : (nj > WN ? WN : nj);
+    if constexpr (VS == 2) nj = WN;
 
     f32x16 acc[WM][WN];
     MBV_CSTAMP(1)
@@ -395,6 +467,9 @@
     }
     const bool full = !VS && wrow0 + 32 * WM <= a.M && t0 + wn * 32 * WN + 32 * WN <= a.T;
     const int64_t lane_off = (int64_t)(wrow0 + 4 * hl) * a.T + t0 + wn * 32 * WN + l31;
+    if constexpr (VS == 2) {
+      conv_acc_init_packed<WM, WN, EPI>(acc, a, pack_ent, wrow0, t0, wn, hl, l31);
+    } else
     if (S == 1) {
       conv_acc_init<WM, WN, EPI>(acc, a, b, wrow0, t0, wn, hl, l31, full, lane_off);
     } else {
@@ -692,6 +767,50 @@
           }
         }
       }
+    } else if constexpr (VS == 2) {
+      int64_t po[WN];
+      bool pok[WN];
+      int whole = 1;
+#pragma unroll
+      for (int j = 0; j < WN; ++j) {
+        const int4 e = pack_ent[(t0 >> 5) + wn * WN + j];
+        pok[j] = e.w && e.y + l31 < T;
+        whole &= (e.w && e.y + 32 <= T) ? 1 : 0;
+        po[j] = (int64_t)e.x * a.y_bstride + (int64_t)(wrow0 + 4 * hl) * T + e.y + l31;
+      }
+      if (__builtin_amdgcn_readfirstlane(whole)) {
+#pragma unroll
+        for (int i = 0; i < WM; ++i)
+#pragma unroll
+          for (int r = 0; r < 16; ++r) {
+            const int k0 = i * 32 + (r & 3) + 8 * (r >> 2);
+            const float bias = __shfl(rowc, k0 + 4 * hl);
+            float* q = a.y + (int64_t)k0 * T;
+#pragma unroll
+            for (int j = 0; j < WN; ++j) {
+              float v = acc[i][j][r] + bias;
+              if constexpr (EPI == EPI_STORE) { if (a.relu) v = fmaxf(v, 0.f); }
+              if constexpr (EPI == EPI_RESID_ACC) v *= a.out_scale;
+              q[po[j]] = v;
+            }
+          }
+      } else {
+#pragma unroll
+        for (int i = 0; i < WM; ++i)
+#pragma unroll
+          for (int r = 0; r < 16; ++r) {
+            const int k0 = i * 32 + (r & 3) + 8 * (r >> 2);
+            const float bias = __shfl(rowc, k0 + 4 * hl);
+            float* q = a.y + (int64_t)k0 * T;
+#pragma unroll
+            for (int j = 0; j < WN; ++j) {
+              float v = acc[i][j][r] + bias;
+              if constexpr (EPI == EPI_STORE) { if (a.relu) v = fmaxf(v, 0.f); }
+              if constexpr (EPI == EPI_RESID_ACC) v *= a.out_scale;
+              if (pok[j]) q[po[j]] = v;
+            }
+          }
+      }
     } else if ((EPI == EPI_STORE || EPI == EPI_RESID || EPI == EPI_RESID_ACC) && full && !a.out_lens) {
       float* py = a.y + (int64_t)b * a.y_bstride + lane_off;
 #pragma unroll
@@ -816,7 +935,8 @@
   const int XL = BN + (a.K - 1) * a.dil;
   const size_t buf_f4 = (size_t)G * 2 * XL + (size_t)a.K * G * 2 * BM + 2 * BM;
   const size_t lds_bytes = buf_f4 * 16 * (NWN == 4 ? 2 : 1);
-  const int tiles_x = VS ? (int)(((long)a.B * a.vs_tv + BN - 1) / BN) : (a.T + BN - 1) / BN, tiles_y = (a.M + BM - 1) / BM;
+  const int tiles_x = VS == 2 ? a.pack_blocks / (BN / 32) - 1 : VS ? (int)(((long)a.B * a.vs_tv + BN - 1) / BN) : (a.T + BN - 1) / BN;
+  const int tiles_y = (a.M + BM - 1) / BM;
   const long total = VS ? (long)tiles_x * tiles_y : (long)tiles_x * tiles_y * a.B;
   const long slots = 256L * (NT == 512 ? 1 : 2);
   const int S = conv_splitk_factor(a, BM, BN, CK, NWN, NT, total, a.trim_map != nullptr);
@@ -902,6 +1022,7 @@
 ConvPlan conv1d_plan(const ConvArgs& a, bool trimmed, int route_T) {
   ConvPlan p{};
   p.S = 1;
+  if (a.tail_pack) trimmed = true;
   if (a.epi == EPI_LN) { p.route = CONV_NARROW_M; return p; }
   if (!trimmed && conv1d_narrow_supported(a)) {
     const long tiles128 = (long)((a.T + 127) / 128) * ((a.M + 127) / 128) * a.B;
@@ -968,6 +1089,15 @@
     return p;
   }
   if (wide_m) {
+    const int64_t lim32 = (1ll << 31) - 64ll * a.x_rstride;
+    if (big && a.tail_pack && a.K > 1 && ck <= 16 && a.prec != 3 && !a.splitk && a.M % 128 == 0 &&
+        (a.epi == EPI_STORE || a.epi == EPI_RESID || a.epi == EPI_RESID_ACC) &&
+        !a.in_lens && !a.out_lens && !a.chan_add && !a.res_chan_add && !a.reflect1 && a.B <= 65535 &&
+        (int64_t)a.B * a.x_bstride < lim32 && (int64_t)a.B * a.y_bstride * 4 < (1ll << 31) &&
+        (int64_t)a.B * a.res_bstride * 4 < (1ll << 31)) {
+      shape(CONV_TAIL_PACK, 128, 384, 512, ck);
+      return p;
+    }
     if (big) shape(CONV_BIG, 128, 384, 512, ck);
     else shape(CONV_SMALL, 128, 128, 256, ck);
   } else {
@@ -999,6 +1129,23 @@
   if (a.epi == EPI_LN && !conv1d_narrow_supported(a)) { fprintf(stderr, "mbv: EPI_LN outside the narrow kernel's range\n"); abort(); }
   const ConvPlan p = conv1d_plan(a, a.trim_map != nullptr, route_T);
   switch (p.route) {
+    case CONV_TAIL_PACK:
+      if (!a.pack_tbl || a.trim_map || a.pack_blocks < 2 * (384 / 32)) {
+        fprintf(stderr, "mbv: conv1d: the packed tail route needs its block table (and takes no tile map)\n");
+        abort();
+      }
+      if (p.ck == 16) {
+        switch (a.epi) {
+          case EPI_STORE: launch_epi<2, 3, 16, 4, EPI_STORE, 0, 2, 2>(a, s); return;
+          case EPI_RESID: launch_epi<2, 3, 16, 4, EPI_RESID, 0, 2, 2>(a, s); return;
+          default: launch_epi<2, 3, 16, 4, EPI_RESID_ACC, 0, 2, 2>(a, s); return;
+        }
+      }
+      switch (a.epi) {
+        case EPI_STORE: launch_epi<2, 3, 8, 4, EPI_STORE, 0, 2, 2>(a, s); return;
+        case EPI_RESID: launch_epi<2, 3, 8, 4, EPI_RESID, 0, 2, 2>(a, s); return;
+        default: launch_epi<2, 3, 8, 4, EPI_RESID_ACC, 0, 2, 2>(a, s); return;
+      }
     case CONV_NARROW_M: launch_conv1d_narrow(a, false, s); return;
     case CONV_NARROW_LAUNCH: launch_conv1d_narrow(a, true, s); return;
     case CONV_VS: {
diff --git a/mb-istft-vits_amd/csrc/kernels.h b/mb-istft-vits_amd/csrc/kernels.h
--- a/mb-istft-vits_amd/csrc/kernels.h
+++ b/mb-istft-vits_amd/csrc/kernels.h
@@ -80,6 +80,9 @@
   const int* trim_map;
   int trim_bn;
   int vs_tv;
+  int tail_pack;
+  const int* pack_tbl;
+  int pack_blocks;
   float* ws;
   size_t ws_floats;
   unsigned* counters;
@@ -101,6 +104,7 @@
   CONV_BIG = 6,
   CONV_SPLIT_BATCH = 7,
   CONV_VS = 8,
+  CONV_TAIL_PACK = 9,
 };
 struct ConvPlan {
   int route;
@@ -486,11 +490,41 @@
 size_t launch_trim_map_ints(int B, int T, int BN);
 void launch_trim_map(const int* lens, int B, int num, int add, int T, int BN, int* out, hipStream_t s);
 constexpr int kTailMapJobs = 24;
-struct TailMapJob { int num, reach, T, BN; int* out; };
+struct TailMapJob { int num, reach, T, BN; int* out; int pack_gap, pad_right; };
 struct TailMapJobs { TailMapJob job[kTailMapJobs]; };
+constexpr int kTailPackHdr = 4;
+__host__ __device__ inline int tail_pack_gap(int halo) { return (halo + 31) & ~31; }
+__host__ __device__ inline int tail_pack_entries_at(int B) { return (kTailPackHdr + B + 3) & ~3; }
+__host__ __device__ inline int tail_pack_blocks(int B, int T, int gap, int BN) {
+  const long per_tile = BN / 32, n = (long)B * ((T + 31) / 32 + gap / 32);
+  return (int)((n + per_tile - 1) / per_tile * per_tile + per_tile);
+}
+__host__ __device__ inline size_t tail_pack_ints(int B, int T, int gap, int BN) {
+  return (size_t)tail_pack_entries_at(B) + 4 * (size_t)tail_pack_blocks(B, T, gap, BN);
+}
+__host__ __device__ inline int tail_pack_sp(long len, int num, int reach, int T, bool donor) {
+  if (donor) return T;
+  long s = len * num + reach;
+  s = s < 0 ? 0 : (s > T ? T : s);
+  s = (s + 31) & ~31L;
+  return (int)(s > T ? T : s);
+}
+__host__ __device__ inline int tail_pack_row_blocks(int sp, int gap) { return (sp + 31) / 32 + gap / 32; }
+__host__ __device__ inline void tail_pack_row(int* out, int B, int b, int first, int sp, int gap, int pad_right) {
+  int* e = out + tail_pack_entries_at(B) + 4 * (long)first;
+  const int n_out = (sp + 31) / 32, n = n_out + gap / 32;
+  for (int k = 0; k < n; ++k, e += 4) { e[0] = b; e[1] = 32 * k; e[2] = sp + pad_right; e[3] = k < n_out; }
+}
+__host__ __device__ inline void tail_pack_finish(int* out, int B, int T, int gap, int BN, int donor, int used) {
+  const int per_tile = BN / 32, cap = tail_pack_blocks(B, T, gap, BN);
+  out[0] = (used + per_tile - 1) / per_tile; out[1] = donor; out[2] = used; out[3] = 0;
+  int* e = out + tail_pack_entries_at(B) + 4 * (long)used;
+  for (int k = used; k < cap; ++k, e += 4) { e[0] = 0; e[1] = 0; e[2] = 0; e[3] = 0; }
+}
 size_t launch_tail_map_ints(int B, int T, int BN);
 void launch_tail_maps(const int* lens, int B, const TailMapJobs& jobs, int n, unsigned long long* dropped, hipStream_t s);
-void launch_tail_fill(float* y, int64_t y_bstride, int B, int M, int T, int BN, const int* map, hipStream_t s);
+void launch_tail_fill(float* y, int64_t y_bstride, int B, int M, int T, int BN, const int* map, hipStream_t s,
+                      bool packed = false);
 constexpr int kRaggedChunk = 256;
 struct RaggedRowsArg { int row[kRaggedChunk]; int len[kRaggedChunk]; };
 void launch_ragged_rows(const RaggedRowsArg& r, int n, int first, int us, int* out, int stride, hipStream_t s);
diff --git a/mb-istft-vits_amd/csrc/ops.hip b/mb-istft-vits_amd/csrc/ops.hip
--- a/mb-istft-vits_amd/csrc/ops.hip
+++ b/mb-istft-vits_amd/csrc/ops.hip
@@ -737,6 +737,32 @@
   const int donor = part_b[0];
   __syncthreads();
   const int full = (T + BN - 1) / BN;
+  if (jb.pack_gap > 0) {
+    const int gap = jb.pack_gap;
+    auto sp_of = [&](int b) { return tail_pack_sp(lens[b], num, reach, T, b == donor); };
+    int s = 0;
+    for (int i = 0; i < per; ++i) { const int b = tid * per + i; if (b < B) s += tail_pack_row_blocks(sp_of(b), gap); }
+    part[tid] = s;
+    __syncthreads();
+    if (tid == 0) { int run = 0; for (int i = 0; i < 256; ++i) { const int v = part[i]; part[i] = run; run += v; } }
+    __syncthreads();
+    int run = part[tid];
+    for (int i = 0; i < per; ++i) {
+      const int b = tid * per + i;
+      if (b < B) {
+        const int sp = sp_of(b);
+        out[kTailPackHdr + b] = sp;
+        tail_pack_row(out, B, b, run, sp, gap, jb.pad_right);
+        run += tail_pack_row_blocks(sp, gap);
+        if (b == B - 1) {
+          tail_pack_finish(out, B, T, gap, BN, donor, run);
+          const long left_out = (long)B * full - out[0];
+          if (dropped && left_out > 0) atomicAdd(dropped, (unsigned long long)left_out);
+        }
+      }
+    }
+    return;
+  }
   auto tiles_of = [&](int b) {
     if (b == donor) return full;
     long lim = (long)lens[b] * num + reach;
@@ -772,12 +798,12 @@
 }
 
 template <bool VEC>
-__global__ void tail_fill_kernel(float* __restrict__ y, int64_t y_bstride, int B, int T, int BN, const int* __restrict__ map) {
+__global__ void tail_fill_kernel(float* __restrict__ y, int64_t y_bstride, int B, int T, int BN, const int* __restrict__ map, int packed) {
   const int m = blockIdx.x, b = blockIdx.y;
   const int full = (T + BN - 1) / BN;
-  const int donor = map[B + 1 + (long)B * full];
+  const int donor = packed ? map[1] : map[B + 1 + (long)B * full];
   if (b == donor) return;
-  const long c0 = (long)(map[b + 1] - map[b]) * BN;
+  const long c0 = packed ? (long)map[kTailPackHdr + b] : (long)(map[b + 1] - map[b]) * BN;
   if (c0 >= T) return;
   const float* src = y + (int64_t)donor * y_bstride + (int64_t)m * T;
   float* dst = y + (int64_t)b * y_bstride + (int64_t)m * T;
@@ -788,10 +814,10 @@
     for (long c = c0 + threadIdx.x; c < T; c += blockDim.x) dst[c] = src[c];
   }
 }
-void launch_tail_fill(float* y, int64_t y_bstride, int B, int M, int T, int BN, const int* map, hipStream_t s) {
+void launch_tail_fill(float* y, int64_t y_bstride, int B, int M, int T, int BN, const int* map, hipStream_t s, bool packed) {
   const bool vec = T % 4 == 0 && y_bstride % 4 == 0 && BN % 4 == 0 && (reinterpret_cast<uintptr_t>(y) & 15) == 0;
-  if (vec) hipLaunchKernelGGL(tail_fill_kernel<true>, dim3(M, B), dim3(256), 0, s, y, y_bstride, B, T, BN, map);
-  else hipLaunchKernelGGL(tail_fill_kernel<false>, dim3(M, B), dim3(256), 0, s, y, y_bstride, B, T, BN, map);
+  if (vec) hipLaunchKernelGGL(tail_fill_kernel<true>, dim3(M, B), dim3(256), 0, s, y, y_bstride, B, T, BN, map, (int)packed);
+  else hipLaunchKernelGGL(tail_fill_kernel<false>, dim3(M, B), dim3(256), 0, s, y, y_bstride, B, T, BN, map, (int)packed);
 }
 
 __global__ void ragged_rows_kernel(const RaggedRowsArg r, int n, int first, int us, int* __restrict__ out, int stride) {
```

Measured after the change: 184.7 million samples/s, median of 6. 1.03x the previous value.
